# Aakash1312/Fluid-Simulation

Measured on AMD Instinct MI355X. Metric: simulated substeps/sec, higher is better.
Workload: dtype f64

## Files before the change

fluid-simulation_amd/csrc/common.h:

```cpp
#pragma once
#include <hip/hip_runtime.h>
#include <stdint.h>

namespace fl {

constexpr uint8_t F_SOLID = 1;
constexpr uint8_t F_FLUID = 2;
constexpr int F_CNT_SHIFT = 2;

struct Grid {
    int N;
    int lo;
    int hi;
    int nx, ny, nz;
    int ox, oy, oz;
    __host__ __device__ inline size_t idx(int ix, int iy, int iz) const
    {
        return ((size_t)ix * ny + (size_t)iy) * nz + (size_t)iz;
    }
    __host__ __device__ inline size_t cells() const { return (size_t)nx * ny * nz; }
    __host__ __device__ inline long sx() const { return (long)ny * nz; }
    __host__ __device__ inline int cx0() const { return lo + ox; }
    __host__ __device__ inline int cy0() const { return lo + oy; }
    __host__ __device__ inline int cz0() const { return lo + oz; }
// ... 153 lines not shown

constexpr int SUM3_PRE = 4;
struct Sum3Loads {
    double a[SUM3_PRE], b[SUM3_PRE], c[SUM3_PRE];
};
__device__ __forceinline__ void sum3_load1(const double* __restrict__ a, int n, double* v)
{
    const int last = n > 0 ? n - 1 : 0;
#pragma unroll
    for (int k = 0; k < SUM3_PRE; ++k) {
        const int i = (int)threadIdx.x + 256 * k;
        v[k] = a[i < last ? i : last];
    }
}
template <bool LATE_C = false>
__device__ __forceinline__ void block_sum3_load(const double* __restrict__ a, int na, const double* __restrict__ b, int nb,
                                                const double* __restrict__ c, int nc, Sum3Loads& v)
{
    sum3_load1(a, na, v.a);
    sum3_load1(nb > 0 ? b : a, nb, v.b);
    if (!LATE_C) sum3_load1(nc > 0 ? c : a, nc, v.c);
}
__device__ __forceinline__ double sum3_thread(const double* __restrict__ a, int n, const double* v)
{
    double s = 0;
#pragma unroll
    for (int k = 0; k < SUM3_PRE; ++k)
        if ((int)threadIdx.x + 256 * k < n) s += v[k];
    for (int i = (int)threadIdx.x + 256 * SUM3_PRE; i < n; i += 256) s += a[i];
    return s;
}
template <bool LATE_C = false>
__device__ __forceinline__ void block_sum3_sum(Sum3Loads& v, const double* __restrict__ a, int na, const double* __restrict__ b, int nb,
                                               const double* __restrict__ c, int nc, double* sm, double& ra, double& rb, double& rc)
{
    if (LATE_C) sum3_load1(nc > 0 ? c : a, nc, v.c);
    double va = sum3_thread(a, na, v.a), vb = sum3_thread(b, nb, v.b), vc = sum3_thread(c, nc, v.c);
    va = wave_sum(va); vb = wave_sum(vb); vc = wave_sum(vc);
    const int lane = threadIdx.x & 63, w = threadIdx.x >> 6;
    if (lane == 0) { sm[w] = va; sm[4 + w] = vb; sm[8 + w] = vc; }
    __syncthreads();
    ra = ((sm[0] + sm[1]) + sm[2]) + sm[3];
    rb = ((sm[4] + sm[5]) + sm[6]) + sm[7];
    rc = ((sm[8] + sm[9]) + sm[10]) + sm[11];
}
__device__ __forceinline__ void block_sum3(const double* __restrict__ a, int na, const double* __restrict__ b, int nb,
                                           const double* __restrict__ c, int nc, double* sm, double& ra, double& rb, double& rc)
{
    Sum3Loads v;
    block_sum3_load(a, na, b, nb, c, nc, v);
    block_sum3_sum(v, a, na, b, nb, c, nc, sm, ra, rb, rc);
}

struct Particles {
    double *px, *py, *pz, *vx, *vy, *vz;
    uint32_t* pid;
    __host__ __device__ inline Particles shifted(long o) const
    {
        Particles q = *this;
        q.px += o; q.py += o; q.pz += o; q.vx += o; q.vy += o; q.vz += o; q.pid += o;
        return q;
    }
};
constexpr uint32_t PID_DEAD = 0xFFFFFFFFu;

void launch_bin_count(hipStream_t st, Grid g, long n, Particles p, int* key, int* slot, int* cell_count, int* part, StepState* ss);
void launch_bin_scatter(hipStream_t st, long n, const int* key, const int* slot, const int* cell_start, const uint32_t* pid, int* order,
                         uint32_t* spid);
void launch_bin_rank(hipStream_t st, long n_pos, long pos0, const int* key, const int* cell_start, const int* order, const uint32_t* spid,
                     int* order2);
void launch_reorder(hipStream_t st, long n, const int* order, Particles src, Particles dst, double* w = nullptr, long wstride = 0);
void launch_weights(hipStream_t st, long n, Particles p, double* w, long stride);
void launch_axpby_box(hipStream_t st, Grid g, Box box, double a, const double* x, double b, const double* y, double* out, const PcgState* gate = nullptr);
long p2g_max_items(Box box);
size_t p2g_part_doubles(Box box);
constexpr int P2G_PILED = 256;
void launch_p2g(hipStream_t st, Grid g, Box box, Particles p, const double* pw, long wstride, const int* cell_start, const uint8_t* flags,
                double* part, int* items, float* container, double* u, double* v, double* w, double* ub, double* vb, double* wb, int2* crowd_list = nullptr,
                Particles park = Particles{});
void launch_p2g_tiles(hipStream_t st, Grid g, Box box, Particles p, const double* pw, long wstride, const int* cell_start, const uint8_t* flags,
                      float* container, double* u, double* v, double* w, double* ub, double* vb, double* wb);
void launch_g2p_tiled(hipStream_t st, Grid g, Box pb, Particles p, const int* cell_start, const double* dcx, const double* dcy, const double* dcz,
                      const double* pcx, const double* pcy, const double* pcz, double blend, StepState* ss);
void launch_g2p(hipStream_t st, Grid g, long n, Particles p, const double* dcx, const double* dcy, const double* dcz, const double* pcx,
                const double* pcy, const double* pcz, double blend, StepState* ss);
void launch_advect(hipStream_t st, Grid g, long n, Particles p, const uint8_t* flags, double max_dt, double dx, StepState* ss);
void launch_advect_bin(hipStream_t st, Grid g, long n, Particles p, const uint8_t* flags, double max_dt, double dx, StepState* ss, int* key,
                       int* slot, int* cell_count, int* part);
void launch_pack_particles(hipStream_t st, long n, Particles p, double* pos_aos, double* vel_aos);
void launch_unpack_records(hipStream_t st, long n, const double* rec, Particles p, long off);
void launch_pack_records(hipStream_t st, long n, Particles p, long off, double* rec);
void launch_unpack_ids(hipStream_t st, long n, const double* pos, const double* vel, const uint32_t* ids, Particles p);
void launch_pack_ids(hipStream_t st, long n, Particles p, long off, double* pos, double* vel, uint32_t* ids);
void launch_unpack_particles(hipStream_t st, long n, const double* pos_aos, const double* vel_aos, Particles p);

struct OutWin {
    int ny, nz;
    int ox, oy, oz;
    int olo[3], ohi[3];
    int lo, off;
    int l0[3], nl[3];
    __host__ __device__ inline long leaves() const { return (long)nl[0] * nl[1] * nl[2]; }
};
void launch_out_mark(hipStream_t st, const float* f, const OutWin& w, int* flags);
void launch_out_pack(hipStream_t st, const float* f, const OutWin& w, const int* flags, const int* slot, float* values, int* origin);
struct SdfGeom {
    int lo, hi;
    int bx0, by0, bz0, bnx, bny, bnz;
    int L0;
    int l0[3], nl[3];
    float R, w, dxf, bg, max2, min2;
    __host__ __device__ inline long leaves() const { return (long)nl[0] * nl[1] * nl[2]; }
    __host__ __device__ inline long cells() const { return (long)bnx * bny * bnz; }
};
void launch_sdf_bbox(hipStream_t st, long n, Particles p, int lo, int hi, int* box, bool live = false);
void launch_sdf_count(hipStream_t st, long n, Particles p, const SdfGeom& g, int* cnt, int* place, bool live = false);
void launch_sdf_scatter(hipStream_t st, long n, Particles p, const SdfGeom& g, const int* start, const int* place, double* sx, double* sy,
                        double* sz, int* ssrc = nullptr);
void launch_sdf_search(hipStream_t st, const SdfGeom& g, const int* start, const double* sx, const double* sy, const double* sz, float* tv,
                       uint64_t* tm, int* flags, unsigned* visits);
void launch_sdf_pack(hipStream_t st, const SdfGeom& g, const int* flags, const int* slot, const float* tv, const uint64_t* tm, float* values,
                     uint64_t* active, int* origin);
void launch_sdf_search_attr(hipStream_t st, const SdfGeom& g, const int* start, const double* sx, const double* sy, const double* sz, float* tv,
                            uint64_t* tm, int* flags, const int* ssrc, Particles p, uint32_t* tid, float* tvel,
                            float* tmin = nullptr);
void launch_sdf_pack_attr(hipStream_t st, const SdfGeom& g, const int* flags, const int* slot, const float* tv, const uint64_t* tm, float* values,
                          uint64_t* active, int* origin, const uint32_t* tid, const float* tvel, uint32_t* ids, float* vel,
                          const float* tmin = nullptr, float* dist2 = nullptr);
void launch_sdf_box(hipStream_t st, const SdfGeom& g, int axis, int W, float off, const int* flags, const uint64_t* tm, const float* src,
                    float* dst);
void launch_sdf_offset(hipStream_t st, const SdfGeom& g, float off, const int* flags, const uint64_t* tm, float* tv);
void launch_sdf_track(hipStream_t st, const SdfGeom& g, bool norm, bool trim, const int* flags, uint64_t* tm, const float* src, float* dst,
                      uint32_t* tid, float* tvel);
void launch_sdf_relist(hipStream_t st, const SdfGeom& g, const int* flags, const uint64_t* tm, const float* tv, int* list);
void launch_mesh_mark(hipStream_t st, const SdfGeom& g, const float* tv, const int* flags, uint64_t* cmask, int* cpre, int* vcnt, int* qcnt,
                      unsigned* tot);
void launch_mesh_emit(hipStream_t st, const SdfGeom& g, const float* tv, const int* flags, const uint64_t* tm, const float* tvel,
                      const uint64_t* cmask, const int* cpre, const int* vcnt, const int* qcnt, const int* vbase, const int* qbase, float* vertices,
                      uint32_t* quads, float* vvel, float* vnrm);
void launch_mesh_tris(hipStream_t st, long nq, long nv, const uint32_t* quads, const float* vertices, uint32_t* tris);
struct RenderGeom {
    SdfGeom g;
    int any;
    int ne[3];
    int e0[3], e1[3];
    __host__ __device__ inline long ext_leaves() const { return (long)ne[0] * ne[1] * ne[2]; }
};
}
struct fluid_camera;
struct fluid_shade;
namespace fl {
void launch_render(hipStream_t st, const RenderGeom& r, const fluid_camera& cam, const fluid_shade& sh, const float* tv, const int* flags,
                   unsigned char* neg, unsigned* occ, unsigned* hits, unsigned char* rgb, float* depth, float* normals);
void launch_exclusive_scan(hipStream_t st, const int* in, int* out, long n, int* block_sums, int* total);
void launch_sort_tail(hipStream_t st, const int* cell_count, int* cell_start, long c1, long ncell);
void launch_index_scan(hipStream_t st, Grid g, const uint8_t* flags, int* indices, int* block_sums, int* total);
void launch_index_scan_flat(hipStream_t st, const uint8_t* flags, int* indices, long n, int* block_sums, int* total);
void launch_flags(hipStream_t st, Grid g, const uint8_t* solid, const float* container, uint8_t* flags, int x0, int x1);
void launch_index_scan_range(hipStream_t st, Grid g, const uint8_t* flags, int* indices, int* block_sums, int* total, int x0, int x1);
void launch_rhs_div(hipStream_t st, Grid g, Box box, const uint8_t* flags, const double* u, const double* v, const double* w,
                    float* rhs, float* diver, double dx, double gdt0, double gdt1, double gdt2, bool rows = false, const PcgState* gate = nullptr);
void launch_vel_update(hipStream_t st, Grid g, Box box, const uint8_t* flags, const double* p, double* u, double* v, double* w,
                       double k, double g0, double g1, double g2, bool rows = false, const PcgState* gate = nullptr);
void launch_flip_delta(hipStream_t st, Grid g, Box box, const double* u, const double* v, const double* w,
                       const double* ub, const double* vb, const double* wb, double* dcx, double* dcy, double* dcz, double* pcx, double* pcy, double* pcz);
void launch_err_norm(hipStream_t st, Grid g, Box box, const uint8_t* flags, const float* b, const float* b2, double* part, StepState* ss,
                     const PcgState* gate = nullptr);
void launch_zero_step_state(hipStream_t st, StepState* ss, int N);
struct ZeroList { float* f4[4]; double* f8[7]; };
void launch_zero_fields(hipStream_t st, const ZeroList& z, Grid g, Box box, bool rows = false);
void launch_unpack_box(hipStream_t st, Grid g, Box box, const double* buf, float* container, double* u, double* v, double* w, double* ub, double* vb,
                       double* wb);

void launch_extrap_init(hipStream_t st, Grid g, const uint8_t* solid, const float* container, int* layer);
void launch_extrap_layer(hipStream_t st, Grid g, int pass, int* layer, double* u, double* v, double* w, int* n_new);
void launch_resample(hipStream_t st, Grid g, long n, Particles p, const int* cell_start, int per_cell, int xlim, double far_, int* n_parked);

struct SinkSet { int n; Box box[8]; };
__host__ __device__ inline uint64_t sm64(uint64_t x)
{
    uint64_t z = x + 0x9E3779B97F4A7C15ull;
    z = (z ^ (z >> 30)) * 0xBF58476D1CE4E5B9ull;
    z = (z ^ (z >> 27)) * 0x94D049BB133111EBull;
    return z ^ (z >> 31);
}
struct OwnBox {
    int lo[3], hi[3];
    int has_lo[3], has_hi[3];
};
struct SolidView {
    const uint8_t* p;
    int o[3];
    long sx, sy;
};
void launch_src_count(hipStream_t st, Grid g, long n, Particles p, Box box, int* hist, bool skip_dead);
void launch_src_plan(hipStream_t st, Grid g, Box box, uint64_t h0, int per_cell, bool fill, OwnBox ob, SolidView sv, const int* hist, int* cnt,
                     int* cnt_own);
void launch_src_emit(hipStream_t st, Grid g, Box box, uint64_t h0, int per_cell, bool fill, OwnBox ob, SolidView sv, const int* hist, const int* off,
                     const int* off_own, Particles p, uint32_t id0, const double vel[3]);
void launch_src_append(hipStream_t st, long n, const double* pos, const double* vel, Particles p, uint32_t pid0);
void launch_interp_from_grid(hipStream_t st, Grid g, long n, Particles p, const double* u, const double* v, const double* w);
void launch_sink_mark(hipStream_t st, Grid g, long n, Particles p, const SinkSet& sk, int* keep_dev, int* keep_pid, int* removed);
void launch_sink_compact(hipStream_t st, long n, Particles a, Particles b, const int* keep_dev, const int* dev_off, const int* pid_new);

void launch_spline_eval(hipStream_t st, int which, long n, const double* x, double* w);
void launch_dot(hipStream_t st, long n, const double* a, const double* b, double* part, int nb, double* out);

LBox make_lbox(const Box& b);
size_t lbox_max_cells(int N);
int pcg_sq_blocks(const LBox& L);
int pcg_xr_blocks(const LBox& L);
void launch_cnt_local(hipStream_t st, Grid g, LBox L, const uint8_t* flags, uint8_t* cnt);
template <typename T>
void launch_pcg_init(hipStream_t st, Grid g, LBox L, const uint8_t* cnt, const float* b, T* x, T* r, Coef<T> cf, double* part_bb,
                     double* part_rz0, PcgState* ps);
template <typename T>
void launch_pcg_sq(hipStream_t st, LBox L, const uint8_t* cnt, const T* r, const T* s_in, T* s_out, T* q, Coef<T> cf,
                   const double* part_rr, const double* part_rz_new, const double* part_rz_old, double* part_pq, PcgState* ps, int first,
                   double tol, int n_rz = -1, int zmode = 0, int sparse = 0, int n_prev = -1);
template <typename T>
void launch_pcg_xr(hipStream_t st, LBox L, const uint8_t* cnt, T* x, T* r, const T* s, const T* q, Coef<T> cf, const double* part_rz_cur,
                   const double* part_pq, double* part_rr, double* part_rz_next, PcgState* ps, int n_rz = -1, int sparse = 0);
void launch_pcg_sq_zf(hipStream_t st, LBox L, const uint8_t* cnt, const float* z, const double* s_in, double* s_out, double* q, Coef<double> cf,
                      const double* part_rr, int n_prev, const double* part_rz_new, const double* part_rz_old, double* part_pq, PcgState* ps, int first,
                      double tol, int n_rz, int sparse, const int* tlist, int nlist);
int pcg_list_blocks(int nlist);
template <typename T>
void launch_pcg_sq_list(hipStream_t st, LBox L, const uint8_t* cnt, const T* r, const T* s_in, T* s_out, T* q, Coef<T> cf,
                        const double* part_rr, int n_prev, const double* part_rz_new, const double* part_rz_old, double* part_pq, PcgState* ps,
                        int first, double tol, int n_rz, int zmode, const int* tlist, int nlist);
template <typename T>
void launch_pcg_xr_list(hipStream_t st, LBox L, const uint8_t* cnt, T* x, T* r, const T* s, const T* q, Coef<T> cf, const double* part_rz_cur,
                        int n_rz, const double* part_pq, double* part_rr, double* part_rz_next, PcgState* ps, const int* tlist, int nlist);
int pcg_row_count(const LBox& L);
int pcg_rows_blocks(int nrows);
void launch_row_list(hipStream_t st, LBox L, const uint8_t* cnt, int* flags, int* pos, int* list, int* block_sums, int* count);
constexpr int DROP_CAP = 65536;
constexpr int DROP_NCTR = 64;
void launch_drop_find(hipStream_t st, LBox L, uint8_t* cnt, int* ctr, int* pre, int* total, int* comp_n, int* comp_cells, const Box* own = nullptr);
void launch_drop_solve(hipStream_t st, Grid g, LBox L, int n_comp, const int* pre, const int* comp_n, const int* comp_cells, const uint8_t* flags,
                       const float* b, Coef<double> cf, double tol, double* pressure, double* keep, int* n_fail = nullptr, const PcgState* gate = nullptr);
template <typename T>
void launch_pcg_xr_rows(hipStream_t st, LBox L, const uint8_t* cnt, T* x, T* r, const T* s, const T* q, Coef<T> cf, const double* part_rz_cur,
                        int n_rz, const double* part_pq, int n_pq, double* part_rr, double* part_rz_next, PcgState* ps, const int* rlist, int nrows);
template <typename T>
void launch_pcg_sq_dist(hipStream_t st, LBox L, const uint8_t* cnt, const T* r, const T* s_in, T* s_out, T* q, Coef<T> cf, const double* g_rr,
                        const double* g_rz_new, const double* g_rz_old, double* part_pq, PcgState* ps, int first, double tol, int zmode);
template <typename T>
void launch_pcg_xr_dist(hipStream_t st, LBox L, const uint8_t* cnt, T* x, T* r, const T* s, const T* q, Coef<T> cf, const double* g_rz_cur,
                        const double* g_pq, double* part_rr, double* part_rz_next, PcgState* ps);
void launch_sum2(hipStream_t st, const double* a, int na, const double* b, int nb, double* out_a, double* out_b);
void launch_pcg_az_dist_zf(hipStream_t st, LBox L, const uint8_t* cnt, const float* z, double* w, Coef<double> cf, double* part_zw, PcgState* ps, const int* tlist, int nlist);
void launch_pcg_cgear_upd_zf(hipStream_t st, LBox L, const uint8_t* cnt, double* x, double* r, double* s, double* q, const float* z, const double* w, const double* g,
                             double* cg, int cur, double* part_rr, PcgState* ps, int first, double tol);
void launch_pcg_poll_stage(hipStream_t st, const double* part_rr, int n, const PcgState* ps, double* out);
void launch_pcg_poll_test(hipStream_t st, const double* g, PcgState* ps);
void launch_sum4(hipStream_t st, const double* a, int na, const double* b, int nb, const double* c, int nc, const double* e, int ne, double* out);
template <typename T>
void launch_pcg_az_dist(hipStream_t st, LBox L, const uint8_t* cnt, const T* z, T* w, Coef<T> cf, double* part_zw, PcgState* ps, const int* tlist = nullptr,
                        int nlist = 0);
template <typename T>
void launch_pcg_cgear_upd(hipStream_t st, LBox L, const uint8_t* cnt, T* x, T* r, T* s, T* q, const T* z, const T* w, const double* g, double* cg, int cur,
                          double* part_rr, PcgState* ps, int first, double tol);
template <typename T>
void launch_stencil_apply(hipStream_t st, Grid g, Box box, const uint8_t* flags, const T* s, T* q, Coef<T> cf);
template <typename T>
bool launch_stencil_march(hipStream_t st, Grid g, const uint8_t* flags, const T* s, T* q, Coef<T> cf, int variant, int cxcode);
template <typename T>
void launch_store_pressure(hipStream_t st, Grid g, LBox L, const uint8_t* cnt, const T* x, double* pressure, double* keep = nullptr,
                           const PcgState* ps = nullptr, bool gated = false);
template <typename T>
void launch_pcg_init_guess(hipStream_t st, Grid g, LBox L, const uint8_t* cnt, const float* b, const double* guess, const double* guess2, double ca,
                           double cb, T* x, T* r, Coef<T> cf, double* part_bb, double* part_rr0, PcgState* ps);

MLevel mg_level0(const LBox& L);
MLevel mg_coarser(const MLevel& f);
void launch_mg_type0(hipStream_t st, Grid g, LBox L, MLevel m, const uint8_t* flags, const uint8_t* cnt, uint8_t* typ);
void launch_mg_coarsen(hipStream_t st, MLevel mf, const uint8_t* tf, MLevel mc, uint8_t* tc, uint8_t* cnt_c);
void launch_mg_coarsen_types(hipStream_t st, MLevel mf, const uint8_t* tf, MLevel mc, uint8_t* tc);
void launch_mg_counts(hipStream_t st, MLevel m, const uint8_t* typ, uint8_t* cnt);
template <typename T>
void launch_mg_restrict(hipStream_t st, MLevel mf, const T* rf, MLevel mc, const uint8_t* cnt_c, T* fc, const PcgState* ps);
constexpr int MG_TAIL_MAX = 4;
constexpr size_t MG_TAIL_LDS = 144 * 1024;
size_t mg_tail_lds_bytes(int nl, const MLevel* lv, size_t elem);
int mg_up_blocks(const MLevel& m);
template <typename T, typename F>
void launch_mg_down(hipStream_t st, MLevel m, const uint8_t* cnt, const F* f, T* u, T* r, MLevel mc, const uint8_t* cnt_c, T* fc, MgCoef<T> cf,
                    const PcgState* ps, const int* tlist = nullptr, int nlist = 0, bool pcr = false);
template <typename T, typename F, typename O>
void launch_mg_up(hipStream_t st, MLevel m, const uint8_t* cnt, const F* f, const T* u, O* out, MLevel mc, const T* ec, MgCoef<T> cf,
                  double* part_dot, const PcgState* ps, double wc, const int* tlist = nullptr, int nlist = 0, const uint8_t* own = nullptr,
                  int pconst = 0);
bool gal_fits_coarsest(const MLevel& m);
void launch_gal_level1(hipStream_t st, MLevel m0, const uint8_t* cnt0, MgCoef<float> cf0, MLevel m1, float* gd, float* gx, float* gy, float* gz, uint8_t* cnt1);
void launch_gal_coarsen(hipStream_t st, MLevel mf, const float* fd, const float* fx, const float* fy, const float* fz, const uint8_t* cntf, MLevel mc,
                        float* gd, float* gx, float* gy, float* gz, uint8_t* cntc);
int gal_tile_count(const MLevel& m);
void launch_gal_tile_flags(hipStream_t st, MLevel m, const uint8_t* cnt, uint8_t* flags);
void launch_gal_down(hipStream_t st, MLevel m, const uint8_t* cnt, const float* gd, const float* gx, const float* gy, const float* gz, const float* f, float* u,
                     MLevel mc, float* fc, const PcgState* ps);
void launch_gal_up(hipStream_t st, MLevel m, const uint8_t* cnt, const float* gd, const float* gx, const float* gy, const float* gz, const float* f, const float* u,
                   float* out, MLevel mc, const float* ec, float wc, const PcgState* ps);
void launch_gal_coarsest(hipStream_t st, MLevel m, const float* gd, const float* gx, const float* gy, const float* gz, const float* f, float* u, int sweeps,
                         const PcgState* ps);
void launch_mg_tile_flags(hipStream_t st, MLevel m, const uint8_t* cnt, uint8_t* flags);
void launch_sq_tile_flags(hipStream_t st, LBox L, const uint8_t* cnt, uint8_t* flags);
int sq_tile_count(const LBox& L);
void launch_compact_flags(hipStream_t st, const uint8_t* flags, int n, int* list, int* count);
template <typename T>
void launch_mg_tail(hipStream_t st, int nl, const T* f0, const MLevel* lv, uint8_t* const* cnt, T* u0, const T* off, int sweeps, const PcgState* ps,
                    double wc);

}
```

fluid-simulation_amd/csrc/fluid_api.hip:

```cpp
#include "sim.h"
#include <algorithm>

using namespace fl;

static thread_local std::string g_err;
int fluid_fail(int code, const std::string& msg)
{
    g_err = msg;
    return code;
}
#define fail fluid_fail

Box fl::clip_dilate(const Box& b, int d, const Grid& g)
{
    Box r;
    r.x0 = b.x0 - d < 0 ? 0 : b.x0 - d;
    r.y0 = b.y0 - d < 0 ? 0 : b.y0 - d;
    r.z0 = b.z0 - d < 0 ? 0 : b.z0 - d;
    r.x1 = b.x1 + d > g.nx - 1 ? g.nx - 1 : b.x1 + d;
    r.y1 = b.y1 + d > g.ny - 1 ? g.ny - 1 : b.y1 + d;
    r.z1 = b.z1 + d > g.nz - 1 ? g.nz - 1 : b.z1 + d;
    return r;
}

// ... 124 lines not shown
    p->cg_tol = 2.220446049250313e-16;
    p->cg_max_iters = 0;
    p->max_outer_passes = 0;
    p->precision = FLUID_PRECISION_FP64;
    p->preconditioner = FLUID_PRECOND_MG;
    p->flip_blend = 1.0;
    p->solve_start = FLUID_START_WARM;
    p->mg_precision = FLUID_MG_FP32;
    p->dist_solve = FLUID_DIST_AUTO;
    return FLUID_OK;
}

int fluid_destroy(fluid_sim_t* s)
{
    if (!s) return FLUID_OK;
    if (s->st) hipStreamSynchronize(s->st);
    if (s->ds) dist_destroy(s);
    prof_resolve(s);
    free_particles(s);
    sources_free(s);
    output_free(s);
    render_free(s);
    mesh_free(s);
    sdf_free(s);
    void* ptrs[] = {s->solid, s->flags, s->container, s->rhs, s->diver, s->diver2, s->u, s->v, s->w, s->ub, s->vb, s->wb, s->dcx, s->dcy,
                    s->dcz, s->pressure, s->p_guess, s->p_guess2, s->p_q, s->indices, s->scan_sums, s->ipart, s->R, s->S[0], s->Q, s->X, s->mg_slab, s->mg_part, s->cntL, s->part_bb, s->part_rr,
                    s->part_rz[0], s->part_rz[1], s->part_pq, s->part_err, s->cell_count, s->cell_start, s->ss,
                    s->pcx, s->pcy, s->pcz, s->p2g_part, s->p2g_items, s->p2g_crowd, s->tl_flags, s->tl_mg, s->tl_sq, s->d_small, s->row_flags, s->row_pos, s->row_list, s->drop_n, s->drop_cells, s->drop_ctr, s->gal_slab};
    for (void* p : ptrs) if (p) hipFree(p);
    for (int i = 0; i < 2; ++i) if (s->ev_poll[i]) hipEventDestroy(s->ev_poll[i]);
    if (s->h_ss) hipHostFree(s->h_ss);
    if (s->h_small) hipHostFree(s->h_small);
    if (s->st) hipStreamDestroy(s->st);
    delete s;
    return FLUID_OK;
}

int fluid_create(const fluid_params_t* p, fluid_sim_t** out)
{
    if (!p || !out) return fail(FLUID_ERR_ARG, "null argument");
    Grid g;
    g.N = p->n;
    g.lo = -(p->n / 2);
    g.hi = g.lo + p->n - 1;
    g.nx = g.ny = g.nz = p->n;
    g.ox = g.oy = g.oz = 0;
    return fluid_create_window(p, g, out);
}

}

int fl::fluid_create_window(const fluid_params_t* p, const Grid& g, fluid_sim_t** out)
{
    if (!p || !out) return fail(FLUID_ERR_ARG, "null argument");
    if (p->n < 8 || p->n > 1024) return fail(FLUID_ERR_ARG, "n must be in [8,1024]");
    if (!(p->dx > 0) || !(p->rho > 0) || !(p->max_dt > 0)) return fail(FLUID_ERR_ARG, "dx, rho, max_dt must be > 0");
    if (p->precision != FLUID_PRECISION_FP64 && p->precision != FLUID_PRECISION_FP32) return fail(FLUID_ERR_ARG, "bad precision");
    if (!(p->flip_blend >= 0.0 && p->flip_blend <= 1.0)) return fail(FLUID_ERR_ARG, "flip_blend must be in [0,1] (1 = the reference's pure FLIP)");
    if (p->preconditioner != FLUID_PRECOND_MG && p->preconditioner != FLUID_PRECOND_JACOBI) return fail(FLUID_ERR_ARG, "bad preconditioner");
    if (p->solve_start != FLUID_START_WARM && p->solve_start != FLUID_START_ZERO) return fail(FLUID_ERR_ARG, "bad solve_start");
    if (p->mg_precision != FLUID_MG_FP32 && p->mg_precision != FLUID_MG_FP64) return fail(FLUID_ERR_ARG, "bad mg_precision");
    if (p->dist_solve < FLUID_DIST_AUTO || p->dist_solve > FLUID_DIST_REPLICATED || p->pad_ != 0) return fail(FLUID_ERR_ARG, "bad dist_solve / pad_");
    int ndev = 0;
    if (hipGetDeviceCount(&ndev) != hipSuccess || ndev <= 0)
        return fail(FLUID_ERR_HIP, "no HIP device visible: libfluid_hip has no CPU path");
    if (p->device < 0 || p->device >= ndev) return fail(FLUID_ERR_ARG, "device ordinal out of range");
    HIPCHK(hipSetDevice(p->device));
    fluid_sim* s = new fluid_sim();
    s->prm = *p;
    s->g = g;
    s->ncell = g.cells();
    s->dt = p->max_dt;
    s->mg_fp32 = p->mg_precision == FLUID_MG_FP32;
    s->warm = p->solve_start == FLUID_START_WARM;
    if (const char* e = getenv("FLUID_MG_CSWEEPS")) s->mg_csweeps = atoi(e);
    if (const char* e = getenv("FLUID_TILE_LISTS")) s->lists_force = atoi(e) != 0;
    if (const char* e = getenv("FLUID_P2G_FORM")) s->p2g_force = !strcmp(e, "rows") ? 1 : (!strcmp(e, "tiles") ? 2 : (!strcmp(e, "crowd") ? 3 : 0));
    if (const char* e = getenv("FLUID_MG_GALERKIN")) s->gal_mode = atoi(e);
    if (const char* e = getenv("FLUID_DROPLETS")) s->drops_on = atoi(e) != 0;
    if (const char* e = getenv("FLUID_ROW_SWEEPS")) s->row_sweeps = atoi(e) != 0;
    if (const char* e = getenv("FLUID_DROPLETS_MIN")) s->drop_min = atoi(e);
    if (const char* e = getenv("FLUID_ADVECT_BIN")) s->advect_bin = atoi(e) != 0;
    if (const char* e = getenv("FLUID_SOLVE_TAIL")) s->solve_tail = atoi(e) != 0;
    *out = nullptr;
    auto bail = [&](int rc) { fluid_destroy(s); return rc; };
#define A(expr) do { hipError_t e_ = (expr); if (e_ != hipSuccess) return bail(fail(FLUID_ERR_HIP, std::string(#expr) + ": " + hipGetErrorString(e_))); } while (0)
    A(hipStreamCreateWithFlags(&s->st, hipStreamNonBlocking));
    const size_t n = s->ncell;
    A(dalloc(&s->solid, n)); A(dalloc(&s->flags, n));
    A(dalloc(&s->container, n)); A(dalloc(&s->rhs, n)); A(dalloc(&s->diver, n)); A(dalloc(&s->diver2, n));
    A(dalloc(&s->u, n)); A(dalloc(&s->v, n)); A(dalloc(&s->w, n));
    A(dalloc(&s->ub, n)); A(dalloc(&s->vb, n)); A(dalloc(&s->wb, n));
    A(dalloc(&s->dcx, n)); A(dalloc(&s->dcy, n)); A(dalloc(&s->dcz, n));
    A(dalloc(&s->pressure, n));
    if (s->warm) {
        A(dalloc(&s->p_guess, n)); A(dalloc(&s->p_guess2, n));
        if (hipMemset(s->p_guess, 0, n * sizeof(double)) != hipSuccess || hipMemset(s->p_guess2, 0, n * sizeof(double)) != hipSuccess) return bail(FLUID_ERR_HIP);
        if (const char* e = getenv("FLUID_EXTRAPOLATE")) s->extrapolate = atoi(e) != 0;
        if (s->extrapolate) { A(dalloc(&s->p_q, n)); if (hipMemset(s->p_q, 0, n * sizeof(double)) != hipSuccess) return bail(FLUID_ERR_HIP); }
    }
    A(dalloc(&s->indices, n));
    A(dalloc(&s->scan_sums, (n + 2) / 2048 + 16));
    A(dalloc(&s->ipart, (size_t)1024 * 8));
    const size_t se = solver_elem(s);
    s->lmax = lbox_max_cells(std::max(g.nx, std::max(g.ny, g.nz)));
    const size_t ln = s->lmax;
    A(dalloc((char**)&s->R, ln * se)); A(dalloc((char**)&s->S[0], 2 * ln * se + 256));
    s->S[1] = (char*)s->S[0] + ln * se;
    A(dalloc((char**)&s->Q, ln * se)); A(dalloc((char**)&s->X, ln * se)); A(dalloc(&s->cntL, ln + 64));
    A(dalloc(&s->mg_part, ln / 256 + 64));
    A(dalloc(&s->part_bb, (size_t)MAX_PARTIALS)); A(dalloc(&s->part_rr, (size_t)MAX_PARTIALS));
    A(dalloc(&s->part_rz[0], (size_t)MAX_PARTIALS)); A(dalloc(&s->part_rz[1], (size_t)MAX_PARTIALS));
    A(dalloc(&s->part_pq, (size_t)MAX_PARTIALS)); A(dalloc(&s->part_err, (size_t)2 * MAX_PARTIALS));
    static_assert(sizeof(StepState) <= STATE_PS_OFF, "PcgState overlaps StepState");
    A(dalloc((char**)&s->ss, STATE_PS_OFF + sizeof(PcgState)));
    s->ps = (PcgState*)((char*)s->ss + STATE_PS_OFF);
    A(dalloc(&s->cell_count, n + 4)); A(dalloc(&s->cell_start, n + 4));
    A(dalloc(&s->d_small, (size_t)32));
    A(hipHostMalloc((void**)&s->h_small, 32 * sizeof(int)));
    A(hipEventCreateWithFlags(&s->ev_poll[0], hipEventDisableTiming));
    A(hipEventCreateWithFlags(&s->ev_poll[1], hipEventDisableTiming));
    A(hipHostMalloc((void**)&s->h_ss, STATE_PS_OFF + 2 * sizeof(PcgState)));
    s->h_ps = (PcgState*)((char*)s->h_ss + STATE_PS_OFF);
#undef A
    std::vector<uint8_t> sol(n, 0);
    const int N = p->n;
    for (int x = 0; x < g.nx; ++x)
        for (int y = 0; y < g.ny; ++y)
            for (int z = 0; z < g.nz; ++z) {
                const int X = x + g.ox, Y = y + g.oy, Z = z + g.oz;
                if (X < 2 || X > N - 3 || Y < 2 || Y > N - 3 || Z < 2 || Z > N - 3) sol[g.idx(x, y, z)] = 1;
            }
    hipError_t e = hipMemcpy(s->solid, sol.data(), n, hipMemcpyHostToDevice);
    if (e == hipSuccess) e = hipMemcpy(s->flags, sol.data(), n, hipMemcpyHostToDevice);
    if (e == hipSuccess) e = hipDeviceSynchronize();
    if (e != hipSuccess) return bail(fail(FLUID_ERR_HIP, std::string("solid upload: ") + hipGetErrorString(e)));
    *out = s;
    return FLUID_OK;
}

extern "C" {

int fluid_set_solid(fluid_sim_t* s, const uint8_t* solid)
{
    if (!s || !solid) return fail(FLUID_ERR_ARG, "null argument");
    const int N = s->g.N;
    const Grid g = s->g;
    for (int x = 0; x < N; ++x)
        for (int y = 0; y < N; ++y)
            for (int z = 0; z < N; ++z) {
                size_t c = ((size_t)x * N + y) * N + z;
                bool outsideW = x < 2 || x > N - 3 || y < 2 || y > N - 3 || z < 2 || z > N - 3;
                if (outsideW && !solid[c]) return fail(FLUID_ERR_ARG, "cells outside W=[lo+2,hi-2]^3 must be solid");
            }
    std::vector<uint8_t> sol(s->ncell);
    for (int x = 0; x < g.nx; ++x)
        for (int y = 0; y < g.ny; ++y)
            for (int z = 0; z < g.nz; ++z)
                sol[g.idx(x, y, z)] = solid[((size_t)(x + g.ox) * N + (y + g.oy)) * N + (z + g.oz)] ? 1 : 0;
    dist_keep_solid(s, solid);
    HIPCHK(hipStreamSynchronize(s->st));
    HIPCHK(hipMemcpy(s->solid, sol.data(), s->ncell, hipMemcpyHostToDevice));
    HIPCHK(hipMemcpy(s->flags, sol.data(), s->ncell, hipMemcpyHostToDevice));
    s->have_p2g = s->have_flags = false;
    s->flags_valid = false;
    s->have_guess = false;
// ... 23 lines not shown
    s->binned = false;
    s->vel_ok = false;
    return FLUID_OK;
}

int fluid_download_particles(fluid_sim_t* s, double* pos, double* vel)
{
    if (!s || !pos || !vel) return fail(FLUID_ERR_ARG, "null argument");
    if (s->dist) return fail(FLUID_ERR_STATE, "decomposed run: use fluid_download_particles_ids");
    if (s->np == 0) return FLUID_OK;
    HIPCHK(hipSetDevice(s->prm.device));
    launch_pack_particles(s->st, s->np, s->pa.shifted(s->p_off), s->stage_pos, s->stage_vel);
    HIPCHK(hipGetLastError());
    HIPCHK(hipMemcpyAsync(pos, s->stage_pos, 3 * s->np * sizeof(double), hipMemcpyDeviceToHost, s->st));
    HIPCHK(hipMemcpyAsync(vel, s->stage_vel, 3 * s->np * sizeof(double), hipMemcpyDeviceToHost, s->st));
    HIPCHK(hipStreamSynchronize(s->st));
    return FLUID_OK;
}

int64_t fluid_num_particles(fluid_sim_t* s) { return s ? s->np : -1; }
int fluid_set_dt(fluid_sim_t* s, double dt)
{
    if (!s || !(dt > 0)) return fail(FLUID_ERR_ARG, "dt must be > 0");
    s->dt = dt;
    return FLUID_OK;
}
int fluid_get_dt(fluid_sim_t* s, double* dt)
{
    if (!s || !dt) return fail(FLUID_ERR_ARG, "null argument");
    *dt = s->dt;
    return FLUID_OK;
}

static inline double u01(uint64_t seed, uint64_t ctr)
{
    uint64_t z = seed * 0x9E3779B97F4A7C15ull + ctr * 0xBF58476D1CE4E5B9ull + 0x94D049BB133111EBull;
    z ^= z >> 30; z *= 0xBF58476D1CE4E5B9ull;
    z ^= z >> 27; z *= 0x94D049BB133111EBull;
    z ^= z >> 31;
    return (double)(z >> 11) * (1.0 / 9007199254740992.0);
}

int64_t fluid_scene_water_cube_drop(int32_t n, int32_t ppc, uint64_t seed, double* pos)
{
    if (n < 8 || ppc < 1) return -1;
    const int m = (int)std::lround((double)n * 41.0 / 121.0);
    const int c0 = -(m / 2), c1 = c0 + m - 1;
    const int lo = -(n / 2), hi = lo + n - 1;
    int64_t cnt = 0;
    uint64_t ctr = 0;
    for (int x = c0; x <= c1; ++x)
        for (int y = c0; y <= c1; ++y)
            for (int z = c0; z <= c1; ++z)
                for (int k = 0; k < ppc; ++k) {
                    const double px = x - 0.5 + u01(seed, ctr), py = y - 0.5 + u01(seed, ctr + 1), pz = z - 0.5 + u01(seed, ctr + 2);
                    ctr += 3;
                    if (px > lo + 2 && px < hi - 2 && py > lo + 2 && py < hi - 2 && pz > lo + 2 && pz < hi - 2) {
                        if (pos) { pos[3 * cnt] = px; pos[3 * cnt + 1] = py; pos[3 * cnt + 2] = pz; }
                        cnt++;
                    }
                }
    return cnt;
}

}

int fl::read_ss(fluid_sim* s)
{
    HIPCHK(hipMemcpyAsync(s->h_ss, s->ss, sizeof(StepState), hipMemcpyDeviceToHost, s->st));
    HIPCHK(hipStreamSynchronize(s->st));
    return FLUID_OK;
}

int fl::clear_dirty(fluid_sim* s)
{
    if (box_empty(s->dirty)) return FLUID_OK;
    const ZeroList z = {{s->container, s->rhs, s->diver, s->diver2}, {s->u, s->v, s->w, s->ub, s->vb, s->wb, s->pressure}};
    launch_zero_fields(s->st, z, s->g, s->dirty, !s->dist && s->row_sweeps);
    HIPCHK(hipGetLastError());
    s->dirty = Box{0, 0, 0, -1, -1, -1};
    return FLUID_OK;
}

int fl::sort_pass(fluid_sim* s, int ax0, int ax1, int* h_tail)
{
    const Grid g = s->g;
    const long ncell = (long)s->ncell, n2 = g.sx();
    const long c0 = (long)ax0 * n2, c1 = (long)(ax1 + 1) * n2;
    launch_zero_step_state(s->st, s->ss, g.N);
    HIPCHK(hipMemsetAsync(s->cell_count + c0, 0, (c1 - c0) * sizeof(int), s->st));
    HIPCHK(hipMemsetAsync(s->cell_count + ncell, 0, 4 * sizeof(int), s->st));
    launch_bin_count(s->st, g, s->np, s->pa.shifted(s->p_off), s->key, s->slot, s->cell_count, s->ipart, s->ss);
    launch_exclusive_scan(s->st, s->cell_count + c0, s->cell_start + c0, c1 - c0, s->scan_sums, s->cell_start + c1);
    launch_sort_tail(s->st, s->cell_count, s->cell_start, c1, ncell);
    launch_bin_scatter(s->st, s->np, s->key, s->slot, s->cell_start, s->pa.shifted(s->p_off).pid, s->order, s->spid);
    launch_bin_rank(s->st, s->np, 0, s->key, s->cell_start, s->order, s->spid, s->order2);
    HIPCHK(hipGetLastError());
    if (h_tail) HIPCHK(hipMemcpyAsync(h_tail, s->cell_start + ncell, 3 * sizeof(int), hipMemcpyDeviceToHost, s->st));
    return read_ss(s);
}

static int sort_binned(fluid_sim* s)
{
    const Grid g = s->g;
    const long ncell = (long)s->ncell, n2 = g.sx();
    const long c0 = (long)s->bin_x0 * n2, c1 = (long)(s->bin_x1 + 1) * n2;
    launch_zero_step_state(s->st, s->ss, g.N);
    launch_exclusive_scan(s->st, s->cell_count + c0, s->cell_start + c0, c1 - c0, s->scan_sums, s->cell_start + c1);
    launch_sort_tail(s->st, s->cell_count, s->cell_start, c1, ncell);
    launch_bin_scatter(s->st, s->np, s->key, s->slot, s->cell_start, s->pa.shifted(s->p_off).pid, s->order, s->spid);
    launch_bin_rank(s->st, s->np, 0, s->key, s->cell_start, s->order, s->spid, s->order2);
    HIPCHK(hipGetLastError());
    StepState& h = *s->h_ss;
    for (int a = 0; a < 3; ++a) h.bbox_min[a] = s->bin_min[a], h.bbox_max[a] = s->bin_max[a];
    h.n_out = s->bin_n_out;
    h.max_cell = s->bin_max_cell;
    return FLUID_OK;
}

static int phase_sort(fluid_sim* s)
{
    const Grid g = s->g;
    int tok = prof_begin(s, FLUID_PROF_SORT, (double)s->np);
    int ax0 = 0, ax1 = g.nx - 1;
    const bool guess = s->sort_hint && !box_empty(s->Pb);
    if (guess) {
        ax0 = std::max(0, s->Pb.x0 - 3);
        ax1 = std::min(g.nx - 1, s->Pb.x1 + 3);
    }
    const bool binned = s->binned && guess && ax0 == s->bin_x0 && ax1 == s->bin_x1 && s->np > 0;
    s->binned = false;
    const auto missed = [&](const int* bmin, const int* bmax) {
        return guess && bmax[0] >= 0 && (bmin[0] < std::min(ax0 + 2, s->Pb.x0) || bmax[0] > std::max(ax1 - 2, s->Pb.x1));
    };
    int rc;
    if (binned && !missed(s->bin_min, s->bin_max)) {
        if ((rc = sort_binned(s))) return rc;
    } else {
        rc = binned ? FLUID_OK : sort_pass(s, ax0, ax1);
        if (rc) return rc;
        if (binned || missed(s->h_ss->bbox_min, s->h_ss->bbox_max)) {
            if ((rc = sort_pass(s, 0, g.nx - 1))) return rc;
        }
    }
    s->sort_hint = true;
    s->n_out = s->h_ss->n_out;
    s->max_cell = s->h_ss->max_cell;
    const StepState& h = *s->h_ss;
    if (h.bbox_max[0] < 0) {
        s->Pb = Box{0, 0, 0, -1, -1, -1};
    } else {
        s->Pb = Box{h.bbox_min[0], h.bbox_min[1], h.bbox_min[2], h.bbox_max[0], h.bbox_max[1], h.bbox_max[2]};
    }
    if (!box_empty(s->Pb)) {
        s->Rb = clip_dilate(s->Pb, 1, g);
        s->Sb = clip_dilate(s->Pb, 2, g);
    } else {
        s->Rb = s->Sb = s->Pb;
    }
    launch_reorder(s->st, s->np, s->order2, s->pa.shifted(s->p_off), s->pb, s->pw, s->cap);
    HIPCHK(hipGetLastError());
    std::swap(s->pa, s->pb);
    s->p_off = 0;
    prof_end(s, FLUID_PROF_SORT, tok);
    s->sorted = true;
    return FLUID_OK;
}

int fl::run_p2g(fluid_sim* s, const Box& box)
{
    const long ref_cells = s->p2g_ref_cells > 0 ? s->p2g_ref_cells : s->Rb.cells();
    const bool airy = s->last_num_active > 0 && (double)s->last_num_active < 0.3 * (double)ref_cells;
    const bool huge = (size_t)12 * sizeof(double) * (size_t)box.cells() > ((size_t)16 << 30);
    const bool piled = s->max_cell > P2G_PILED || airy;
    if (s->p2g_force ? s->p2g_force == 2 : huge) {
        s->stats.paths |= FLUID_PATH_P2G_TILES;
        launch_p2g_tiles(s->st, s->g, box, s->pa, s->pw, s->cap, s->cell_start, s->flags, s->container, s->u, s->v, s->w, s->ub, s->vb, s->wb);
        return FLUID_OK;
    }
    const bool crowd = s->p2g_force ? s->p2g_force == 3 : piled;
    if (crowd) {
        s->stats.paths |= FLUID_PATH_P2G_CROWD;
        const size_t nl = (size_t)s->cap / 16 + 64;
        if (nl > s->p2g_crowd_cap) {
            if (s->p2g_crowd) { HIPCHK(hipStreamSynchronize(s->st)); hipFree(s->p2g_crowd); s->p2g_crowd = nullptr; }
            HIPCHK(hipMalloc((void**)&s->p2g_crowd, nl * sizeof(int2)));
            s->p2g_crowd_cap = nl;
        }
    }
    const size_t need = p2g_part_doubles(box);
    if (need > s->p2g_part_cap) {
        if (s->p2g_part) { HIPCHK(hipStreamSynchronize(s->st)); hipFree(s->p2g_part); s->p2g_part = nullptr; }
// ... 32 lines not shown
        prof_end(s, FLUID_PROF_P2G, tok);
        if (rc) return rc;
        HIPCHK(hipGetLastError());
        s->dirty = s->Sb;
    }
    s->have_p2g = true;
    s->step_counter++;
    s->have_flags = false;
    return FLUID_OK;
}

template <typename T>
Coef<T> fl::make_coef(const fluid_sim* s)
{
    const double scale = s->dt / (s->prm.rho * s->prm.dx * s->prm.dx);
    Coef<T> c;
    float acc = 0.0f;
    c.diag[0] = 0;
    c.inv[0] = 0;
    for (int k = 1; k <= 6; ++k) {
        acc = (float)((double)acc + scale);
        c.diag[k] = (T)acc;
        c.inv[k] = (T)1 / c.diag[k];
    }
    c.off = (T)(float)(-1 * scale);
    return c;
}
template Coef<double> fl::make_coef<double>(const fluid_sim*);
template Coef<float> fl::make_coef<float>(const fluid_sim*);

hipError_t fl::zero_search(fluid_sim* s, size_t lb)
{
    const size_t step = (lb + 255) / 256 * 256;
    s->S[1] = (char*)s->S[0] + step;
    return hipMemsetAsync(s->S[0], 0, step + lb, s->st);
}


static int gal_build(fluid_sim* s);
static int mg_setup(fluid_sim* s)
{
    s->mgl[0] = mg_level0(s->L);
    int nl = 1;
    while (nl < fluid_sim::MG_MAXL && (nl < 2 || s->mgl[nl - 1].dx > 8 || s->mgl[nl - 1].dy > 8 || s->mgl[nl - 1].dz > 8)) {
        s->mgl[nl] = mg_coarser(s->mgl[nl - 1]);
        ++nl;
    }
    if (s->mgl[nl - 1].dx > 8 || s->mgl[nl - 1].dy > 8 || s->mgl[nl - 1].dz > 8) return fail(FLUID_ERR_STATE, "multigrid: too many levels");
    s->mg_nl = nl;
    int tail = nl - 1;
    const size_t es = s->mg_fp32 ? sizeof(float) : sizeof(double);
    auto fits = [&](int t) {
        const size_t b = nl - t <= MG_TAIL_MAX ? mg_tail_lds_bytes(nl - t, s->mgl + t, es) : 0;
        return b > 0 && b <= MG_TAIL_LDS;
    };
    while (tail > 1 && fits(tail - 1)) --tail;
    if (!fits(tail)) return fail(FLUID_ERR_STATE, "multigrid: coarsest level does not fit the tail kernel");
    s->mg_tail = tail;
    size_t total = 0;
    auto take = [&](size_t bytes) { const size_t o = total; total += (bytes + 255) / 256 * 256; return o; };
    size_t o_typ[fluid_sim::MG_MAXL], o_cnt[fluid_sim::MG_MAXL], o_u[fluid_sim::MG_MAXL], o_v[fluid_sim::MG_MAXL], o_f[fluid_sim::MG_MAXL],
        o_r[fluid_sim::MG_MAXL];
    for (int l = 0; l < nl; ++l) {
        const size_t c = s->mgl[l].cells + 64;
        o_typ[l] = take(c); o_cnt[l] = take(c);
        o_u[l] = take(c * es); o_v[l] = take(c * es); o_f[l] = take(c * es); o_r[l] = take(c * es);
    }
    const size_t o_z = take((s->mgl[0].cells + 64) * 8);
    if (total > s->mg_slab_cap) {
        if (s->mg_slab) { HIPCHK(hipStreamSynchronize(s->st)); hipFree(s->mg_slab); s->mg_slab = nullptr; }
        const size_t cap = total + total / 4;
        HIPCHK(hipMalloc((void**)&s->mg_slab, cap));
        s->mg_slab_cap = cap;
    }
    for (int l = 0; l < nl; ++l) {
        s->mg_typ[l] = (uint8_t*)(s->mg_slab + o_typ[l]);
        s->mg_cnt[l] = l ? (uint8_t*)(s->mg_slab + o_cnt[l]) : nullptr;
        s->mg_u[l] = s->mg_slab + o_u[l]; s->mg_v[l] = s->mg_slab + o_v[l];
        s->mg_f[l] = l ? s->mg_slab + o_f[l] : nullptr;
        s->mg_r[l] = s->mg_slab + o_r[l];
    }
    s->Zmg = s->mg_slab + o_z;
    HIPCHK(hipMemsetAsync(s->mg_slab, 0, total, s->st));
    launch_mg_type0(s->st, s->g, s->L, s->mgl[0], s->flags, s->cntL, s->mg_typ[0]);
    for (int l = 1; l < nl; ++l) launch_mg_coarsen(s->st, s->mgl[l - 1], s->mg_typ[l - 1], s->mgl[l], s->mg_typ[l], s->mg_cnt[l]);
    { int rcg = gal_build(s); if (rcg) return rcg; }
    HIPCHK(hipGetLastError());
    return FLUID_OK;
}

MgCoef<double> fl::mg_coef(const fluid_sim* s, int level)
{
    MgCoef<double> c;
    if (level == 0) {
        const Coef<double> f = make_coef<double>(s);
        for (int k = 0; k < 7; ++k) { c.diag[k] = f.diag[k]; c.inv[k] = f.inv[k]; }
        c.off = f.off;
        return c;
    }
    const double scale = s->dt / (s->prm.rho * s->prm.dx * s->prm.dx) / std::pow(4.0, level);
    c.off = -scale;
    c.diag[0] = 0; c.inv[0] = 0;
    for (int k = 1; k < 7; ++k) { c.diag[k] = scale * k; c.inv[k] = 1.0 / c.diag[k]; }
    return c;
}

static int mg_rz_blocks(const fluid_sim* s) { return s->lists_on ? s->n_tl_mg : mg_up_blocks(s->mgl[0]); }

template <typename V>
static MgCoef<V> mg_coef_as(const fluid_sim* s, int level)
{
    const MgCoef<double> d = mg_coef(s, level);
    MgCoef<V> c;
    for (int k = 0; k < 7; ++k) { c.diag[k] = (V)d.diag[k]; c.inv[k] = (V)d.inv[k]; }
    c.off = (V)d.off;
    return c;
}
static int gal_build(fluid_sim* s)
{
    s->gal = false;
    s->gal_eligible = false;
    const int nl = s->mg_nl;
    int lc = 1;
    while (lc < nl - 1 && !gal_fits_coarsest(s->mgl[lc])) ++lc;
    if (!(s->gal_mode && s->lists_on && s->mg_fp32 && !s->dist && (long)s->mgl[0].dx * s->mgl[0].dy * s->mgl[0].dz > 200000 &&
          gal_fits_coarsest(s->mgl[lc]) && lc >= 2)) {
        s->gal_it[0] = s->gal_it[1] = -1;
        return FLUID_OK;
    }
    s->gal_eligible = true;
    bool use = s->gal_mode >= 2;
    if (s->gal_mode == 1) {
        if (s->gal_it[0] < 0) use = false;
        else if (s->gal_it[1] < 0) use = true;
        else {
            use = 21 * s->gal_it[1] < 20 * s->gal_it[0];
            if (++s->gal_since_probe >= 32) { use = !use; s->gal_since_probe = 0; }
        }
    }
    if (!use) return FLUID_OK;
    size_t total = 0, off[fluid_sim::MG_MAXL][6];
    for (int l = 1; l <= lc; ++l)
        for (int q = 0; q < 6; ++q) {
            off[l][q] = total;
            total += (q < 5 ? ((q < 4 ? sizeof(float) : 1) * (s->mgl[l].cells + 64) + 255) / 256 * 256 : ((size_t)gal_tile_count(s->mgl[l]) + 255) / 256 * 256);
        }
    if (total > s->gal_slab_cap) {
        if (s->gal_slab) { HIPCHK(hipStreamSynchronize(s->st)); hipFree(s->gal_slab); s->gal_slab = nullptr; }
        HIPCHK(hipMalloc((void**)&s->gal_slab, total + total / 4));
        s->gal_slab_cap = total + total / 4;
    }
    HIPCHK(hipMemsetAsync(s->gal_slab, 0, total, s->st));
    for (int l = 1; l <= lc; ++l) {
        for (int q = 0; q < 4; ++q) s->gal_c[l][q] = (float*)(s->gal_slab + off[l][q]);
        s->gal_cnt[l] = (uint8_t*)(s->gal_slab + off[l][4]);
        s->gal_tfl[l] = (uint8_t*)(s->gal_slab + off[l][5]);
    }
    launch_gal_level1(s->st, s->mgl[0], s->cntL, mg_coef_as<float>(s, 0), s->mgl[1], s->gal_c[1][0], s->gal_c[1][1], s->gal_c[1][2], s->gal_c[1][3], s->gal_cnt[1]);
    for (int l = 2; l <= lc; ++l)
        launch_gal_coarsen(s->st, s->mgl[l - 1], s->gal_c[l - 1][0], s->gal_c[l - 1][1], s->gal_c[l - 1][2], s->gal_c[l - 1][3], s->gal_cnt[l - 1], s->mgl[l],
                           s->gal_c[l][0], s->gal_c[l][1], s->gal_c[l][2], s->gal_c[l][3], s->gal_cnt[l]);
    for (int l = 1; l < lc; ++l) launch_gal_tile_flags(s->st, s->mgl[l], s->gal_cnt[l], s->gal_tfl[l]);
    s->gal = true;
    s->gal_lc = lc;
    s->gal_dt = s->dt;
    HIPCHK(hipGetLastError());
    return FLUID_OK;
}
static int mg_vcycle_gal(fluid_sim* s, const double* rhs0, float* z0, double* part_rz)
{
    typedef float V;
    const PcgState* ps = s->ps;
    const int lc = s->gal_lc;
    auto U = [&](int l) { return (V*)s->mg_u[l]; };
    auto W = [&](int l) { return (V*)s->mg_v[l]; };
    auto F = [&](int l) { return (V*)s->mg_f[l]; };
    auto C = [&](int l, int q) { return (const float*)s->gal_c[l][q]; };
    const MLevel& m0 = s->mgl[0];
    launch_mg_down<V, double>(s->st, m0, s->cntL, rhs0, U(0), (V*)s->mg_r[0], s->mgl[1], nullptr, F(1), mg_coef_as<V>(s, 0), ps, s->tl_mg, s->n_tl_mg, true);
    for (int l = 1; l < lc; ++l) launch_gal_down(s->st, s->mgl[l], s->gal_tfl[l], C(l, 0), C(l, 1), C(l, 2), C(l, 3), F(l), U(l), s->mgl[l + 1], F(l + 1), ps);
    launch_gal_coarsest(s->st, s->mgl[lc], C(lc, 0), C(lc, 1), C(lc, 2), C(lc, 3), F(lc), U(lc), s->gal_sweeps, ps);
    for (int l = lc - 1; l >= 1; --l)
        launch_gal_up(s->st, s->mgl[l], s->gal_tfl[l], C(l, 0), C(l, 1), C(l, 2), C(l, 3), F(l), U(l), W(l), s->mgl[l + 1], l + 1 == lc ? U(l + 1) : W(l + 1),
                      (float)s->gal_wc, ps);
    const int tok = prof_begin(s, FLUID_PROF_MG_UP0, (double)s->Rb.cells());
    launch_mg_up<V, double, float>(s->st, m0, s->cntL, rhs0, (const V*)U(0), z0, s->mgl[1], W(1), mg_coef_as<V>(s, 0), part_rz, ps, s->gal_wc, s->tl_mg, s->n_tl_mg,
                                   nullptr, 1);
    prof_end(s, FLUID_PROF_MG_UP0, tok);
    HIPCHK(hipGetLastError());
    return FLUID_OK;
}

template <typename V>
static int mg_vcycle_t(fluid_sim* s, const double* rhs0, V* z0, double* part_rz)
{
    const int nl = s->mg_nl, tail = s->mg_tail;
    const PcgState* ps = s->ps;
    auto U = [&](int l) { return (V*)s->mg_u[l]; };
    auto W = [&](int l) { return (V*)s->mg_v[l]; };
    auto F = [&](int l) { return (V*)s->mg_f[l]; };
    auto R = [&](int l) { return (V*)s->mg_r[l]; };
    for (int l = 0; l < tail; ++l) {
        const MLevel& m = s->mgl[l];
        const bool fold = l > 0 || (long)m.dx * m.dy * m.dz <= 200000;
        V* fc = fold ? F(l + 1) : nullptr;
        const uint8_t* cc = fold ? s->mg_cnt[l + 1] : nullptr;
        const bool lst = s->lists_on && !fold;
        if (l == 0) launch_mg_down<V, double>(s->st, m, s->cntL, rhs0, U(0), R(0), s->mgl[1], cc, fc, mg_coef_as<V>(s, 0), ps, lst ? s->tl_mg : nullptr, s->n_tl_mg);
        else launch_mg_down<V, V>(s->st, m, s->mg_cnt[l], (const V*)F(l), U(l), R(l), s->mgl[l + 1], cc, fc, mg_coef_as<V>(s, l), ps);
        if (!fold) launch_mg_restrict<V>(s->st, m, (const V*)R(l), s->mgl[l + 1], s->mg_cnt[l + 1], F(l + 1), ps);
    }
    {
        V off[fluid_sim::MG_MAXL];
        for (int l = tail; l < nl; ++l) off[l] = (V)mg_coef(s, l).off;
        launch_mg_tail<V>(s->st, nl - tail, (const V*)F(tail), s->mgl + tail, s->mg_cnt + tail, U(tail), off + tail, s->mg_csweeps, ps, s->mg_wc[3]);
    }
    for (int l = tail - 1; l >= 0; --l) {
        const MLevel& m = s->mgl[l];
        const V* ec = l + 1 == tail ? U(l + 1) : W(l + 1);
        if (l == 0) {
            const int tok = prof_begin(s, FLUID_PROF_MG_UP0, (double)s->Rb.cells());
            launch_mg_up<V, double, V>(s->st, m, s->cntL, rhs0, (const V*)U(0), z0, s->mgl[1], ec, mg_coef_as<V>(s, 0), part_rz, ps, s->mg_wc[0],
                                       s->lists_on ? s->tl_mg : nullptr, s->n_tl_mg);
            prof_end(s, FLUID_PROF_MG_UP0, tok);
        } else {
            launch_mg_up<V, V, V>(s->st, m, s->mg_cnt[l], (const V*)F(l), (const V*)U(l), W(l), s->mgl[l + 1], ec, mg_coef_as<V>(s, l), nullptr, ps, s->mg_wc[l == 1 ? 1 : 2]);
        }
    }
    HIPCHK(hipGetLastError());
    return FLUID_OK;
}
static int mg_vcycle(fluid_sim* s, const double* rhs0, void* z0, double* part_rz)
{
    if (s->gal && s->lists_on) return mg_vcycle_gal(s, rhs0, (float*)z0, part_rz);
    return s->mg_fp32 ? mg_vcycle_t<float>(s, rhs0, (float*)z0, part_rz) : mg_vcycle_t<double>(s, rhs0, (double*)z0, part_rz);
}

static int phase_vel_update(fluid_sim* s, const PcgState* gate = nullptr);
static int phase_rhs_div(fluid_sim* s, int which, const PcgState* gate = nullptr);
static int solve_mg(fluid_sim* s, bool with_tail)
{
    typedef double T;
    const Grid g = s->g;
    const LBox L = s->L;
    T* X = (T*)s->X;
    T* R = (T*)s->R;
    T* Q = (T*)s->Q;
    T* Sx[2] = {(T*)s->S[0], (T*)s->S[1]};
    T* Z = (T*)s->Zmg;
    const uint8_t* cnt = s->cntL;
    const Coef<T> cf = make_coef<T>(s);
    const double tol = s->prm.cg_tol;
    long max_it = s->prm.cg_max_iters > 0 ? s->prm.cg_max_iters : 2 * (long)s->stats.num_active;
    if (max_it < 1) max_it = 1;
    const double cells = (double)s->Rb.cells();
    const int sparse = (double)s->stats.num_active < 0.4 * (double)L.cells();
    const bool lists = s->lists_on;
    const bool rows = lists && s->rows_on && s->n_rows > 0;
    const int n_init = pcg_xr_blocks(L), n_list = rows ? pcg_rows_blocks(s->n_rows) : pcg_list_blocks(s->n_tl_sq);
    const int n_rz_raw = mg_rz_blocks(s);
    const bool fold = n_rz_raw > 1024;
    const int n_rz = fold ? 1 : n_rz_raw;
    int rc;
    int tsolve = prof_begin(s, FLUID_PROF_SOLVE, cells);
    if (s->gal && s->gal_dt != s->dt) {
        const int keep = s->gal_mode; s->gal_mode = 2; rc = gal_build(s); s->gal_mode = keep;
        if (rc) return rc;
    }
    if (s->gal) s->stats.paths |= FLUID_PATH_MG_GALERKIN;
    const bool guess = s->warm && s->have_guess;
    const double *g1, *g2;
    double gca, gcb;
    s->start_guess(g1, g2, gca, gcb);
    if (guess) launch_pcg_init_guess<T>(s->st, g, L, cnt, s->diver, g1, g2, gca, gcb, X, R, cf, s->part_bb, s->part_rz[1], s->ps);
    else launch_pcg_init<T>(s->st, g, L, cnt, s->diver, X, R, cf, s->part_bb, s->part_rr, s->ps);
    long it = 0;
    const int pclass = s->pass_class();
    long batch = s->mg_last_iters_k[pclass] > 5 ? s->mg_last_iters_k[pclass] + 1 : 4;
    bool done = false;
    const bool zf = s->mg_fp32 || (s->gal && s->lists_on);
    auto sq = [&](int cur, const double* part_rr, int n_prev, const double* rz_new, const double* rz_old, int first, int sp) {
        const int prv = cur ^ 1;
        if (zf)
            launch_pcg_sq_zf(s->st, L, cnt, (const float*)s->Zmg, Sx[prv], Sx[cur], Q, cf, part_rr, n_prev, rz_new, rz_old, s->part_pq, s->ps, first, tol, n_rz, sp,
                             lists ? s->tl_sq : nullptr, s->n_tl_sq);
        else if (lists)
            launch_pcg_sq_list<T>(s->st, L, cnt, Z, Sx[prv], Sx[cur], Q, cf, part_rr, n_prev, rz_new, rz_old, s->part_pq, s->ps, first, tol, n_rz, 1, s->tl_sq, s->n_tl_sq);
        else
            launch_pcg_sq<T>(s->st, L, cnt, Z, Sx[prv], Sx[cur], Q, cf, part_rr, rz_new, rz_old, s->part_pq, s->ps, first, tol, n_rz, 1, sp, n_prev);
    };
    const bool will_make_q = s->warm && s->p_q && s->stats.outer_passes == 1 && s->guess_step == s->step_counter && s->guess_pass == 0;
    auto solution_out = [&](const PcgState* gate) {
        launch_store_pressure<T>(s->st, g, L, cnt, X, s->pressure, s->warm ? s->p_guess2 : nullptr, s->ps, gate != nullptr);
        launch_drop_solve(s->st, g, L, s->n_drop, s->drop_ctr + 64 * DROP_NCTR, s->drop_n, s->drop_cells, s->flags, s->diver, make_coef<double>(s), tol,
                          s->pressure, s->warm ? s->p_guess2 : nullptr, &s->ss->n_drop_fail, gate);
        if (will_make_q) launch_axpby_box(s->st, g, s->Rb, 1.0, s->p_guess2, -(1.0 - s->prm.update_frac), s->p_guess, s->p_q, gate);
    };
    bool first_poll = true;
// ... 224 lines not shown
    HIPCHK(hipStreamSynchronize(s->st));
    int iters = s->h_ps->iters;
    const double rr = s->h_ps->rr;
    if (!s->h_ps->done) {
        iters = (int)max_it;
    }
    launch_store_pressure<T>(s->st, g, L, cnt, X, s->pressure);
    launch_drop_solve(s->st, g, L, s->n_drop, s->drop_ctr + 64 * DROP_NCTR, s->drop_n, s->drop_cells, s->flags, s->diver, make_coef<double>(s), tol,
                      s->pressure, nullptr, &s->ss->n_drop_fail);
    HIPCHK(hipGetLastError());
    prof_end(s, FLUID_PROF_SOLVE, tsolve);
    s->stats.cg_iters_last = iters;
    s->stats.cg_iters += iters;
    s->stats.relres = s->h_ps->bb > 0 ? std::sqrt(rr / s->h_ps->bb) : 0.0;
    if (s->h_ps->breakdown) return fail(FLUID_ERR_SOLVER, "PCG breakdown: s.As <= 0 or NaN (matrix not SPD for these flags)");
    return FLUID_OK;
}

static int phase_solve(fluid_sim* s, bool with_tail = false)
{
    s->tail_ran = false;
    if (!s->have_flags) return fail(FLUID_ERR_STATE, "solve before flags_index");
    if (box_empty(s->Rb)) return FLUID_OK;
    if (use_mg(s) && s->mg_nl >= 2) return solve_mg(s, with_tail);
    return s->prm.precision == FLUID_PRECISION_FP32 ? solve_impl<float>(s) : solve_impl<double>(s);
}

static int phase_vel_update(fluid_sim* s, const PcgState* gate)
{
    if (!s->have_flags) return fail(FLUID_ERR_STATE, "vel_update before flags_index");
    if (box_empty(s->Sb)) return FLUID_OK;
    const double dtp = s->dt * s->prm.update_frac;
    const double k = dtp / (s->prm.rho * s->prm.dx);
    launch_vel_update(s->st, s->g, s->Sb, s->flags, s->pressure, s->u, s->v, s->w, k, s->prm.gravity[0] * dtp, s->prm.gravity[1] * dtp,
                      s->prm.gravity[2] * dtp, !s->dist && s->row_sweeps, gate);
    HIPCHK(hipGetLastError());
    return FLUID_OK;
}

int fl::phase_pressure_pass(fluid_sim* s, double* error)
{
    int rc;
    if ((rc = phase_rhs_div(s, 0))) return rc;
    if ((rc = phase_solve(s, true))) return rc;
    const bool tail_ran = s->tail_ran;
    s->tail_ran = false;
    if (!tail_ran) {
        if ((rc = phase_vel_update(s))) return rc;
        if ((rc = phase_rhs_div(s, 1))) return rc;
    }
    double err = NAN;
    if (!box_empty(s->Rb)) {
        if (!tail_ran) {
            launch_err_norm(s->st, s->g, s->Rb, s->flags, s->diver, s->diver2, s->part_err, s->ss);
            HIPCHK(hipGetLastError());
            if ((rc = read_ss(s))) return rc;
        }
        if (s->h_ss->n_drop_fail > 0) s->stats.paths |= FLUID_PATH_DROPLETS_SHORT;
        err = std::sqrt(s->h_ss->err_num) / std::sqrt(s->h_ss->err_den);
    }
    s->stats.error = err;
    s->stats.outer_passes++;
    if (error) *error = err;
    return FLUID_OK;
}

int fl::pic_fields(fluid_sim* s)
{
    if (s->prm.flip_blend >= 1.0 || s->pcx) return FLUID_OK;
    double** f[3] = {&s->pcx, &s->pcy, &s->pcz};
    for (double** q : f) {
        HIPCHK(hipMalloc((void**)q, s->ncell * sizeof(double)));
        HIPCHK(hipMemsetAsync(*q, 0, s->ncell * sizeof(double), s->st));
    }
    return FLUID_OK;
}

static int phase_flip_advect(fluid_sim* s)
{
    if (!s->have_p2g) return fail(FLUID_ERR_STATE, "flip_advect before p2g");
    HIPCHK(hipSetDevice(s->prm.device));
    int rcp = pic_fields(s);
    if (rcp) return rcp;
    if (!box_empty(s->Rb)) launch_flip_delta(s->st, s->g, s->Rb, s->u, s->v, s->w, s->ub, s->vb, s->wb, s->dcx, s->dcy, s->dcz, s->pcx, s->pcy, s->pcz);
    int tok = prof_begin(s, FLUID_PROF_G2P, (double)s->np);
    if (s->sorted && s->p_off == 0 && (double)s->np >= 4.0 * (double)s->Pb.cells()) {
        launch_g2p_tiled(s->st, s->g, s->Pb, s->pa, s->cell_start, s->dcx, s->dcy, s->dcz, s->pcx, s->pcy, s->pcz, s->prm.flip_blend, s->ss);
        if (!box_empty(s->Pb)) s->stats.paths |= FLUID_PATH_G2P_TILES;
        if (s->n_out > 0)
            launch_g2p(s->st, s->g, s->n_out, s->pa.shifted(s->np - s->n_out), s->dcx, s->dcy, s->dcz, s->pcx, s->pcy, s->pcz, s->prm.flip_blend, s->ss);
    } else {
        launch_g2p(s->st, s->g, s->np, s->pa.shifted(s->p_off), s->dcx, s->dcy, s->dcz, s->pcx, s->pcy, s->pcz, s->prm.flip_blend, s->ss);
    }
    prof_end(s, FLUID_PROF_G2P, tok);
    const bool bin = s->advect_bin && !s->dist && s->np > 0 && s->sorted && s->sort_hint && !box_empty(s->Pb);
    s->binned = false;
    if (bin) {
        const Grid g = s->g;
        s->bin_x0 = std::max(0, s->Pb.x0 - 3);
        s->bin_x1 = std::min(g.nx - 1, s->Pb.x1 + 3);
        const long n2 = g.sx(), c0 = (long)s->bin_x0 * n2, c1 = (long)(s->bin_x1 + 1) * n2;
        HIPCHK(hipMemsetAsync(s->cell_count + c0, 0, (c1 - c0) * sizeof(int), s->st));
        HIPCHK(hipMemsetAsync(s->cell_count + s->ncell, 0, 4 * sizeof(int), s->st));
        launch_advect_bin(s->st, g, s->np, s->pa.shifted(s->p_off), s->flags, s->prm.max_dt, s->prm.dx, s->ss, s->key, s->slot, s->cell_count, s->ipart);
    } else {
        launch_advect(s->st, s->g, s->np, s->pa.shifted(s->p_off), s->flags, s->prm.max_dt, s->prm.dx, s->ss);
    }
    HIPCHK(hipGetLastError());
    int rc = read_ss(s);
    if (rc) return rc;
    if (bin) {
        const StepState& h = *s->h_ss;
        for (int a = 0; a < 3; ++a) s->bin_min[a] = h.bbox_min[a], s->bin_max[a] = h.bbox_max[a];
        s->bin_n_out = h.n_out;
        s->bin_max_cell = h.max_cell;
        s->binned = true;
    }
    s->dt = s->h_ss->dt;
    double ms;
    memcpy(&ms, &s->h_ss->max_speed_bits, sizeof(double));
    s->stats.max_speed = ms;
    s->stats.dt_out = s->dt;
    s->sorted = false;
    s->have_p2g = false;
    s->vel_ok = true;
    return FLUID_OK;
}

extern "C" {

#define PHASE_GUARD(s)                                                                                        \
    if (!(s)) return fail(FLUID_ERR_ARG, "null handle");                                                      \
    if ((s)->dist) return fail(FLUID_ERR_STATE, "per-phase entry points are single-GPU only; a decomposed run steps with fluid_step")
int fluid_p2g(fluid_sim_t* s) { PHASE_GUARD(s); return phase_p2g(s); }
int fluid_flags_index(fluid_sim_t* s) { PHASE_GUARD(s); return phase_flags(s); }
int fluid_rhs_div(fluid_sim_t* s, int which) { PHASE_GUARD(s); return phase_rhs_div(s, which, nullptr); }
int fluid_solve(fluid_sim_t* s) { PHASE_GUARD(s); return phase_solve(s, false); }
int fluid_vel_update(fluid_sim_t* s) { PHASE_GUARD(s); return phase_vel_update(s, nullptr); }
int fluid_pressure_pass(fluid_sim_t* s, double* error) { PHASE_GUARD(s); return phase_pressure_pass(s, error); }
int fluid_flip_advect(fluid_sim_t* s) { PHASE_GUARD(s); return phase_flip_advect(s); }

int fluid_extrapolate(fluid_sim_t* s, int32_t* n_layers)
{
    PHASE_GUARD(s);
    if (!s->have_p2g) return fail(FLUID_ERR_STATE, "extrapolate before p2g");
    HIPCHK(hipSetDevice(s->prm.device));
    const Grid g = s->g;
    int* layer = s->indices;
    int* n_new = s->d_small;
    launch_extrap_init(s->st, g, s->solid, s->container, layer);
    int pass = 0;
    for (bool more = true; more;) {
        HIPCHK(hipMemsetAsync(n_new, 0, sizeof(int), s->st));
        for (int k = 0; k < 8; ++k) launch_extrap_layer(s->st, g, ++pass, layer, s->u, s->v, s->w, n_new);
        HIPCHK(hipGetLastError());
        HIPCHK(hipMemcpyAsync(s->h_small, n_new, sizeof(int), hipMemcpyDeviceToHost, s->st));
        HIPCHK(hipStreamSynchronize(s->st));
        more = s->h_small[0] != 0 && pass < 3 * g.N + 8;
    }
    const size_t bytes = s->ncell * sizeof(double);
    HIPCHK(hipMemcpyAsync(s->ub, s->u, bytes, hipMemcpyDeviceToDevice, s->st));
    HIPCHK(hipMemcpyAsync(s->vb, s->v, bytes, hipMemcpyDeviceToDevice, s->st));
    HIPCHK(hipMemcpyAsync(s->wb, s->w, bytes, hipMemcpyDeviceToDevice, s->st));
    s->flags_valid = false;
    s->have_flags = false;
    s->dirty = Box{0, 0, 0, g.nx - 1, g.ny - 1, g.nz - 1};
    HIPCHK(hipStreamSynchronize(s->st));
    if (n_layers) *n_layers = pass;
    return FLUID_OK;
}

int fluid_get_droplets(fluid_sim_t* s, int32_t* n_components, int64_t* cells, int32_t cap_components)
{
    if (!s) return fail(FLUID_ERR_ARG, "null handle");
    if (n_components) *n_components = s->n_drop;
    if (!cells || s->n_drop <= 0 || cap_components <= 0) return FLUID_OK;
    HIPCHK(hipSetDevice(s->prm.device));
    const int n = std::min(s->n_drop, (int)cap_components);
    std::vector<int> pre(DROP_NCTR + 1), an(DROP_CAP), ac((size_t)DROP_CAP * 64), hn(n), hc((size_t)n * 64);
    HIPCHK(hipStreamSynchronize(s->st));
    HIPCHK(hipMemcpy(pre.data(), s->drop_ctr + 64 * DROP_NCTR, pre.size() * sizeof(int), hipMemcpyDeviceToHost));
    HIPCHK(hipMemcpy(an.data(), s->drop_n, an.size() * sizeof(int), hipMemcpyDeviceToHost));
    HIPCHK(hipMemcpy(ac.data(), s->drop_cells, ac.size() * sizeof(int), hipMemcpyDeviceToHost));
    for (int d = 0, c = 0; d < n; ++d) {
        while (c + 1 < DROP_NCTR && pre[c + 1] <= d) ++c;
        const size_t slot = (size_t)c * (DROP_CAP / DROP_NCTR) + (size_t)(d - pre[c]);
// ... 305 lines not shown
```

fluid-simulation_amd/csrc/fluid_dist.hip:

```cpp
#include "sim.h"
#include "dist_kernels.h"

using namespace fl;
#define fail fluid_fail
int cuts_from_hist(int n, const int64_t* hist, int P, int32_t* cuts);

#define COMMCHK(expr)                                                                              \
    do {                                                                                           \
        if ((expr) != 0) return fail(FLUID_ERR_HIP, std::string("comm callback failed: ") + #expr); \
    } while (0)

namespace {

constexpr int HALO_W = 4;

struct IBox {
    int lo[3], hi[3];
};
inline bool ib_empty(const IBox& b) { return b.hi[0] <= b.lo[0] || b.hi[1] <= b.lo[1] || b.hi[2] <= b.lo[2]; }
inline IBox ib_isect(const IBox& a, const IBox& b)
{
    IBox r;
    for (int k = 0; k < 3; ++k) { r.lo[k] = std::max(a.lo[k], b.lo[k]); r.hi[k] = std::min(a.hi[k], b.hi[k]); }
    if (ib_empty(r)) for (int k = 0; k < 3; ++k) { r.lo[k] = a.lo[k]; r.hi[k] = a.lo[k]; }
// ... 830 lines not shown
            if (halo_pending) {
                if (d->n_int) launch_mg_down<G, double>(s->st, L.m, L.cnt, rhs0, GU(0), (G*)s->mg_r[0], mc, nullptr, GF(1), coef_as<G>(s, 0), ps, d->tl_int, d->n_int, true);
                if ((rc = halo_exchange_end(s, L.plan, sizeof(double)))) return rc;
                if (d->n_bnd) launch_mg_down<G, double>(s->st, L.m, L.cnt, rhs0, GU(0), (G*)s->mg_r[0], mc, nullptr, GF(1), coef_as<G>(s, 0), ps, d->tl_bnd, d->n_bnd, true);
            } else {
                launch_mg_down<G, double>(s->st, L.m, L.cnt, rhs0, GU(0), (G*)s->mg_r[0], mc, nullptr, GF(1), coef_as<G>(s, 0), ps, s->lists_on ? s->tl_mg : nullptr,
                                          s->n_tl_mg, true);
            }
            HIPCHK(hipGetLastError());
        } else if (halo_pending) {
            if ((rc = halo_exchange_end(s, L.plan, sizeof(double)))) return rc;
        }
        if (d->split_exchange) {
            if ((rc = halo_exchange1(s, d->plan_split, sizeof(G), GF(1)))) return rc;
        } else {
            int lo[3];
            for (int a = 0; a < 3; ++a) lo[a] = d->dom0.lo[a] >> 1;
            IBox gb;
            for (int a = 0; a < 3; ++a) { gb.lo[a] = lo[a]; gb.hi[a] = lo[a] + (a == 0 ? s->mgl[1].dx : (a == 1 ? s->mgl[1].dy : s->mgl[1].dz)); }
            const IBox o = ib_isect(block_level(d, d->comm.rank, 1, s->g.N), gb);
            launch_mask_outside<G>(s->st, s->mgl[1], to_box(o, lo), GF(1));
            HIPCHK(hipGetLastError());
            if ((rc = comm_allreduce(s, GF(1), (long)s->mgl[1].cells, FLUID_DT_F32, FLUID_OP_SUM))) return rc;
        }
        for (int l = 1; l < lc; ++l) launch_gal_down(s->st, s->mgl[l], s->gal_tfl[l], C(l, 0), C(l, 1), C(l, 2), C(l, 3), GF(l), GU(l), s->mgl[l + 1], GF(l + 1), ps);
        launch_gal_coarsest(s->st, s->mgl[lc], C(lc, 0), C(lc, 1), C(lc, 2), C(lc, 3), GF(lc), GU(lc), s->gal_sweeps, ps);
        for (int l = lc - 1; l >= 1; --l)
            launch_gal_up(s->st, s->mgl[l], s->gal_tfl[l], C(l, 0), C(l, 1), C(l, 2), C(l, 3), GF(l), GU(l), GW(l), s->mgl[l + 1], l + 1 == lc ? GU(l + 1) : GW(l + 1),
                          (float)s->gal_wc, ps);
        if (!ib_empty(L.dom)) {
            const int tok = prof_begin(s, FLUID_PROF_MG_UP0, (double)ib_cells(L.dom));
            if (zf)
                launch_mg_up<G, double, float>(s->st, L.m, L.cnt, rhs0, (const G*)GU(0), (float*)z0v, mc, GW(1), coef_as<G>(s, 0), part_rz, ps, s->gal_wc,
                                               s->lists_on ? s->tl_mg : nullptr, s->n_tl_mg, d->cnt_pcg, 1);
            else
                launch_mg_up<G, double, double>(s->st, L.m, L.cnt, rhs0, (const G*)GU(0), z0, mc, GW(1), coef_as<G>(s, 0), part_rz, ps, s->gal_wc,
                                                s->lists_on ? s->tl_mg : nullptr, s->n_tl_mg, d->cnt_pcg, 1);
            prof_end(s, FLUID_PROF_MG_UP0, tok);
        }
        HIPCHK(hipGetLastError());
        return FLUID_OK;
    }
    for (int l = 0; l < split; ++l) {
        DLevel& L = d->lv[l];
        const MLevel mc = ib_empty(L.dom) ? s->mgl[l + 1] : under(l);
        const uint8_t* cc = l + 1 < split ? d->lv[l + 1].cnt : s->mg_cnt[l + 1];
        if (!ib_empty(L.dom)) {
            if (l == 0) {
                if (halo_pending) {
                    if (d->n_int) launch_mg_down<V, double>(s->st, L.m, L.cnt, rhs0, U(0), R(0), mc, nullptr, nullptr, coef_as<V>(s, 0), ps, d->tl_int, d->n_int);
                    if ((rc = halo_exchange_end(s, L.plan, sizeof(double)))) return rc;
                    if (d->n_bnd) launch_mg_down<V, double>(s->st, L.m, L.cnt, rhs0, U(0), R(0), mc, nullptr, nullptr, coef_as<V>(s, 0), ps, d->tl_bnd, d->n_bnd);
                } else {
                    launch_mg_down<V, double>(s->st, L.m, L.cnt, rhs0, U(0), R(0), mc, nullptr, nullptr, coef_as<V>(s, 0), ps, s->lists_on ? s->tl_mg : nullptr, s->n_tl_mg);
                }
                launch_mg_restrict<V>(s->st, L.m, (const V*)R(0), mc, cc, F(1), ps);
            } else {
                launch_mg_down<V, V>(s->st, L.m, L.cnt, (const V*)F(l), U(l), R(l), mc, cc, F(l + 1), coef_as<V>(s, l), ps);
            }
            HIPCHK(hipGetLastError());
        }
        if (l + 1 < split) {
            if ((rc = halo_exchange1(s, d->lv[l + 1].plan, sizeof(V), F(l + 1)))) return rc;
        } else {
            if (d->split_exchange) {
                if ((rc = halo_exchange1(s, d->plan_split, sizeof(V), F(l + 1)))) return rc;
            } else {
                int lo[3];
                for (int a = 0; a < 3; ++a) lo[a] = d->dom0.lo[a] >> (l + 1);
                IBox gb;
                for (int a = 0; a < 3; ++a) { gb.lo[a] = lo[a]; gb.hi[a] = lo[a] + (a == 0 ? s->mgl[l + 1].dx : (a == 1 ? s->mgl[l + 1].dy : s->mgl[l + 1].dz)); }
                const IBox o = ib_isect(block_level(d, d->comm.rank, l + 1, s->g.N), gb);
                launch_mask_outside<V>(s->st, s->mgl[l + 1], to_box(o, lo), F(l + 1));
                HIPCHK(hipGetLastError());
                if ((rc = comm_allreduce(s, F(l + 1), (long)s->mgl[l + 1].cells, sizeof(V) == 4 ? FLUID_DT_F32 : FLUID_DT_F64, FLUID_OP_SUM))) return rc;
            }
        }
    }
    for (int l = split; l < tail; ++l)
        launch_mg_down<V, V>(s->st, s->mgl[l], s->mg_cnt[l], (const V*)F(l), U(l), R(l), s->mgl[l + 1], s->mg_cnt[l + 1], F(l + 1), coef_as<V>(s, l), ps);
    {
        V off[fluid_sim::MG_MAXL];
        for (int l = tail; l < nl; ++l) off[l] = (V)mg_coef(s, l).off;
        launch_mg_tail<V>(s->st, nl - tail, (const V*)F(tail), s->mgl + tail, s->mg_cnt + tail, U(tail), off + tail, s->mg_csweeps, ps, s->mg_wc[3]);
    }
    for (int l = tail - 1; l >= split; --l) {
        const V* ec = l + 1 == tail ? U(l + 1) : W(l + 1);
        launch_mg_up<V, V, V>(s->st, s->mgl[l], s->mg_cnt[l], (const V*)F(l), (const V*)U(l), W(l), s->mgl[l + 1], ec, coef_as<V>(s, l), nullptr, ps,
                              s->mg_wc[l == 1 ? 1 : 2]);
    }
    HIPCHK(hipGetLastError());
    for (int l = split - 1; l >= 0; --l) {
        DLevel& L = d->lv[l];
        const V* ec = l + 1 == tail ? U(l + 1) : W(l + 1);
        if (!ib_empty(L.dom)) {
            const MLevel mc = under(l);
            if (l == 0) {
                const int tok = prof_begin(s, FLUID_PROF_MG_UP0, (double)ib_cells(L.dom));
                if constexpr (std::is_same<V, float>::value) {
                    if (zf)
                        launch_mg_up<float, double, float>(s->st, L.m, L.cnt, rhs0, (const float*)U(0), (float*)z0v, mc, ec, coef_as<float>(s, 0), part_rz, ps, s->mg_wc[0],
                                                           s->lists_on ? s->tl_mg : nullptr, s->n_tl_mg, d->cnt_pcg);
                }
                if (!zf)
                    launch_mg_up<V, double, double>(s->st, L.m, L.cnt, rhs0, (const V*)U(0), z0, mc, ec, coef_as<V>(s, 0), part_rz, ps, s->mg_wc[0],
                                                    s->lists_on ? s->tl_mg : nullptr, s->n_tl_mg, d->cnt_pcg);
                prof_end(s, FLUID_PROF_MG_UP0, tok);
            } else {
                launch_mg_up<V, V, V>(s->st, L.m, L.cnt, (const V*)F(l), (const V*)U(l), W(l), mc, ec, coef_as<V>(s, l), nullptr, ps, s->mg_wc[l == 1 ? 1 : 2]);
            }
            HIPCHK(hipGetLastError());
        }
        if (l > 0 && (rc = halo_exchange1(s, L.plan, sizeof(V), W(l)))) return rc;
    }
    return FLUID_OK;
}

int dist_solve(fluid_sim* s)
{
    typedef double T;
    DistState* d = s->ds;
    const Grid g = s->g;
    const LBox L = s->L;
    T *X = (T*)s->X, *R = (T*)s->R, *Q = (T*)s->Q, *Z = (T*)s->Zmg;
    T* Sx[2] = {(T*)s->S[0], (T*)s->S[1]};
    const uint8_t* cnt = d->cnt_pcg;
    const Coef<T> cf = make_coef<T>(s);
    const double tol = s->prm.cg_tol;
    const bool mg = use_mg(s);
    long max_it = s->prm.cg_max_iters > 0 ? s->prm.cg_max_iters : 2 * (long)s->stats.num_active;
    if (max_it < 1) max_it = 1;
    const bool lists = mg && s->lists_on;
    const int nxr = pcg_xr_blocks(L), nsq = lists && d->cg_form == 1 ? pcg_list_blocks(s->n_tl_sq) : pcg_sq_blocks(L);
    const int n_rz = ib_empty(d->lv[0].dom) ? 0 : (lists ? s->n_tl_mg : mg_up_blocks(d->lv[0].m));
    const double cells = (double)ib_cells(d->lv[0].own);
    int rc;
    int tsolve = prof_begin(s, FLUID_PROF_SOLVE, cells);
    const bool guess = mg && s->warm && s->have_guess;
    const double *g1, *g2;
    double gca, gcb;
    s->start_guess(g1, g2, gca, gcb);
    if (guess) launch_pcg_init_guess<T>(s->st, g, L, cnt, s->diver, g1, g2, gca, gcb, X, R, cf, s->part_bb, s->part_rz[1], s->ps);
    else launch_pcg_init<T>(s->st, g, L, cnt, s->diver, X, R, cf, s->part_bb, s->part_rz[0], s->ps);
    if (mg && d->overlap && !d->overlap_checked && d->comm.size > 1) {
        HaloPlan& hp = d->lv[0].plan;
        const size_t nb = hp.n ? (size_t)hp.rtotal * sizeof(T) : 0;
        std::vector<unsigned char> a(nb), b(nb);
        if ((rc = halo_exchange1(s, hp, sizeof(T), R))) return rc;
        if (nb) HIPCHK(hipMemcpyAsync(a.data(), d->hr, nb, hipMemcpyDeviceToHost, s->st));
        if (nb) HIPCHK(hipMemsetAsync(d->hr, 0xFF, nb, s->st));
        if (hp.n && !ib_empty(d->lv[0].dom)) {
            if ((rc = halo_exchange_begin(s, hp, sizeof(T), R))) return rc;
            if ((rc = halo_exchange_end(s, hp, sizeof(T)))) return rc;
        } else if ((rc = halo_exchange1(s, hp, sizeof(T), R))) return rc;
        if (nb) HIPCHK(hipMemcpyAsync(b.data(), d->hr, nb, hipMemcpyDeviceToHost, s->st));
        HIPCHK(hipStreamSynchronize(s->st));
        int* flag = d->h_cnt + 97;
        *flag = nb && memcmp(a.data(), b.data(), nb) != 0 ? 1 : 0;
        HIPCHK(hipMemcpyAsync(d->d_cnt + 97, flag, sizeof(int), hipMemcpyHostToDevice, s->st));
        if ((rc = comm_allreduce(s, d->d_cnt + 97, 1, FLUID_DT_I32, FLUID_OP_MAX))) return rc;
        HIPCHK(hipMemcpyAsync(flag, d->d_cnt + 97, sizeof(int), hipMemcpyDeviceToHost, s->st));
        HIPCHK(hipStreamSynchronize(s->st));
        d->overlap_checked = *flag ? 2 : 1;
        if (*flag) d->overlap = false;
    }
    long it = 0;
    const int pclass = s->pass_class();
// ... 884 lines not shown
```

fluid-simulation_amd/csrc/kernels_grid.hip:

```cpp
#include "common.h"

namespace fl {

constexpr int SCAN_T = 256;
constexpr int SCAN_E = 8;
constexpr int SCAN_CHUNK = SCAN_T * SCAN_E;

template <int MODE>
__device__ __forceinline__ int scan_load(const void* in, long i)
{
    if (MODE == 0) return ((const int*)in)[i];
    return (((const uint8_t*)in)[i] & F_FLUID) ? 1 : 0;
}

template <int MODE, bool VEC>
__device__ __forceinline__ void scan_load8(const void* in, long base, long n, int v[SCAN_E])
{
    if (VEC && base >= 0 && base + SCAN_E <= n) {
        if (MODE == 0) {
            const int4 a = *(const int4*)((const int*)in + base), b = *(const int4*)((const int*)in + base + 4);
            v[0] = a.x; v[1] = a.y; v[2] = a.z; v[3] = a.w;
            v[4] = b.x; v[5] = b.y; v[6] = b.z; v[7] = b.w;
        } else {
            const uint2 w = *(const uint2*)((const uint8_t*)in + base);
#pragma unroll
            for (int e = 0; e < 4; ++e) {
                v[e] = ((w.x >> (8 * e)) & F_FLUID) ? 1 : 0;
                v[4 + e] = ((w.y >> (8 * e)) & F_FLUID) ? 1 : 0;
            }
        }
    } else {
#pragma unroll
        for (int e = 0; e < SCAN_E; ++e) v[e] = (base + e >= 0 && base + e < n) ? scan_load<MODE>(in, base + e) : 0;
    }
}

template <int MODE, bool VEC>
__global__ __launch_bounds__(SCAN_T) void k_scan_sums(const void* __restrict__ in, long n, int lead, int* __restrict__ block_sums)
{
    __shared__ int sm[4];
    const long base = (long)blockIdx.x * SCAN_CHUNK + (long)threadIdx.x * SCAN_E - lead;
    int v[SCAN_E];
    scan_load8<MODE, VEC>(in, base, n, v);
    int s = 0;
#pragma unroll
    for (int e = 0; e < SCAN_E; ++e) s += v[e];
    s = block_sum<int, 4>(s, sm);
    if (threadIdx.x == 0) block_sums[blockIdx.x] = s;
}

__global__ __launch_bounds__(1024) void k_scan_block_sums(int* __restrict__ block_sums, int nb, int* __restrict__ total)
{
    __shared__ int wsum[16];
    __shared__ int carry_s;
    if (threadIdx.x == 0) carry_s = 0;
    __syncthreads();
    const int lane = threadIdx.x & 63, w = threadIdx.x >> 6;
    for (int base = 0; base < nb; base += 1024) {
        int i = base + threadIdx.x;
        int v = i < nb ? block_sums[i] : 0;
        int inc = v;
#pragma unroll
        for (int o = 1; o < 64; o <<= 1) {
            int t = __shfl_up(inc, o, 64);
            if (lane >= o) inc += t;
        }
        if (lane == 63) wsum[w] = inc;
        __syncthreads();
        int woff = 0;
        for (int k = 0; k < w; ++k) woff += wsum[k];
        int carry = carry_s;
        if (i < nb) block_sums[i] = carry + woff + inc - v;
        __syncthreads();
        if (threadIdx.x == 1023) carry_s = carry + woff + inc;
        __syncthreads();
    }
    if (threadIdx.x == 0) *total = carry_s;
}

template <int MODE, bool VEC>
__global__ __launch_bounds__(SCAN_T) void k_scan_final(const void* __restrict__ in, long n, int lead, const int* __restrict__ block_sums,
                                                       int* __restrict__ out)
{
    __shared__ int wsum[4];
    const long base = (long)blockIdx.x * SCAN_CHUNK + (long)threadIdx.x * SCAN_E - lead;
    int v[SCAN_E];
    scan_load8<MODE, VEC>(in, base, n, v);
    int s = 0;
#pragma unroll
    for (int e = 0; e < SCAN_E; ++e) s += v[e];
    const int lane = threadIdx.x & 63, w = threadIdx.x >> 6;
    int inc = s;
#pragma unroll
    for (int o = 1; o < 64; o <<= 1) {
        int t = __shfl_up(inc, o, 64);
        if (lane >= o) inc += t;
    }
    if (lane == 63) wsum[w] = inc;
    __syncthreads();
    int off = block_sums[blockIdx.x] + inc - s;
    for (int k = 0; k < w; ++k) off += wsum[k];
    int r[SCAN_E];
#pragma unroll
    for (int e = 0; e < SCAN_E; ++e) {
        r[e] = (MODE == 0 || v[e]) ? off : -1;
        off += v[e];
    }
    if (VEC && base >= 0 && base + SCAN_E <= n) {
        *(int4*)(out + base) = make_int4(r[0], r[1], r[2], r[3]);
        *(int4*)(out + base + 4) = make_int4(r[4], r[5], r[6], r[7]);
    } else {
#pragma unroll
        for (int e = 0; e < SCAN_E; ++e)
            if (base + e >= 0 && base + e < n) out[base + e] = r[e];
    }
}

template <int MODE>
static void scan_impl(hipStream_t st, const void* in, int* out, long n, int* block_sums, int* total)
{
    const int lead = MODE == 0 ? (int)(((uintptr_t)in & 15) / 4) : (int)((uintptr_t)in & 7);
    const bool vec = (((uintptr_t)out - (uintptr_t)4 * lead) & 15) == 0 && (MODE == 1 || ((uintptr_t)in & 3) == 0);
    if (vec) {
        const int nb = (int)((n + lead + SCAN_CHUNK - 1) / SCAN_CHUNK);
        hipLaunchKernelGGL((k_scan_sums<MODE, true>), dim3(nb), dim3(SCAN_T), 0, st, in, n, lead, block_sums);
        hipLaunchKernelGGL(k_scan_block_sums, dim3(1), dim3(1024), 0, st, block_sums, nb, total);
        hipLaunchKernelGGL((k_scan_final<MODE, true>), dim3(nb), dim3(SCAN_T), 0, st, in, n, lead, (const int*)block_sums, out);
    } else {
        const int nb = (int)((n + SCAN_CHUNK - 1) / SCAN_CHUNK);
        hipLaunchKernelGGL((k_scan_sums<MODE, false>), dim3(nb), dim3(SCAN_T), 0, st, in, n, 0, block_sums);
        hipLaunchKernelGGL(k_scan_block_sums, dim3(1), dim3(1024), 0, st, block_sums, nb, total);
        hipLaunchKernelGGL((k_scan_final<MODE, false>), dim3(nb), dim3(SCAN_T), 0, st, in, n, 0, (const int*)block_sums, out);
    }
}

void launch_exclusive_scan(hipStream_t st, const int* in, int* out, long n, int* block_sums, int* total)
{
    scan_impl<0>(st, in, out, n, block_sums, total);
}
void launch_index_scan_flat(hipStream_t st, const uint8_t* flags, int* indices, long n, int* block_sums, int* total)
{
    scan_impl<1>(st, flags, indices, n, block_sums, total);
}
void launch_index_scan(hipStream_t st, Grid g, const uint8_t* flags, int* indices, int* block_sums, int* total)
{
    scan_impl<1>(st, flags, indices, (long)g.cells(), block_sums, total);
}

__global__ __launch_bounds__(256) void k_flags(Grid g, const uint8_t* __restrict__ solid, const float* __restrict__ container,
                                               uint8_t* __restrict__ flags, long c_begin, long c_end)
{
    long c = c_begin + (long)blockIdx.x * 256 + threadIdx.x;
    if (c >= c_end) return;
    const int iz = (int)(c % g.nz), iy = (int)((c / g.nz) % g.ny), ix = (int)(c / g.sx());
    const uint8_t sol = solid[c] ? F_SOLID : 0;
    uint8_t f = sol;
    if (!sol && container[c] > 0) {
        int cnt = 0;
        cnt += (ix > 0) ? !solid[c - g.sx()] : 1;
        cnt += (ix < g.nx - 1) ? !solid[c + g.sx()] : 1;
        cnt += (iy > 0) ? !solid[c - g.nz] : 1;
        cnt += (iy < g.ny - 1) ? !solid[c + g.nz] : 1;
        cnt += (iz > 0) ? !solid[c - 1] : 1;
        cnt += (iz < g.nz - 1) ? !solid[c + 1] : 1;
        f = (uint8_t)(F_FLUID | (cnt << F_CNT_SHIFT));
    }
    flags[c] = f;
}

__global__ __launch_bounds__(256) void k_flags4(Grid g, const uint8_t* __restrict__ solid, const float* __restrict__ container,
                                                uint8_t* __restrict__ flags, long c_begin, long c_end)
{
    const long c = c_begin + ((long)blockIdx.x * 256 + threadIdx.x) * 4;
    if (c >= c_end) return;
    const int iz = (int)(c % g.nz), iy = (int)((c / g.nz) % g.ny), ix = (int)(c / g.sx());
    const uint32_t so = *(const uint32_t*)(solid + c);
    const float4 co = *(const float4*)(container + c);
    const float cv[4] = {co.x, co.y, co.z, co.w};
    bool any = false;
#pragma unroll
    for (int q = 0; q < 4; ++q) any |= !((so >> (8 * q)) & 0xff) && cv[q] > 0;
    uint32_t out = 0;
#pragma unroll
    for (int q = 0; q < 4; ++q) out |= (((so >> (8 * q)) & 0xff) ? (uint32_t)F_SOLID : 0u) << (8 * q);
    if (any) {
        const uint32_t xm = ix > 0 ? *(const uint32_t*)(solid + c - g.sx()) : 0u, xp = ix < g.nx - 1 ? *(const uint32_t*)(solid + c + g.sx()) : 0u;
        const uint32_t ym = iy > 0 ? *(const uint32_t*)(solid + c - g.nz) : 0u, yp = iy < g.ny - 1 ? *(const uint32_t*)(solid + c + g.nz) : 0u;
        const uint32_t zm = iz > 0 ? solid[c - 1] : 0u, zp = iz + 4 < g.nz ? solid[c + 4] : 0u;
        out = 0;
#pragma unroll
        for (int q = 0; q < 4; ++q) {
            const uint32_t sol = (so >> (8 * q)) & 0xff;
            uint32_t f = sol ? (uint32_t)F_SOLID : 0u;
            if (!sol && cv[q] > 0) {
                int cnt = 0;
                cnt += !((xm >> (8 * q)) & 0xff);
                cnt += !((xp >> (8 * q)) & 0xff);
                cnt += !((ym >> (8 * q)) & 0xff);
                cnt += !((yp >> (8 * q)) & 0xff);
                cnt += !(q == 0 ? zm : (so >> (8 * (q - 1))) & 0xff);
                cnt += !(q == 3 ? zp : (so >> (8 * (q + 1))) & 0xff);
                f = (uint32_t)(F_FLUID | (cnt << F_CNT_SHIFT));
            }
            out |= f << (8 * q);
        }
    }
    *(uint32_t*)(flags + c) = out;
}

void launch_flags(hipStream_t st, Grid g, const uint8_t* solid, const float* container, uint8_t* flags, int x0, int x1)
{
    const long n2 = g.sx(), c0 = (long)x0 * n2, c1 = (long)(x1 + 1) * n2;
    if (c1 <= c0) return;
    if (g.nz % 4 == 0)
        hipLaunchKernelGGL(k_flags4, dim3((unsigned)(((c1 - c0) / 4 + 255) / 256)), dim3(256), 0, st, g, solid, container, flags, c0, c1);
    else
        hipLaunchKernelGGL(k_flags, dim3((unsigned)((c1 - c0 + 255) / 256)), dim3(256), 0, st, g, solid, container, flags, c0, c1);
}

void launch_index_scan_range(hipStream_t st, Grid g, const uint8_t* flags, int* indices, int* block_sums, int* total, int x0, int x1)
{
// ... 503 lines not shown
```

fluid-simulation_amd/csrc/kernels_mg.hip:

```cpp
#include "common.h"
#include <cstdlib>
#include <cstring>

namespace fl {

constexpr double MG_W1 = 0.5617, MG_W2 = 1.3895;

template <typename T>
__device__ __forceinline__ void mg_load_coef(T* sd, T* si, const MgCoef<T>& cf)
{
    if (threadIdx.x == 0) {
#pragma unroll
        for (int i = 0; i < 7; ++i) {
            sd[i] = cf.diag[i];
            si[i] = cf.inv[i];
        }
    }
    __syncthreads();
}

__device__ __forceinline__ bool mg_cell(const MLevel& m, long t, int& i, int& j, int& k)
{
    const unsigned n = (unsigned)m.dx * (unsigned)m.dy * (unsigned)m.dz;
    if (t >= (long)n) return false;
    const unsigned u = (unsigned)t, dz = (unsigned)m.dz, dy = (unsigned)m.dy;
    const unsigned q = u / dz;
    k = (int)(u - q * dz);
    const unsigned p = q / dy;
    j = (int)(q - p * dy);
    i = (int)p;
    return true;
}

__global__ __launch_bounds__(256) void k_mg_type0(Grid g, LBox L, MLevel m, const uint8_t* __restrict__ flags, const uint8_t* __restrict__ cnt,
                                                  uint8_t* __restrict__ typ)
{
    int i, j, k;
    if (!mg_cell(m, (long)blockIdx.x * 256 + threadIdx.x, i, j, k)) return;
    const int gx = L.x0 + i - 1, gy = L.y0 + j - 1, gz = L.z0 + k - 1;
    uint8_t t = 0;
    const size_t c = m.at(i, j, k);
    if (gx >= 0 && gx < g.nx && gy >= 0 && gy < g.ny && gz >= 0 && gz < g.nz) {
        const uint8_t f = flags[g.idx(gx, gy, gz)];
        t = (f & F_SOLID) ? 0 : (cnt[c] ? 2 : 1);
    }
    typ[c] = t;
}

__global__ __launch_bounds__(256) void k_mg_coarsen(MLevel mf, const uint8_t* __restrict__ tf, MLevel mc, uint8_t* __restrict__ tc)
{
    int I, J, K;
    if (!mg_cell(mc, (long)blockIdx.x * 256 + threadIdx.x, I, J, K)) return;
    bool any_air = false, all_solid = true;
#pragma unroll
    for (int a = 0; a < 8; ++a) {
        const int i = 2 * I + (a & 1), j = 2 * J + ((a >> 1) & 1), k = 2 * K + (a >> 2);
        uint8_t t = 0;
        if (i < mf.dx && j < mf.dy && k < mf.dz) t = tf[mf.at(i, j, k)];
        any_air |= (t == 1);
        all_solid &= (t == 0);
    }
    tc[mc.at(I, J, K)] = any_air ? 1 : (all_solid ? 0 : 2);
}

__global__ __launch_bounds__(256) void k_mg_cnt(MLevel m, const uint8_t* __restrict__ typ, uint8_t* __restrict__ cnt)
{
    int i, j, k;
    if (!mg_cell(m, (long)blockIdx.x * 256 + threadIdx.x, i, j, k)) return;
    const size_t c = m.at(i, j, k);
    uint8_t n = 0;
    if (typ[c] == 2) {
        n = (typ[c - m.sx] != 0) + (typ[c + m.sx] != 0) + (typ[c - m.sy] != 0) + (typ[c + m.sy] != 0) + (typ[c - 1] != 0) + (typ[c + 1] != 0);
    }
    cnt[c] = n;
}


struct IoPlain {
    template <typename X> static __device__ __forceinline__ X ld(const X* p) { return *p; }
    template <typename X> static __device__ __forceinline__ void st(X* p, X v) { *p = v; }
};
struct IoSc1 {
    template <typename X> static __device__ __forceinline__ X ld(const X* p) { return __hip_atomic_load(p, __ATOMIC_RELAXED, __HIP_MEMORY_SCOPE_AGENT); }
    template <typename X> static __device__ __forceinline__ void st(X* p, X v) { __hip_atomic_store(p, v, __ATOMIC_RELAXED, __HIP_MEMORY_SCOPE_AGENT); }
};


template <typename T, typename IO = IoPlain>
__device__ __forceinline__ void d_restrict(const MLevel& mf, const T* __restrict__ rf, const MLevel& mc, const uint8_t* __restrict__ cnt_c,
                                           T* __restrict__ fc, long t)
{
    int I, J, K;
    if (!mg_cell(mc, t, I, J, K)) return;
    const size_t C = mc.at(I, J, K);
    T out = 0;
    if (!cnt_c[C]) return;
    {
        auto w = [](int a) { return (a == 0 || a == 3) ? (T)0.25 : (T)0.75; };
        const int i0 = 2 * I - 1, j0 = 2 * J - 1, k0 = 2 * K - 1;
        T acc = 0;
        if (i0 >= 0 && i0 + 3 < mf.dx && j0 >= 0 && j0 + 3 < mf.dy && k0 >= 0 && k0 + 3 < mf.dz) {
            const T* p = rf + mf.at(i0, j0, k0);
#pragma unroll
            for (int a = 0; a < 4; ++a) {
#pragma unroll
                for (int b = 0; b < 4; ++b) {
                    const T* q = p + a * mf.sx + b * mf.sy;
                    acc += w(a) * w(b) * ((T)0.25 * (q[0] + q[3]) + (T)0.75 * (q[1] + q[2]));
                }
            }
        } else {
            for (int a = 0; a < 4; ++a) {
                const int i = i0 + a;
                if (i < 0 || i >= mf.dx) continue;
                for (int b = 0; b < 4; ++b) {
                    const int j = j0 + b;
                    if (j < 0 || j >= mf.dy) continue;
                    T row = 0;
#pragma unroll
                    for (int d = 0; d < 4; ++d) {
                        const int k = k0 + d;
                        if (k >= 0 && k < mf.dz) row += w(d) * rf[mf.at(i, j, k)];
                    }
                    acc += w(a) * w(b) * row;
                }
            }
        }
        out = acc * (T)0.125;
    }
    IO::st(fc + C, out);
}

template <int RY, int RZ>
__device__ __forceinline__ void region_cell(int t, int& x, int& y, int& z)
{
    x = t / (RY * RZ);
    const int r = t - x * (RY * RZ);
    y = r / RZ;
    z = r - y * RZ;
}
__device__ __forceinline__ bool in_level(const MLevel& m, int i, int j, int k)
{
    return (unsigned)i < (unsigned)m.dx && (unsigned)j < (unsigned)m.dy && (unsigned)k < (unsigned)m.dz;
}

__device__ __forceinline__ int clampi(int v, int hi) { return min(max(v, 0), hi); }

template <typename T, int TX, int TY, int TZ, bool RESTRICT>
struct DownTile {
    static constexpr int H = RESTRICT ? 3 : 2;
    static constexpr int AX = TX + 2 * H, AY = TY + 2 * H, AZ = TZ + 2 * H;
    static constexpr int BX = AX - 2, BY = AY - 2, BZ = AZ - 2;
    static constexpr int CX = BX - 2, CY = BY - 2, CZ = BZ - 2;
    static constexpr int nA = AX * AY * AZ, nB = BX * BY * BZ, nR = RESTRICT ? CX * CY * CZ : 4;
    static constexpr int oA = 0, oB = (oA + nA * (int)sizeof(T) + 15) / 16 * 16, oR = (oB + nB * (int)sizeof(T) + 15) / 16 * 16,
                         oC = (oR + nR * (int)sizeof(T) + 15) / 16 * 16, bytes = (oC + nA + 15) / 16 * 16;
};
// ... 289 lines not shown
    }
    __syncthreads();
    if (actB && (NG == 1 || xb0 < BX)) {
        const int a0 = (yb + 1) * AZ + zb + 1 + xb0 * AY * AZ;
        T cm = sA[a0], c0 = sA[a0 + AY * AZ];
#pragma unroll
        for (int p = 0; p < PB; ++p) {
            const int x = xb0 + p;
            if (NG == 1 || x < BX) {
                const int a = a0 + (p + 1) * AY * AZ;
                const T cp = sA[a + AY * AZ];
                const int n = sC[a];
                const T nb = cm + cp + sA[a - AZ] + sA[a + AZ] + sA[a - 1] + sA[a + 1];
                sB[(x * BY + yb) * BZ + zb] = c0 + (T)MG_W2 * si[n] * (fb[p] - (sd[n] * c0 + off * nb));
                cm = c0;
                c0 = cp;
            }
        }
    }
    __syncthreads();
    double acc = 0;
    if (NG == 1 || xt0 < TX) {
        const int b0 = ((xt0 + 1) * BY + yt + 1) * BZ + zt + 1;
        T cm = sB[b0 - BY * BZ], c0 = sB[b0];
#pragma unroll
        for (int x = 0; x < XT; ++x) {
            if (NG == 1 || xt0 + x < TX) {
                const int b = b0 + x * BY * BZ;
                const T cp = sB[b + BY * BZ];
                const int n = sC[((xt0 + x + 2) * AY + yt + 2) * AZ + zt + 2];
                const T nb = cm + cp + sB[b - BZ] + sB[b + BZ] + sB[b - 1] + sB[b + 1];
                const T o = c0 + (T)MG_W1 * si[n] * ((T)ft[x] - (sd[n] * c0 + off * nb));
                if (n && live) {
                    const size_t qo = qt + (size_t)((long)(i0 + xt0 + x) * sx);
                    IO::st(out + qo, (O)o);
                    if (!own || (own[qo] && !(own[qo] & 0x80))) acc += (double)ft[x] * (double)o;
                }
                cm = c0;
                c0 = cp;
            }
        }
    }
    if (NG == 1 && part_dot) {
        acc = block_sum<double, 4>(acc, red);
        if (threadIdx.x == 0) part_dot[blockIdx.x] = acc;
    }
}

template <typename T, typename F, typename O, int TX, int TY, int TZ>
__global__ __launch_bounds__(256, 5) void k_mg_up(MLevel m, const uint8_t* __restrict__ cnt, const F* __restrict__ f, const T* __restrict__ u,
                                                                      O* __restrict__ out, MLevel mc, const T* __restrict__ ec, MgCoef<T> cf,
                                                                      double* __restrict__ part_dot, const PcgState* ps, int gx, int gy, T wc,
                                                                      const int* __restrict__ tlist, const uint8_t* __restrict__ own, int pconst)
{
    __shared__ __attribute__((aligned(16))) char lds[UpTile<T, TX, TY, TZ>::bytes];
    __shared__ T sd[8], si[8];
    __shared__ double red[4];
    const int dn = vload(&ps->done);
    const int tile = tlist ? tlist[xcd_remap(blockIdx.x, gridDim.x)] : xcd_remap(blockIdx.x, gridDim.x);
    mg_up_body<T, F, O, TX, TY, TZ, IoPlain, 1>(m, cnt, f, u, out, mc, ec, &cf, cf.off, part_dot, tile, gx, gy, wc, own, true, (int)threadIdx.x, lds, sd, si, red, 0,
                                                pconst != 0, dn);
}

template <typename T>
__global__ __launch_bounds__(256) void k_mg_restrict(MLevel mf, const T* __restrict__ rf, MLevel mc, const uint8_t* __restrict__ cnt_c,
                                                     T* __restrict__ fc, const PcgState* ps)
{
    if (ps && ps->done) return;
    d_restrict<T>(mf, rf, mc, cnt_c, fc, (long)blockIdx.x * 256 + threadIdx.x);
}

constexpr int MG_TAIL_Q0 = 4;
template <typename T>
struct MgTail {
    int nl;
    MLevel mg[MG_TAIL_MAX];
    const uint8_t* cnt[MG_TAIL_MAX];
    const T* f0;
    T* u0;
    MLevel ml[MG_TAIL_MAX];
    int o_u[MG_TAIL_MAX], o_v[MG_TAIL_MAX], o_f[MG_TAIL_MAX], o_c[MG_TAIL_MAX];
    int lds_bytes;
    T off[MG_TAIL_MAX];
    int sweeps;
    double wc;
};

struct TailCell {
    int c;
    int n;
    int up;
    int down;
    int bits;
};
__device__ __forceinline__ TailCell tail_cell(const MLevel& m, bool has_coarser, const MLevel& coarser, bool has_finer, const MLevel& finer, int t)
{
    TailCell d;
    d.c = -1; d.n = 0; d.up = 0; d.down = 0; d.bits = 0;
    int i, j, k;
    if (mg_cell(m, t, i, j, k)) {
        d.c = (int)m.at(i, j, k);
        d.bits = (i & 1) | ((j & 1) << 1) | ((k & 1) << 2) | ((((i + j + k) & 1) == 0) << 3);
        if (has_coarser) d.up = (int)coarser.at(i >> 1, j >> 1, k >> 1);
        if (has_finer) d.down = (int)finer.at(2 * i - 1, 2 * j - 1, 2 * k - 1);
    }
    return d;
}
template <typename T>
__device__ __forceinline__ T tail_nb(const T* p, int c, int sx, int sy)
{
    return p[c - sx] + p[c + sx] + p[c - sy] + p[c + sy] + p[c - 1] + p[c + 1];
}

template <typename T, typename IO>
__device__ __forceinline__ void mg_tail_body(const MgTail<T>& a, double* tail_lds, T (*sd)[8], T (*si)[8], int tid)
{
    char* base = (char*)tail_lds;
#define TU(lv) ((T*)(base + a.o_u[lv]))
#define TV(lv) ((T*)(base + a.o_v[lv]))
#define TF(lv) ((T*)(base + a.o_f[lv]))
#define TC(lv) ((uint8_t*)(base + a.o_c[lv]))
    TailCell z[MG_TAIL_Q0];
    T zf[MG_TAIL_Q0];
    int zg[MG_TAIL_Q0];
#pragma unroll
    for (int q = 0; q < MG_TAIL_Q0; ++q) {
        z[q] = tail_cell(a.ml[0], a.nl > 1, a.ml[1], false, a.ml[0], tid + 1024 * q);
        zg[q] = 0;
        zf[q] = 0;
        if (z[q].c >= 0) {
            int i, j, k;
            mg_cell(a.mg[0], tid + 1024 * q, i, j, k);
            zg[q] = (int)a.mg[0].at(i, j, k);
            z[q].n = a.cnt[0][zg[q]];
            zf[q] = IO::ld(a.f0 + zg[q]);
        }
    }
    TailCell w[MG_TAIL_MAX];
#pragma unroll
    for (int l = 1; l < MG_TAIL_MAX; ++l) {
        w[l].c = -1; w[l].n = 0; w[l].up = 0; w[l].down = 0; w[l].bits = 0;
        if (l < a.nl) {
            w[l] = tail_cell(a.ml[l], l + 1 < a.nl, a.ml[l + 1 < MG_TAIL_MAX ? l + 1 : l], true, a.ml[l - 1], tid);
            if (w[l].c >= 0) {
                int i, j, k;
                mg_cell(a.mg[l], tid, i, j, k);
                w[l].n = a.cnt[l][a.mg[l].at(i, j, k)];
            }
        }
    }
    if (tid < a.nl * 8) {
        const int l = tid >> 3, n = tid & 7;
        T off = a.off[0];
#pragma unroll
        for (int q = 1; q < MG_TAIL_MAX; ++q) off = (l == q) ? a.off[q] : off;
        const T d = -off * (T)n;
        sd[l][n] = d;
        si[l][n] = n ? (T)1 / d : (T)0;
    }
    for (int q = tid; q < a.lds_bytes / 8; q += 1024) tail_lds[q] = 0;
    __syncthreads();
#pragma unroll
    for (int q = 0; q < MG_TAIL_Q0; ++q) {
        if (z[q].c >= 0) {
            TC(0)[z[q].c] = (uint8_t)z[q].n;
            TF(0)[z[q].c] = z[q].n ? zf[q] : (T)0;
        }
    }
#pragma unroll
    for (int l = 1; l < MG_TAIL_MAX; ++l)
        if (l < a.nl && w[l].c >= 0) TC(l)[w[l].c] = (uint8_t)w[l].n;
    __syncthreads();
    const T w1 = (T)MG_W1, w2 = (T)MG_W2;
#define OWN(lv, ...)                                                                   \
    do {                                                                               \
        if ((lv) == 0) {                                                               \
            _Pragma("unroll") for (int q_ = 0; q_ < MG_TAIL_Q0; ++q_) {                \
                const TailCell& cell = z[q_];                                          \
                if (cell.c >= 0) { __VA_ARGS__ }                                       \
            }                                                                          \
        } else {                                                                       \
            const TailCell& cell = w[(lv) ? (lv) : 1];                                 \
            if (cell.c >= 0) { __VA_ARGS__ }                                           \
        }                                                                              \
    } while (0)
#pragma unroll
    for (int l = 0; l < MG_TAIL_MAX - 1; ++l) {
        if (l < a.nl - 1) {
            const int sx = (int)a.ml[l].sx, sy = (int)a.ml[l].sy;
            T *U = TU(l), *V = TV(l), *F = TF(l);
            const T off = a.off[l];
            OWN(l, V[cell.c] = w1 * si[l][cell.n] * F[cell.c];);
            __syncthreads();
            OWN(l, const T v = V[cell.c]; U[cell.c] = v + w2 * si[l][cell.n] * (F[cell.c] - (sd[l][cell.n] * v + off * tail_nb(V, cell.c, sx, sy))););
            __syncthreads();
            OWN(l, V[cell.c] = cell.n ? F[cell.c] - (sd[l][cell.n] * U[cell.c] + off * tail_nb(U, cell.c, sx, sy)) : (T)0;);
            __syncthreads();
            {
                const TailCell& cc = w[l + 1];
                if (cc.c >= 0 && cc.n) {
                    auto wt = [](int q) { return (q == 0 || q == 3) ? (T)0.25 : (T)0.75; };
                    const T* p = V + cc.down;
                    T acc = 0;
#pragma unroll
                    for (int x = 0; x < 4; ++x) {
#pragma unroll
                        for (int y = 0; y < 4; ++y) {
                            const T* q = p + x * sx + y * sy;
                            acc += wt(x) * wt(y) * ((T)0.25 * (q[0] + q[3]) + (T)0.75 * (q[1] + q[2]));
                        }
                    }
                    TF(l + 1)[cc.c] = acc * (T)0.125;
                }
            }
            __syncthreads();
        }
    }
#pragma unroll
    for (int lc = 0; lc < MG_TAIL_MAX; ++lc) {
        if (lc == a.nl - 1) {
            const TailCell& cell = lc == 0 ? z[0] : w[lc ? lc : 1];
            T* su = TU(lc);
            const int sx = (int)a.ml[lc].sx, sy = (int)a.ml[lc].sy;
            const bool mine = cell.c >= 0 && cell.n;
            const bool isred = (cell.bits & 8) != 0;
            const T fv = mine ? TF(lc)[cell.c] : (T)0, inv = si[lc][cell.n], off = a.off[lc];
            for (int s = 0; s < 2 * a.sweeps; ++s) {
                const bool fwd = s < a.sweeps;
#pragma unroll
                for (int h = 0; h < 2; ++h) {
                    const bool col = fwd ? (h == 0) : (h == 1);
                    if (mine && isred == col) su[cell.c] = (fv - off * tail_nb(su, cell.c, sx, sy)) * inv;
                    __syncthreads();
                }
            }
        }
    }
#pragma unroll
    for (int l = MG_TAIL_MAX - 2; l >= 0; --l) {
        if (l < a.nl - 1) {
            const int sx = (int)a.ml[l].sx, sy = (int)a.ml[l].sy;
            const int cx = (int)a.ml[l + 1].sx, cy = (int)a.ml[l + 1].sy;
            T *U = TU(l), *V = TV(l), *F = TF(l);
            const T* E = TU(l + 1);
            const T off = a.off[l];
            OWN(l, {
                const int ex = (cell.bits & 1) ? cx : -cx, ey = (cell.bits & 2) ? cy : -cy, ez = (cell.bits & 4) ? 1 : -1;
                const T* e = E + cell.up;
                const T p = (T)0.75, m = (T)0.25;
                const T pe = p * p * p * e[0] + p * p * m * (e[ex] + e[ey] + e[ez]) + p * m * m * (e[ex + ey] + e[ex + ez] + e[ey + ez]) +
                             m * m * m * e[ex + ey + ez];
                if (cell.n) U[cell.c] += (T)a.wc * pe;
            });
            __syncthreads();
            OWN(l, const T v = U[cell.c]; V[cell.c] = v + w2 * si[l][cell.n] * (F[cell.c] - (sd[l][cell.n] * v + off * tail_nb(U, cell.c, sx, sy))););
            __syncthreads();
            OWN(l, const T v = V[cell.c]; U[cell.c] = v + w1 * si[l][cell.n] * (F[cell.c] - (sd[l][cell.n] * v + off * tail_nb(V, cell.c, sx, sy))););
            __syncthreads();
        }
    }
#pragma unroll
    for (int q = 0; q < MG_TAIL_Q0; ++q)
        if (z[q].c >= 0 && z[q].n) IO::st(a.u0 + zg[q], TU(0)[z[q].c]);
#undef OWN
#undef TU
#undef TV
#undef TF
#undef TC
}

template <typename T>
__global__ __launch_bounds__(1024) void k_mg_tail(MgTail<T> a, const PcgState* ps)
{
    extern __shared__ double tail_lds[];
    __shared__ T sd[MG_TAIL_MAX][8], si[MG_TAIL_MAX][8];
    if (ps && ps->done) return;
    mg_tail_body<T, IoPlain>(a, tail_lds, sd, si, threadIdx.x);
}

static inline unsigned mg_blocks(const MLevel& m) { return (unsigned)(((long)m.dx * m.dy * m.dz + 255) / 256); }

MLevel mg_level0(const LBox& L)
{
    MLevel m;
    m.dx = L.nx + 2; m.dy = L.ny + 2; m.dz = L.nz + 2;
    m.sx = (long)L.Ly * L.Lz; m.sy = L.Lz;
    m.ox = 0; m.oy = 0; m.oz = LBOX_K0 - 1;
    m.cells = L.cells() + 2 * (size_t)L.Lz;
    return m;
}
MLevel mg_coarser(const MLevel& f)
{
    MLevel m;
    m.dx = (f.dx + 1) / 2; m.dy = (f.dy + 1) / 2; m.dz = (f.dz + 1) / 2;
    const int Lz = (16 + m.dz + 1 + 15) / 16 * 16;
    m.sy = Lz; m.sx = (long)(m.dy + 2) * Lz;
    m.ox = 1; m.oy = 1; m.oz = 16;
    m.cells = (size_t)(m.dx + 2) * m.sx + Lz;
    return m;
}

void launch_mg_type0(hipStream_t st, Grid g, LBox L, MLevel m, const uint8_t* flags, const uint8_t* cnt, uint8_t* typ)
{
    hipLaunchKernelGGL(k_mg_type0, dim3(mg_blocks(m)), dim3(256), 0, st, g, L, m, flags, cnt, typ);
}
void launch_mg_coarsen_types(hipStream_t st, MLevel mf, const uint8_t* tf, MLevel mc, uint8_t* tc)
{
    if (mg_blocks(mc)) hipLaunchKernelGGL(k_mg_coarsen, dim3(mg_blocks(mc)), dim3(256), 0, st, mf, tf, mc, tc);
}
void launch_mg_counts(hipStream_t st, MLevel m, const uint8_t* typ, uint8_t* cnt)
{
    if (mg_blocks(m)) hipLaunchKernelGGL(k_mg_cnt, dim3(mg_blocks(m)), dim3(256), 0, st, m, typ, cnt);
}
void launch_mg_coarsen(hipStream_t st, MLevel mf, const uint8_t* tf, MLevel mc, uint8_t* tc, uint8_t* cnt_c)
{
    hipLaunchKernelGGL(k_mg_coarsen, dim3(mg_blocks(mc)), dim3(256), 0, st, mf, tf, mc, tc);
    hipLaunchKernelGGL(k_mg_cnt, dim3(mg_blocks(mc)), dim3(256), 0, st, mc, (const uint8_t*)tc, cnt_c);
}
template <typename T>
void launch_mg_restrict(hipStream_t st, MLevel mf, const T* rf, MLevel mc, const uint8_t* cnt_c, T* fc, const PcgState* ps)
{
    if (mg_blocks(mc)) hipLaunchKernelGGL((k_mg_restrict<T>), dim3(mg_blocks(mc)), dim3(256), 0, st, mf, rf, mc, cnt_c, fc, ps);
}
constexpr int MG_TX = 8, MG_TY = 8, MG_TZ = 16;
constexpr int MG_RX = 8, MG_RY = 8, MG_RZ = 8;
constexpr unsigned MG_FEW_TILES = 384;
template <int TX, int TY, int TZ>
__global__ __launch_bounds__(256) void k_mg_tile_flags(MLevel m, const uint8_t* __restrict__ cnt, int gx, int gy, uint8_t* __restrict__ flags)
{
    const int tile = blockIdx.x;
    const int tbx = tile % gx, tby = (tile / gx) % gy, tbz = tile / (gx * gy);
    const int i0 = tbz * TX, j0 = tby * TY, k0 = tbx * TZ;
    int any = 0;
    for (int t = threadIdx.x; t < TX * TY * TZ; t += 256) {
        const int z = t % TZ, y = (t / TZ) % TY, x = t / (TZ * TY);
        const int i = i0 + x, j = j0 + y, k = k0 + z;
        if (i < m.dx && j < m.dy && k < m.dz) any |= cnt[m.at(i, j, k)];
    }
    any = __syncthreads_or(any);
    if (threadIdx.x == 0) flags[tile] = any != 0;
}

static inline bool mg_ng4() { return true; }
static inline dim3 mg_tiles(const MLevel& m, int tx, int ty, int tz)
{
    return dim3((unsigned)((m.dz + tz - 1) / tz), (unsigned)((m.dy + ty - 1) / ty), (unsigned)((m.dx + tx - 1) / tx));
}
int mg_up_blocks(const MLevel& m)
{
    const dim3 g = mg_tiles(m, MG_TX, MG_TY, MG_TZ);
    return (int)(g.x * g.y * g.z);
}
template <typename T, typename F>
void launch_mg_down(hipStream_t st, MLevel m, const uint8_t* cnt, const F* f, T* u, T* r, MLevel mc, const uint8_t* cnt_c, T* fc, MgCoef<T> cf,
                    const PcgState* ps, const int* tlist, int nlist, bool pcr)
{
    if (m.dx <= 0 || m.dy <= 0 || m.dz <= 0) return;
    if (fc && !pcr) {
        const dim3 g = mg_tiles(m, MG_RX, MG_RY, MG_RZ);
        if (sizeof(F) == sizeof(T) && g.x * g.y * g.z <= MG_FEW_TILES && mg_ng4())
            hipLaunchKernelGGL((k_mg_down<T, F, MG_RX, MG_RY, MG_RZ, true, 4>), dim3(g.x * g.y * g.z), dim3(1024), 0, st, m, cnt, f, u, r, mc, cnt_c, fc, cf,
                               ps, (int)g.x, (int)g.y, (const int*)nullptr);
        else
            hipLaunchKernelGGL((k_mg_down<T, F, MG_RX, MG_RY, MG_RZ, true>), dim3(g.x * g.y * g.z), dim3(256), 0, st, m, cnt, f, u, r, mc, cnt_c, fc, cf,
                               ps, (int)g.x, (int)g.y, (const int*)nullptr);
    } else {
        const dim3 g = mg_tiles(m, MG_TX, MG_TY, MG_TZ);
        hipLaunchKernelGGL((k_mg_down<T, F, MG_TX, MG_TY, MG_TZ, false>), dim3(tlist ? (unsigned)nlist : g.x * g.y * g.z), dim3(256), 0, st, m, cnt, f, u,
                           r, mc, cnt_c, fc, cf, ps, (int)g.x, (int)g.y, tlist);
    }
}
template <typename T, typename F, typename O>
void launch_mg_up(hipStream_t st, MLevel m, const uint8_t* cnt, const F* f, const T* u, O* out, MLevel mc, const T* ec, MgCoef<T> cf,
                  double* part_dot, const PcgState* ps, double wc, const int* tlist, int nlist, const uint8_t* own, int pconst)
{
    const dim3 g = mg_tiles(m, MG_TX, MG_TY, MG_TZ);
    if (!tlist && g.x * g.y * g.z == 0) return;
    hipLaunchKernelGGL((k_mg_up<T, F, O, MG_TX, MG_TY, MG_TZ>), dim3(tlist ? (unsigned)nlist : g.x * g.y * g.z), dim3(256), 0, st, m, cnt, f, u, out, mc,
                       ec, cf, part_dot, ps, (int)g.x, (int)g.y, (T)wc, tlist, own, pconst);
}
void launch_mg_tile_flags(hipStream_t st, MLevel m, const uint8_t* cnt, uint8_t* flags)
{
    const dim3 g = mg_tiles(m, MG_TX, MG_TY, MG_TZ);
    hipLaunchKernelGGL((k_mg_tile_flags<MG_TX, MG_TY, MG_TZ>), dim3(g.x * g.y * g.z), dim3(256), 0, st, m, cnt, (int)g.x, (int)g.y, flags);
}

static MLevel tail_lds_level(const MLevel& g)
{
    MLevel m;
    m.dx = g.dx; m.dy = g.dy; m.dz = g.dz;
    m.sy = g.dz + 3; m.sx = (long)(g.dy + 3) * (g.dz + 3);
    m.ox = m.oy = m.oz = 1;
    m.cells = (size_t)(g.dx + 3) * m.sx;
    return m;
}
size_t mg_tail_lds_bytes(int nl, const MLevel* lv, size_t elem)
{
    size_t total = 0;
    for (int l = 0; l < nl; ++l) {
        const long cells = (long)lv[l].dx * lv[l].dy * lv[l].dz;
        if (cells > (l == 0 ? 1024L * MG_TAIL_Q0 : 1024L)) return 0;
        const size_t c = tail_lds_level(lv[l]).cells;
        total += 3 * ((c * elem + 15) / 16 * 16) + (c + 15) / 16 * 16;
    }
    return total;
}
template <typename T>
static MgTail<T> make_mg_tail(int nl, const T* f0, const MLevel* lv, uint8_t* const* cnt, T* u0, const T* off, int sweeps, double wc)
{
    MgTail<T> a;
    a.wc = wc;
    a.nl = nl;
    a.f0 = f0; a.u0 = u0;
    size_t o = 0;
    auto take = [&](size_t bytes) { const size_t at = o; o += (bytes + 15) / 16 * 16; return (int)at; };
    for (int l = 0; l < MG_TAIL_MAX; ++l) {
        const int q = l < nl ? l : nl - 1;
        a.mg[l] = lv[q]; a.cnt[l] = cnt[q]; a.off[l] = off[q];
        a.ml[l] = tail_lds_level(lv[q]);
        if (l < nl) {
            const size_t c = a.ml[l].cells;
            a.o_u[l] = take(c * sizeof(T)); a.o_v[l] = take(c * sizeof(T)); a.o_f[l] = take(c * sizeof(T)); a.o_c[l] = take(c);
        } else {
            a.o_u[l] = a.o_u[q]; a.o_v[l] = a.o_v[q]; a.o_f[l] = a.o_f[q]; a.o_c[l] = a.o_c[q];
        }
    }
    a.lds_bytes = (int)o;
    a.sweeps = sweeps;
    return a;
}
template <typename T>
void launch_mg_tail(hipStream_t st, int nl, const T* f0, const MLevel* lv, uint8_t* const* cnt, T* u0, const T* off, int sweeps, const PcgState* ps,
                    double wc)
{
    const MgTail<T> a = make_mg_tail<T>(nl, f0, lv, cnt, u0, off, sweeps, wc);
    static bool attr_set = false;
    if (!attr_set) {
        hipFuncSetAttribute((const void*)k_mg_tail<T>, hipFuncAttributeMaxDynamicSharedMemorySize, (int)MG_TAIL_LDS);
        attr_set = true;
    }
    hipLaunchKernelGGL((k_mg_tail<T>), dim3(1), dim3(1024), (size_t)a.lds_bytes, st, a, ps);
}

#define INSTMG(T)                                                                                                                        \
    template void launch_mg_down<T, T>(hipStream_t, MLevel, const uint8_t*, const T*, T*, T*, MLevel, const uint8_t*, T*, MgCoef<T>, const PcgState*, \
                                       const int*, int, bool); \
    template void launch_mg_up<T, T, T>(hipStream_t, MLevel, const uint8_t*, const T*, const T*, T*, MLevel, const T*, MgCoef<T>, double*,  \
                                        const PcgState*, double, const int*, int, const uint8_t*, int);                                                                          \
    template void launch_mg_restrict<T>(hipStream_t, MLevel, const T*, MLevel, const uint8_t*, T*, const PcgState*);                     \
    template void launch_mg_tail<T>(hipStream_t, int, const T*, const MLevel*, uint8_t* const*, T*, const T*, int, const PcgState*, double);
INSTMG(double)
INSTMG(float)
template void launch_mg_down<float, double>(hipStream_t, MLevel, const uint8_t*, const double*, float*, float*, MLevel, const uint8_t*, float*,
                                            MgCoef<float>, const PcgState*, const int*, int, bool);
template void launch_mg_up<float, double, double>(hipStream_t, MLevel, const uint8_t*, const double*, const float*, double*, MLevel, const float*,
                                                  MgCoef<float>, double*, const PcgState*, double, const int*, int, const uint8_t*, int);
template void launch_mg_up<float, double, float>(hipStream_t, MLevel, const uint8_t*, const double*, const float*, float*, MLevel, const float*,
                                                  MgCoef<float>, double*, const PcgState*, double, const int*, int, const uint8_t*, int);

}
```

fluid-simulation_amd/csrc/kernels_particles.hip:

```cpp
#include "common.h"

namespace fl {

struct BinAcc {
    int mn[3] = {0x7fffffff, 0x7fffffff, 0x7fffffff}, mx[3] = {-1, -1, -1};
    int nout = 0, cmax = 0;
};
__device__ __forceinline__ void bin_one(const Grid& g, long ncell, long i, double px, double py, double pz, bool dead, int* __restrict__ key,
                                        int* __restrict__ slot, int* __restrict__ cell_count, BinAcc& acc)
{
    int bx = (int)round(px) - g.cx0(), by = (int)round(py) - g.cy0(), bz = (int)round(pz) - g.cz0();
    bool in = bx >= 0 && bx < g.nx && by >= 0 && by < g.ny && bz >= 0 && bz < g.nz;
    int k = in ? (int)g.idx(bx, by, bz) : (int)ncell;
    if (dead) { k = (int)ncell + 1; in = false; }
    key[i] = k;
    {
        const int lane = threadIdx.x & 63;
        const int kp = __shfl_up(k, 1, 64);
        const bool head = lane == 0 || kp != k;
        const unsigned long long hm = __ballot(head);
        const unsigned long long below = hm & ((2ull << lane) - 1ull);
        const int start = 63 - __clzll((long long)below);
        const unsigned long long above = (lane == 63) ? 0ull : (hm >> (lane + 1)) << (lane + 1);
        const unsigned long long act = __ballot(true);
// ... 665 lines not shown
                sw_ = ((sw_ + w0) + W[1]) + w2;
            }
        }
    }
    if (!live) return;
    if (wf > 0) {
        const double wd = (double)wf;
        su /= wd; sv_ /= wd; sw_ /= wd;
    }
    container[c] = wf;
    u[c] = su; v[c] = sv_; w[c] = sw_;
    ub[c] = su; vb[c] = sv_; wb[c] = sw_;
}

__global__ __launch_bounds__(256) void k_g2p(Grid g, long n, Particles p, const double* __restrict__ dcx, const double* __restrict__ dcy,
                                             const double* __restrict__ dcz, const double* __restrict__ pcx, const double* __restrict__ pcy,
                                             const double* __restrict__ pcz, double blend, StepState* ss)
{
    __shared__ double sm[4];
    long i = (long)blockIdx.x * 256 + threadIdx.x;
    double len = 0;
    if (i < n && p.pid[i] != PID_DEAD) {
        const double cx = p.px[i], cy = p.py[i], cz = p.pz[i];
        const int wlo = g.lo + 2, whi = g.hi - 2;
        const int fcx = (int)round(cx), fcy = (int)round(cy), fcz = (int)round(cz);
        double wx[3], wy[3], wz[3];
        int ox[3], oy[3], oz[3];
        const int sxs = (int)g.sx();
#pragma unroll
        for (int d = 0; d < 3; ++d) {
            const int ax = fcx - 1 + d, ay = fcy - 1 + d, az = fcz - 1 + d;
            wx[d] = (ax >= wlo && ax <= whi) ? spline_at(cx, ax, d) : 0.0;
            wy[d] = (ay >= wlo && ay <= whi) ? spline_at(cy, ay, d) : 0.0;
            wz[d] = (az >= wlo && az <= whi) ? spline_at(cz, az, d) : 0.0;
            ox[d] = (min(max(ax, g.cx0()), g.cx1()) - g.cx0()) * sxs;
            oy[d] = (min(max(ay, g.cy0()), g.cy1()) - g.cy0()) * g.nz;
            oz[d] = min(max(az, g.cz0()), g.cz1()) - g.cz0();
        }
        double weight = 0, d0 = 0, d1 = 0, d2 = 0, q0 = 0, q1 = 0, q2 = 0;
#pragma unroll
        for (int xi = 0; xi < 3; ++xi)
#pragma unroll
            for (int yi = 0; yi < 3; ++yi)
#pragma unroll
                for (int zi = 0; zi < 3; ++zi) {
                    const int c = ox[xi] + oy[yi] + oz[zi];
                    const double cw = wx[xi] * wy[yi] * wz[zi];
                    weight += cw;
                    d0 += dcx[c] * cw;
                    d1 += dcy[c] * cw;
                    d2 += dcz[c] * cw;
                    if (pcx) {
                        q0 += pcx[c] * cw;
                        q1 += pcy[c] * cw;
                        q2 += pcz[c] * cw;
                    }
                }
        double vx = p.vx[i], vy = p.vy[i], vz = p.vz[i];
        if (weight != 0) {
            vx += d0 / weight;
            vy += d1 / weight;
            vz += d2 / weight;
            if (pcx) {
                vx = blend * vx + (1.0 - blend) * (q0 / weight);
                vy = blend * vy + (1.0 - blend) * (q1 / weight);
                vz = blend * vz + (1.0 - blend) * (q2 / weight);
            }
            p.vx[i] = vx; p.vy[i] = vy; p.vz[i] = vz;
        }
        len = sqrt(vx * vx + vy * vy + vz * vz);
        if (!(len == len)) len = 0;
    }
    len = wave_max(len);
    if ((threadIdx.x & 63) == 0) sm[threadIdx.x >> 6] = len;
    __syncthreads();
    if (threadIdx.x == 0) {
        double m = sm[0];
        for (int k = 1; k < 4; ++k) m = sm[k] > m ? sm[k] : m;
        if (m > 0) atomicMax(&ss->max_speed_bits, (unsigned long long)__double_as_longlong(m));
    }
}

constexpr int G2P_TX = 4, G2P_TY = 4, G2P_TZ = 30;
template <bool PIC>
__global__ __launch_bounds__(256) void k_g2p_tiled(Grid g, Box pb, Particles p, const int* __restrict__ cell_start,
                                                   const double* __restrict__ dcx, const double* __restrict__ dcy,
                                                   const double* __restrict__ dcz, const double* __restrict__ pcx,
                                                   const double* __restrict__ pcy, const double* __restrict__ pcz, double blend, StepState* ss)
{
    constexpr int LX = G2P_TX + 2, LY = G2P_TY + 2, LZ = G2P_TZ + 2, LN = LX * LY * LZ, NROW = G2P_TX * G2P_TY;
    __shared__ double sf[PIC ? 6 : 3][LN];
    __shared__ int srow[NROW][2];
    __shared__ double sm[4];
    const int tid = threadIdx.x;
    const int nty = (pb.ny() + G2P_TY - 1) / G2P_TY, ntz = (pb.nz() + G2P_TZ - 1) / G2P_TZ;
    const int tile = blockIdx.x;
    const int tz = tile % ntz, ty = (tile / ntz) % nty, tx = tile / (ntz * nty);
    const int x0 = pb.x0 + tx * G2P_TX, y0 = pb.y0 + ty * G2P_TY, z0 = pb.z0 + tz * G2P_TZ;
    const int z1 = z0 + G2P_TZ - 1 < pb.z1 ? z0 + G2P_TZ - 1 : pb.z1;
    if (tid < NROW) {
        const int cx = x0 + tid / G2P_TY, cy = y0 + tid % G2P_TY;
        int a = 0, b = 0;
        if (cx <= pb.x1 && cy <= pb.y1) {
            a = cell_start[g.idx(cx, cy, z0)];
            b = cell_start[g.idx(cx, cy, z1) + 1];
        }
        srow[tid][0] = a;
        srow[tid][1] = b;
    }
    for (int t = tid; t < LN; t += 256) {
        const int lx = t / (LY * LZ), r = t - lx * (LY * LZ), ly = r / LZ, lz = r - ly * LZ;
        const int gx = x0 - 1 + lx, gy = y0 - 1 + ly, gz = z0 - 1 + lz;
        const bool in = gx >= 0 && gx < g.nx && gy >= 0 && gy < g.ny && gz >= 0 && gz < g.nz;
        const size_t c = in ? g.idx(gx, gy, gz) : 0;
        sf[0][t] = in ? dcx[c] : 0.0;
        sf[1][t] = in ? dcy[c] : 0.0;
        sf[2][t] = in ? dcz[c] : 0.0;
        if (PIC) {
            sf[PIC ? 3 : 0][t] = in ? pcx[c] : 0.0;
            sf[PIC ? 4 : 0][t] = in ? pcy[c] : 0.0;
            sf[PIC ? 5 : 0][t] = in ? pcz[c] : 0.0;
        }
    }
    __syncthreads();
    const int wlo = g.lo + 2, whi = g.hi - 2;
    double len = 0;
    for (int row = 0; row < NROW; ++row) {
        const int a = srow[row][0], b = srow[row][1];
        for (int i = a + tid; i < b; i += 256) {
            const double cx = p.px[i], cy = p.py[i], cz = p.pz[i];
            const int fcx = (int)round(cx), fcy = (int)round(cy), fcz = (int)round(cz);
            double wx[3], wy[3], wz[3];
#pragma unroll
            for (int d = 0; d < 3; ++d) {
                const int ax = fcx - 1 + d, ay = fcy - 1 + d, az = fcz - 1 + d;
                wx[d] = (ax >= wlo && ax <= whi) ? spline_at(cx, ax, d) : 0.0;
                wy[d] = (ay >= wlo && ay <= whi) ? spline_at(cy, ay, d) : 0.0;
                wz[d] = (az >= wlo && az <= whi) ? spline_at(cz, az, d) : 0.0;
            }
            const int lb = ((fcx - g.cx0() - x0) * LY + (fcy - g.cy0() - y0)) * LZ + (fcz - g.cz0() - z0);
            double weight = 0, d0 = 0, d1 = 0, d2 = 0, q0 = 0, q1 = 0, q2 = 0;
#pragma unroll
            for (int xi = 0; xi < 3; ++xi)
#pragma unroll
                for (int yi = 0; yi < 3; ++yi)
#pragma unroll
                    for (int zi = 0; zi < 3; ++zi) {
                        const int c = lb + (xi * LY + yi) * LZ + zi;
                        const double cw = wx[xi] * wy[yi] * wz[zi];
                        weight += cw;
                        d0 += sf[0][c] * cw;
                        d1 += sf[1][c] * cw;
                        d2 += sf[2][c] * cw;
                        if (PIC) {
                            q0 += sf[PIC ? 3 : 0][c] * cw;
                            q1 += sf[PIC ? 4 : 0][c] * cw;
                            q2 += sf[PIC ? 5 : 0][c] * cw;
                        }
                    }
            double vx = p.vx[i], vy = p.vy[i], vz = p.vz[i];
            if (weight != 0) {
                vx += d0 / weight;
                vy += d1 / weight;
                vz += d2 / weight;
                if (PIC) {
                    vx = blend * vx + (1.0 - blend) * (q0 / weight);
                    vy = blend * vy + (1.0 - blend) * (q1 / weight);
                    vz = blend * vz + (1.0 - blend) * (q2 / weight);
                }
                p.vx[i] = vx; p.vy[i] = vy; p.vz[i] = vz;
            }
            double l = sqrt(vx * vx + vy * vy + vz * vz);
            if (!(l == l)) l = 0;
            len = l > len ? l : len;
        }
    }
    len = wave_max(len);
    if ((tid & 63) == 0) sm[tid >> 6] = len;
    __syncthreads();
    if (tid == 0) {
        double m = sm[0];
        for (int k = 1; k < 4; ++k) m = sm[k] > m ? sm[k] : m;
        if (m > 0) atomicMax(&ss->max_speed_bits, (unsigned long long)__double_as_longlong(m));
    }
}

__device__ __forceinline__ bool is_solid(const Grid& g, const uint8_t* flags, int x, int y, int z)
{
    if (x < g.cx0() || x > g.cx1() || y < g.cy0() || y > g.cy1() || z < g.cz0() || z > g.cz1()) return false;
    return flags[g.idx(x - g.cx0(), y - g.cy0(), z - g.cz0())] & F_SOLID;
}

__device__ __forceinline__ double advect_timestep(double max_dt, double dx, const StepState* ss)
{
    const double maxSpeed = __longlong_as_double((long long)ss->max_speed_bits);
    if (maxSpeed != 0) return max_dt < dx / maxSpeed ? max_dt : dx / maxSpeed;
    return max_dt;
}
__device__ __forceinline__ void advect_one(const Grid& g, const Particles& p, const uint8_t* __restrict__ flags, double timestep, long i, double& P0,
                                           double& P1, double& P2)
// ... 118 lines not shown
    hipLaunchKernelGGL(k_bin_bbox, dim3(1), dim3(256), 0, st, (const int*)part, (int)nb, ss);
}
void launch_bin_scatter(hipStream_t st, long n, const int* key, const int* slot, const int* cell_start, const uint32_t* pid, int* order,
                         uint32_t* spid)
{
    if (n > 0) hipLaunchKernelGGL(k_bin_scatter, dim3(nblk(n)), dim3(256), 0, st, n, key, slot, cell_start, pid, order, spid);
}
void launch_bin_rank(hipStream_t st, long n_pos, long pos0, const int* key, const int* cell_start, const int* order, const uint32_t* spid,
                     int* order2)
{
    if (n_pos > 0) hipLaunchKernelGGL(k_bin_rank, dim3(nblk(n_pos)), dim3(256), 0, st, n_pos, pos0, key, cell_start, order, spid, order2);
}
void launch_reorder(hipStream_t st, long n, const int* order, Particles src, Particles dst, double* w, long wstride)
{
    if (n > 0) hipLaunchKernelGGL(k_reorder, dim3(nblk(n)), dim3(256), 0, st, n, order, src, dst, w, wstride);
}
void launch_weights(hipStream_t st, long n, Particles p, double* w, long stride)
{
    if (n > 0) hipLaunchKernelGGL(k_weights, dim3(nblk(n)), dim3(256), 0, st, n, p, w, stride);
}
static void p2g_cut(const Box& box, int& ntz, int& zt, int& nseg)
{
    ntz = (box.nz() + P2G_ZT - 1) / P2G_ZT;
    zt = (box.nz() + ntz - 1) / ntz;
    nseg = 1;
    long best = -1;
    const long per = (long)(box.nx() + 2) * ntz;
    for (int k = 1; k <= box.ny(); ++k) {
        const long ys = (box.ny() + k - 1) / k, rounds = (per * k + P2G_SLOTS - 1) / P2G_SLOTS, cost = rounds * (ys + 2);
        if (best < 0 || cost < best) { best = cost; nseg = k; }
    }
}
size_t p2g_part_doubles(Box box)
{
    int ntz, zt, nseg;
    p2g_cut(box, ntz, zt, nseg);
    return (size_t)12 * box.cells() + ((size_t)3 * box.nx() * box.ny() * ntz + 7) / 8 + 8;
}
long p2g_max_items(Box box)
{
    int ntz, zt, nseg;
    p2g_cut(box, ntz, zt, nseg);
    return (long)(box.nx() + 2) * box.ny() * ntz;
}
void launch_p2g(hipStream_t st, Grid g, Box box, Particles p, const double* pw, long wstride, const int* cell_start, const uint8_t* flags,
                double* part, int* items, float* container, double* u, double* v, double* w, double* ub, double* vb, double* wb, int2* crowd_list,
                Particles park)
{
    int ntz, zt, nseg;
    p2g_cut(box, ntz, zt, nseg);
    const long cells = box.cells();
    const int budget = P2G_BUDGET;
    const unsigned nt = (unsigned)((box.nx() + 2) * nseg * ntz);
    hipLaunchKernelGGL(k_p2g_items, dim3(nblk((long)(box.nx() + 2) * nseg)), dim3(256), 0, st, g, box, cell_start, nseg, ntz, budget, items);
    const bool vec = ((((uintptr_t)pw | (uintptr_t)p.vx | (uintptr_t)p.vy | (uintptr_t)p.vz) & 15) == 0) && (wstride & 1) == 0;
    uint8_t* colflag = reinterpret_cast<uint8_t*>(part + 12 * cells);
    if (crowd_list) {
        Box sb = box;
        sb.x0 = sb.x0 > 0 ? sb.x0 - 1 : 0, sb.y0 = sb.y0 > 0 ? sb.y0 - 1 : 0, sb.z0 = sb.z0 > 0 ? sb.z0 - 1 : 0;
        sb.x1 = sb.x1 < g.nx - 1 ? sb.x1 + 1 : g.nx - 1, sb.y1 = sb.y1 < g.ny - 1 ? sb.y1 + 1 : g.ny - 1, sb.z1 = sb.z1 < g.nz - 1 ? sb.z1 + 1 : g.nz - 1;
        hipLaunchKernelGGL(k_p2g_crowd_list, dim3(nblk((long)sb.nx() * sb.ny() * ((sb.nz() + 3) / 4))), dim3(256), 0, st, g, sb, cell_start, crowd_list, items + 1);
        hipLaunchKernelGGL(k_p2g_crowd_sum, dim3(2048), dim3(64 * PC_WAVES), 0, st, p, pw, wstride, crowd_list, items + 1, park);
        if (vec) hipLaunchKernelGGL((k_p2g_rows<true, true>), dim3(nt), dim3(P2G_THREADS), 0, st, g, box, p, pw, wstride, cell_start, part, cells, zt, items, park, colflag, ntz);
        else hipLaunchKernelGGL((k_p2g_rows<false, true>), dim3(nt), dim3(P2G_THREADS), 0, st, g, box, p, pw, wstride, cell_start, part, cells, zt, items, park, colflag, ntz);
    } else if (vec) hipLaunchKernelGGL((k_p2g_rows<true, false>), dim3(nt), dim3(P2G_THREADS), 0, st, g, box, p, pw, wstride, cell_start, part, cells, zt, items, park, colflag, ntz);
    else hipLaunchKernelGGL((k_p2g_rows<false, false>), dim3(nt), dim3(P2G_THREADS), 0, st, g, box, p, pw, wstride, cell_start, part, cells, zt, items, park, colflag, ntz);
    hipLaunchKernelGGL(k_p2g_combine, dim3(nblk(cells)), dim3(256), 0, st, g, box, part, cells, flags, container, u, v, w, ub, vb, wb, items, colflag, zt, ntz);
}
void launch_p2g_tiles(hipStream_t st, Grid g, Box box, Particles p, const double* pw, long wstride, const int* cell_start, const uint8_t* flags,
                      float* container, double* u, double* v, double* w, double* ub, double* vb, double* wb)
{
    const int ntz = (box.nz() + P2G_ZT - 1) / P2G_ZT, zt = (box.nz() + ntz - 1) / ntz;
    const unsigned nt = (unsigned)(((box.nx() + P2GT_T - 1) / P2GT_T) * ((box.ny() + P2GT_T - 1) / P2GT_T) * ntz);
    hipLaunchKernelGGL(k_p2g_tiles, dim3(nt), dim3(P2GT_THREADS), 0, st, g, box, p, pw, wstride, cell_start, flags, container, u, v, w, ub, vb, wb, zt);
}
void launch_g2p_tiled(hipStream_t st, Grid g, Box pb, Particles p, const int* cell_start, const double* dcx, const double* dcy, const double* dcz,
                      const double* pcx, const double* pcy, const double* pcz, double blend, StepState* ss)
{
    if (pb.cells() <= 0) return;
    const unsigned nt = (unsigned)(((pb.nx() + G2P_TX - 1) / G2P_TX) * ((pb.ny() + G2P_TY - 1) / G2P_TY) * ((pb.nz() + G2P_TZ - 1) / G2P_TZ));
    if (pcx) hipLaunchKernelGGL(k_g2p_tiled<true>, dim3(nt), dim3(256), 0, st, g, pb, p, cell_start, dcx, dcy, dcz, pcx, pcy, pcz, blend, ss);
    else hipLaunchKernelGGL(k_g2p_tiled<false>, dim3(nt), dim3(256), 0, st, g, pb, p, cell_start, dcx, dcy, dcz, pcx, pcy, pcz, blend, ss);
}
void launch_g2p(hipStream_t st, Grid g, long n, Particles p, const double* dcx, const double* dcy, const double* dcz, const double* pcx,
                const double* pcy, const double* pcz, double blend, StepState* ss)
{
    if (n > 0) hipLaunchKernelGGL(k_g2p, dim3(nblk(n)), dim3(256), 0, st, g, n, p, dcx, dcy, dcz, pcx, pcy, pcz, blend, ss);
}
void launch_advect(hipStream_t st, Grid g, long n, Particles p, const uint8_t* flags, double max_dt, double dx, StepState* ss)
{
    if (n > 0) hipLaunchKernelGGL(k_advect, dim3(nblk(n)), dim3(256), 0, st, g, n, p, flags, max_dt, dx, ss);
    hipLaunchKernelGGL(k_publish_dt, dim3(1), dim3(1), 0, st, max_dt, dx, ss, (const int*)nullptr, 0);
}
void launch_advect_bin(hipStream_t st, Grid g, long n, Particles p, const uint8_t* flags, double max_dt, double dx, StepState* ss, int* key,
                       int* slot, int* cell_count, int* part)
{
    unsigned nb = nblk(n);
    if (nb > 1024) nb = 1024;
    hipLaunchKernelGGL(k_advect_bin, dim3(nb), dim3(256), 0, st, g, n, p, flags, max_dt, dx, ss, key, slot, cell_count, part);
    hipLaunchKernelGGL(k_publish_dt, dim3(1), dim3(256), 0, st, max_dt, dx, ss, (const int*)part, (int)nb);
}
void launch_unpack_records(hipStream_t st, long n, const double* rec, Particles p, long off)
{
    if (n > 0) hipLaunchKernelGGL(k_unpack_records, dim3(nblk(n)), dim3(256), 0, st, n, rec, p, off);
}
void launch_pack_records(hipStream_t st, long n, Particles p, long off, double* rec)
{
    if (n > 0) hipLaunchKernelGGL(k_pack_records, dim3(nblk(n)), dim3(256), 0, st, n, p, off, rec);
}
void launch_unpack_ids(hipStream_t st, long n, const double* pos, const double* vel, const uint32_t* ids, Particles p)
{
    if (n > 0) hipLaunchKernelGGL(k_unpack_ids, dim3(nblk(n)), dim3(256), 0, st, n, pos, vel, ids, p);
}
void launch_pack_ids(hipStream_t st, long n, Particles p, long off, double* pos, double* vel, uint32_t* ids)
{
    if (n > 0) hipLaunchKernelGGL(k_pack_ids, dim3(nblk(n)), dim3(256), 0, st, n, p, off, pos, vel, ids);
}
void launch_pack_particles(hipStream_t st, long n, Particles p, double* pos_aos, double* vel_aos)
{
    if (n > 0) hipLaunchKernelGGL(k_pack, dim3(nblk(n)), dim3(256), 0, st, n, p, pos_aos, vel_aos);
}
void launch_unpack_particles(hipStream_t st, long n, const double* pos_aos, const double* vel_aos, Particles p)
{
    if (n > 0) hipLaunchKernelGGL(k_unpack, dim3(nblk(n)), dim3(256), 0, st, n, pos_aos, vel_aos, p);
}

}
```

fluid-simulation_amd/csrc/sim.h:

```cpp
#pragma once
#include "common.h"
#include "../../include/fluid_hip.h"

#include <cmath>
#include <cstdio>
#include <cstdlib>
#include <cstring>
#include <string>
#include <utility>
#include <vector>

int fluid_fail(int code, const std::string& msg);
#define HIPCHK(expr)                                                                                              \
    do {                                                                                                          \
        hipError_t e_ = (expr);                                                                                   \
        if (e_ != hipSuccess)                                                                                     \
            return fluid_fail(FLUID_ERR_HIP, std::string(#expr) + ": " + hipGetErrorString(e_) + " @" + std::to_string(__LINE__)); \
    } while (0)
#include "snap_ring.h"

using namespace fl;

struct ProfClass {
    long launches = 0, sampled = 0;
// ... 16 lines not shown
    double* p_guess2 = nullptr;
    long guess_step = -1, guess2_step = -1;
    int guess_pass = -1, guess2_pass = -1;
    long step_counter = 0;
    bool extrapolate = true;
    double* p_q = nullptr;
    long q_step = -1;
    void start_guess(const double*& g1, const double*& g2, double& ca, double& cb) const
    {
        g1 = p_guess, g2 = nullptr, ca = 1.0, cb = 0.0;
        const int k = stats.outer_passes;
        const bool same_step = p_guess2 && k >= 2 && guess_step == step_counter && guess2_step == step_counter && guess_pass == k - 1 && guess2_pass == k - 2;
        const double f = 1.0 - prm.update_frac;
        if (extrapolate && same_step) {
            g2 = p_guess2, ca = 1.0 + f, cb = -f;
        } else if (extrapolate && p_q && q_step >= 0 && step_counter - q_step <= 4 && k == 1 && guess_step == step_counter && guess_pass == 0) {
            g2 = p_q, ca = f, cb = 1.0;
        }
    }
    bool make_q() const { return warm && p_q && stats.outer_passes == 1 && guess_step == step_counter && guess_pass == 1 && guess2_step == step_counter && guess2_pass == 0; }
    void rotate_guess()
    {
        std::swap(p_guess, p_guess2);
        guess2_step = guess_step, guess2_pass = guess_pass;
        guess_step = step_counter, guess_pass = stats.outer_passes;
    }
    int *indices = nullptr, *scan_sums = nullptr, *ipart = nullptr;
    void *R = nullptr, *S[2] = {nullptr, nullptr}, *Q = nullptr, *X = nullptr, *Zmg = nullptr;
    double *pcx = nullptr, *pcy = nullptr, *pcz = nullptr;
    uint8_t* cntL = nullptr;
    LBox L{};
    size_t lmax = 0;
    double *part_bb = nullptr, *part_rr = nullptr, *part_rz[2] = {nullptr, nullptr}, *part_pq = nullptr, *part_err = nullptr;
    PcgState* ps = nullptr;
    PcgState* h_ps = nullptr;
    hipEvent_t ev_poll[2] = {nullptr, nullptr};
    long np = 0, cap = 0;
    Particles pa{}, pb{};
    int *key = nullptr, *slot = nullptr, *order = nullptr, *order2 = nullptr, *cell_count = nullptr, *cell_start = nullptr;
    uint32_t* spid = nullptr;
    double *stage_pos = nullptr, *stage_vel = nullptr;
    double* pw = nullptr;
    double* p2g_part = nullptr;
    size_t p2g_part_cap = 0;
    int2* p2g_crowd = nullptr;
    size_t p2g_crowd_cap = 0;
    int* p2g_items = nullptr;
    size_t p2g_items_cap = 0;
    int max_cell = 0;
    uint8_t* tl_flags = nullptr;
    int *tl_mg = nullptr, *tl_sq = nullptr;
    size_t tl_cap = 0;
    int n_tl_mg = 0, n_tl_sq = 0;
    int *row_flags = nullptr, *row_pos = nullptr, *row_list = nullptr;
    size_t row_cap = 0;
    int n_rows = 0;
    bool rows_on = true;
    bool drops_on = true;
    bool row_sweeps = true;
    int* drop_ctr = nullptr;
    int* drop_n = nullptr;
    int* drop_cells = nullptr;
    int n_drop = 0;
    int drop_last = -1;
    int drop_min = 4000;
    int drop_skipped = 0;
    bool lists_hint = false;
    bool lists_on = false;
    int lists_force = -1;
    int p2g_force = 0;
    long p2g_ref_cells = 0;
    long last_num_active = 0;
    StepState* ss = nullptr;
    StepState* h_ss = nullptr;
    Box Pb{0, 0, 0, -1, -1, -1}, Rb{0, 0, 0, -1, -1, -1}, Sb{0, 0, 0, -1, -1, -1};
    Box dirty{0, 0, 0, -1, -1, -1};
    int flag_x0 = 0, flag_x1 = -1;
    bool flags_valid = false;
    bool sorted = false, have_p2g = false, have_flags = false;
    long n_out = 0;
    bool sort_hint = false;
    bool advect_bin = true;
    bool binned = false;
    int bin_x0 = 0, bin_x1 = -1;
    int bin_min[3] = {0, 0, 0}, bin_max[3] = {-1, -1, -1}, bin_n_out = 0, bin_max_cell = 0;
    bool solve_tail = true;
    bool tail_ran = false;
    double dt = 0.1;
    fluid_step_stats_t stats{};
    static constexpr int MG_MAXL = 8;
    int mg_nl = 0, mg_tail = 0;
    long mg_last_iters_k[3] = {0, 0, 0};
    int pass_class() const { return stats.outer_passes < 2 ? stats.outer_passes : 2; }
    int mg_csweeps = 3;
    MLevel mgl[MG_MAXL];
    uint8_t *mg_typ[MG_MAXL] = {}, *mg_cnt[MG_MAXL] = {};
    int gal_mode = 1;
    int gal_it[2] = {-1, -1};
    int gal_since_probe = 0;
    bool gal_eligible = false;
    bool gal = false;
    int gal_lc = 0;
    double gal_dt = 0;
    double gal_wc = 1.8;
    int gal_sweeps = 3;
    char* gal_slab = nullptr;
    size_t gal_slab_cap = 0;
    float* gal_c[MG_MAXL][4] = {};
    uint8_t* gal_cnt[MG_MAXL] = {};
    uint8_t* gal_tfl[MG_MAXL] = {};
    char *mg_u[MG_MAXL] = {}, *mg_v[MG_MAXL] = {}, *mg_f[MG_MAXL] = {}, *mg_r[MG_MAXL] = {};
    double mg_wc[4] = {1.25, 1.1, 1.0, 1.0};
    bool mg_fp32 = true;
    double* mg_part = nullptr;
    char* mg_slab = nullptr;
    size_t mg_slab_cap = 0;
    bool dist = false;
    struct DistState* ds = nullptr;
    long p_off = 0;
    int* d_small = nullptr;
    int* h_small = nullptr;
    struct SrcSlot {
        bool on = false;
        bool mask_ok = false;
        fluid_source_t src{};
        Box box{};
        int* buf = nullptr;
    };
    SrcSlot src[FLUID_MAX_SOURCES];
    Box sink[FLUID_MAX_SINKS] = {};
    bool sink_on[FLUID_MAX_SINKS] = {};
    int* src_sums = nullptr;
    long n_steps = 0;
    bool vel_ok = false;
    long src_emit_last = 0, src_rm_last = 0, src_emit_total = 0, src_rm_total = 0;
    struct OutState* out = nullptr;
    int out_every = 0;
    struct SdfState* sdf = nullptr;
    struct MeshState* mesh = nullptr;
    struct RenderState* render = nullptr;
    int prof_every = 0;
    ProfClass prof[FLUID_PROF_COUNT];
};

namespace fl {
inline bool box_empty(const Box& b) { return b.x1 < b.x0 || b.y1 < b.y0 || b.z1 < b.z0; }
Box clip_dilate(const Box& b, int d, const Grid& g);
template <typename T>
inline hipError_t dalloc(T** p, size_t n)
{
    hipError_t e = hipMalloc((void**)p, n * sizeof(T));
    if (e == hipSuccess) e = hipMemset(*p, 0, n * sizeof(T));
    return e;
}
template <typename T>
inline hipError_t regrow(T*& p, size_t n)
{
    if (p) hipFree(p);
    p = nullptr;
    return hipMalloc((void**)&p, n * sizeof(T));
}
inline int grid_leaves(const Grid& g) { return ((g.hi & ~7) - (g.lo & ~7)) / 8 + 1; }
inline int snap_guard(const fluid_sim* s, const char* why, bool want_dist = false)
{
    if (!s) return fluid_fail(FLUID_ERR_ARG, "null handle");
    return s->dist != want_dist ? fluid_fail(FLUID_ERR_STATE, why) : FLUID_OK;
}
constexpr const char* ATTR_SINGLE = "these surface attribute calls are single-GPU only: a decomposed handle gives a rank record with squared distances (fluid_dist_sdf_snapshot_attr) and the records merge on the host (fluid_sdf_attr_grids_merge)";
inline size_t solver_elem(const fluid_sim* s) { return s->prm.precision == FLUID_PRECISION_FP32 ? 4 : 8; }
inline bool use_mg(const fluid_sim* s) { return s->prm.preconditioner == FLUID_PRECOND_MG && s->prm.precision == FLUID_PRECISION_FP64; }

int prof_begin(fluid_sim* s, int k, double cells);
void prof_end(fluid_sim* s, int k, int tok);
int alloc_particles(fluid_sim* s, long n);
int grow_particles(fluid_sim* s, long need);
int read_ss(fluid_sim* s);
int sort_pass(fluid_sim* s, int ax0, int ax1, int* h_tail = nullptr);
int clear_dirty(fluid_sim* s);
int run_p2g(fluid_sim* s, const Box& box);
// ... 76 lines not shown
```

Baseline: 158.8.

## Fuse sort tail into scan, G2P delta, MG hierarchy build, tail reciprocals, down groups

Adds five default-on options. The sort-tail computation and tail-count zeroing move into the scan's block-sum kernel, and the flip-delta face-averaging moves into the tiled G2P tile load. The MG type and coarsening levels are built by a single hierarchy kernel, the MG tail uses precomputed reciprocal multipliers in place of integer divides, and the mixed-precision MG down-sweep can use a two-group 512-thread variant. The aim is fewer launches and less intermediate memory traffic. In exchange the G2P kernel reads six fields with neighbours per tile cell, and correctness depends on the tail_zero bookkeeping between sort and advect.

```diff
diff --git a/fluid-simulation_amd/csrc/common.h b/fluid-simulation_amd/csrc/common.h
--- a/fluid-simulation_amd/csrc/common.h
+++ b/fluid-simulation_amd/csrc/common.h
@@ -259,6 +259,8 @@
                       float* container, double* u, double* v, double* w, double* ub, double* vb, double* wb);
 void launch_g2p_tiled(hipStream_t st, Grid g, Box pb, Particles p, const int* cell_start, const double* dcx, const double* dcy, const double* dcz,
                       const double* pcx, const double* pcy, const double* pcz, double blend, StepState* ss);
+void launch_g2p_tiled_delta(hipStream_t st, Grid g, Box pb, Particles p, const int* cell_start, const double* u, const double* v, const double* w,
+                            const double* ub, const double* vb, const double* wb, StepState* ss);
 void launch_g2p(hipStream_t st, Grid g, long n, Particles p, const double* dcx, const double* dcy, const double* dcz, const double* pcx,
                 const double* pcy, const double* pcz, double blend, StepState* ss);
 void launch_advect(hipStream_t st, Grid g, long n, Particles p, const uint8_t* flags, double max_dt, double dx, StepState* ss);
@@ -330,6 +332,7 @@
 void launch_render(hipStream_t st, const RenderGeom& r, const fluid_camera& cam, const fluid_shade& sh, const float* tv, const int* flags,
                    unsigned char* neg, unsigned* occ, unsigned* hits, unsigned char* rgb, float* depth, float* normals);
 void launch_exclusive_scan(hipStream_t st, const int* in, int* out, long n, int* block_sums, int* total);
+void launch_exclusive_scan_tail(hipStream_t st, int* in, int* out, long n, int* block_sums, int* total, int* tail_cnt, int* tail_start);
 void launch_sort_tail(hipStream_t st, const int* cell_count, int* cell_start, long c1, long ncell);
 void launch_index_scan(hipStream_t st, Grid g, const uint8_t* flags, int* indices, int* block_sums, int* total);
 void launch_index_scan_flat(hipStream_t st, const uint8_t* flags, int* indices, long n, int* block_sums, int* total);
@@ -453,6 +456,8 @@
 MLevel mg_level0(const LBox& L);
 MLevel mg_coarser(const MLevel& f);
 void launch_mg_type0(hipStream_t st, Grid g, LBox L, MLevel m, const uint8_t* flags, const uint8_t* cnt, uint8_t* typ);
+void launch_mg_hierarchy(hipStream_t st, Grid g, LBox L, int nl, const MLevel* m, uint8_t* const* typ, uint8_t* const* cnt, const uint8_t* flags,
+                         const uint8_t* cnt0);
 void launch_mg_coarsen(hipStream_t st, MLevel mf, const uint8_t* tf, MLevel mc, uint8_t* tc, uint8_t* cnt_c);
 void launch_mg_coarsen_types(hipStream_t st, MLevel mf, const uint8_t* tf, MLevel mc, uint8_t* tc);
 void launch_mg_counts(hipStream_t st, MLevel m, const uint8_t* typ, uint8_t* cnt);
@@ -464,7 +469,8 @@
 int mg_up_blocks(const MLevel& m);
 template <typename T, typename F>
 void launch_mg_down(hipStream_t st, MLevel m, const uint8_t* cnt, const F* f, T* u, T* r, MLevel mc, const uint8_t* cnt_c, T* fc, MgCoef<T> cf,
-                    const PcgState* ps, const int* tlist = nullptr, int nlist = 0, bool pcr = false);
+                    const PcgState* ps, const int* tlist = nullptr, int nlist = 0, bool pcr = false,
+                    int groups = 1);
 template <typename T, typename F, typename O>
 void launch_mg_up(hipStream_t st, MLevel m, const uint8_t* cnt, const F* f, const T* u, O* out, MLevel mc, const T* ec, MgCoef<T> cf,
                   double* part_dot, const PcgState* ps, double wc, const int* tlist = nullptr, int nlist = 0, const uint8_t* own = nullptr,
@@ -487,6 +493,6 @@
 void launch_compact_flags(hipStream_t st, const uint8_t* flags, int n, int* list, int* count);
 template <typename T>
 void launch_mg_tail(hipStream_t st, int nl, const T* f0, const MLevel* lv, uint8_t* const* cnt, T* u0, const T* off, int sweeps, const PcgState* ps,
-                    double wc);
-
-}
+                    double wc, bool recip);
+
+}
diff --git a/fluid-simulation_amd/csrc/fluid_api.hip b/fluid-simulation_amd/csrc/fluid_api.hip
--- a/fluid-simulation_amd/csrc/fluid_api.hip
+++ b/fluid-simulation_amd/csrc/fluid_api.hip
@@ -230,6 +230,11 @@
     if (const char* e = getenv("FLUID_DROPLETS_MIN")) s->drop_min = atoi(e);
     if (const char* e = getenv("FLUID_ADVECT_BIN")) s->advect_bin = atoi(e) != 0;
     if (const char* e = getenv("FLUID_SOLVE_TAIL")) s->solve_tail = atoi(e) != 0;
+    if (const char* e = getenv("FLUID_SORT_FOLD")) s->sort_fold = atoi(e) != 0;
+    if (const char* e = getenv("FLUID_MG_FUSED")) s->mg_fused = atoi(e) != 0;
+    if (const char* e = getenv("FLUID_G2P_DELTA")) s->g2p_delta = atoi(e) != 0;
+    if (const char* e = getenv("FLUID_TAIL_RECIP")) s->tail_recip = atoi(e) != 0;
+    if (const char* e = getenv("FLUID_DOWN_NG2")) s->down_ng2 = atoi(e) != 0;
     *out = nullptr;
     auto bail = [&](int rc) { fluid_destroy(s); return rc; };
 #define A(expr) do { hipError_t e_ = (expr); if (e_ != hipSuccess) return bail(fail(FLUID_ERR_HIP, std::string(#expr) + ": " + hipGetErrorString(e_))); } while (0)
@@ -419,6 +424,19 @@
     return FLUID_OK;
 }
 
+static void sort_scan(fluid_sim* s, long c0, long c1)
+{
+    const long ncell = (long)s->ncell;
+    if (s->sort_fold) {
+        launch_exclusive_scan_tail(s->st, s->cell_count + c0, s->cell_start + c0, c1 - c0, s->scan_sums, s->cell_start + c1, s->cell_count + ncell,
+                                   s->cell_start + ncell);
+        s->tail_zero = true;
+    } else {
+        launch_exclusive_scan(s->st, s->cell_count + c0, s->cell_start + c0, c1 - c0, s->scan_sums, s->cell_start + c1);
+        launch_sort_tail(s->st, s->cell_count, s->cell_start, c1, ncell);
+    }
+}
+
 int fl::sort_pass(fluid_sim* s, int ax0, int ax1, int* h_tail)
 {
     const Grid g = s->g;
@@ -428,8 +446,7 @@
     HIPCHK(hipMemsetAsync(s->cell_count + c0, 0, (c1 - c0) * sizeof(int), s->st));
     HIPCHK(hipMemsetAsync(s->cell_count + ncell, 0, 4 * sizeof(int), s->st));
     launch_bin_count(s->st, g, s->np, s->pa.shifted(s->p_off), s->key, s->slot, s->cell_count, s->ipart, s->ss);
-    launch_exclusive_scan(s->st, s->cell_count + c0, s->cell_start + c0, c1 - c0, s->scan_sums, s->cell_start + c1);
-    launch_sort_tail(s->st, s->cell_count, s->cell_start, c1, ncell);
+    sort_scan(s, c0, c1);
     launch_bin_scatter(s->st, s->np, s->key, s->slot, s->cell_start, s->pa.shifted(s->p_off).pid, s->order, s->spid);
     launch_bin_rank(s->st, s->np, 0, s->key, s->cell_start, s->order, s->spid, s->order2);
     HIPCHK(hipGetLastError());
@@ -440,11 +457,10 @@
 static int sort_binned(fluid_sim* s)
 {
     const Grid g = s->g;
-    const long ncell = (long)s->ncell, n2 = g.sx();
+    const long n2 = g.sx();
     const long c0 = (long)s->bin_x0 * n2, c1 = (long)(s->bin_x1 + 1) * n2;
     launch_zero_step_state(s->st, s->ss, g.N);
-    launch_exclusive_scan(s->st, s->cell_count + c0, s->cell_start + c0, c1 - c0, s->scan_sums, s->cell_start + c1);
-    launch_sort_tail(s->st, s->cell_count, s->cell_start, c1, ncell);
+    sort_scan(s, c0, c1);
     launch_bin_scatter(s->st, s->np, s->key, s->slot, s->cell_start, s->pa.shifted(s->p_off).pid, s->order, s->spid);
     launch_bin_rank(s->st, s->np, 0, s->key, s->cell_start, s->order, s->spid, s->order2);
     HIPCHK(hipGetLastError());
@@ -643,8 +659,12 @@
     }
     s->Zmg = s->mg_slab + o_z;
     HIPCHK(hipMemsetAsync(s->mg_slab, 0, total, s->st));
-    launch_mg_type0(s->st, s->g, s->L, s->mgl[0], s->flags, s->cntL, s->mg_typ[0]);
-    for (int l = 1; l < nl; ++l) launch_mg_coarsen(s->st, s->mgl[l - 1], s->mg_typ[l - 1], s->mgl[l], s->mg_typ[l], s->mg_cnt[l]);
+    if (s->mg_fused) {
+        launch_mg_hierarchy(s->st, s->g, s->L, nl, s->mgl, s->mg_typ, s->mg_cnt, s->flags, s->cntL);
+    } else {
+        launch_mg_type0(s->st, s->g, s->L, s->mgl[0], s->flags, s->cntL, s->mg_typ[0]);
+        for (int l = 1; l < nl; ++l) launch_mg_coarsen(s->st, s->mgl[l - 1], s->mg_typ[l - 1], s->mgl[l], s->mg_typ[l], s->mg_cnt[l]);
+    }
     { int rcg = gal_build(s); if (rcg) return rcg; }
     HIPCHK(hipGetLastError());
     return FLUID_OK;
@@ -738,7 +758,7 @@
     auto F = [&](int l) { return (V*)s->mg_f[l]; };
     auto C = [&](int l, int q) { return (const float*)s->gal_c[l][q]; };
     const MLevel& m0 = s->mgl[0];
-    launch_mg_down<V, double>(s->st, m0, s->cntL, rhs0, U(0), (V*)s->mg_r[0], s->mgl[1], nullptr, F(1), mg_coef_as<V>(s, 0), ps, s->tl_mg, s->n_tl_mg, true);
+    launch_mg_down<V, double>(s->st, m0, s->cntL, rhs0, U(0), (V*)s->mg_r[0], s->mgl[1], nullptr, F(1), mg_coef_as<V>(s, 0), ps, s->tl_mg, s->n_tl_mg, true, s->down_ng2 ? 2 : 1);
     for (int l = 1; l < lc; ++l) launch_gal_down(s->st, s->mgl[l], s->gal_tfl[l], C(l, 0), C(l, 1), C(l, 2), C(l, 3), F(l), U(l), s->mgl[l + 1], F(l + 1), ps);
     launch_gal_coarsest(s->st, s->mgl[lc], C(lc, 0), C(lc, 1), C(lc, 2), C(lc, 3), F(lc), U(lc), s->gal_sweeps, ps);
     for (int l = lc - 1; l >= 1; --l)
@@ -767,14 +787,14 @@
         V* fc = fold ? F(l + 1) : nullptr;
         const uint8_t* cc = fold ? s->mg_cnt[l + 1] : nullptr;
         const bool lst = s->lists_on && !fold;
-        if (l == 0) launch_mg_down<V, double>(s->st, m, s->cntL, rhs0, U(0), R(0), s->mgl[1], cc, fc, mg_coef_as<V>(s, 0), ps, lst ? s->tl_mg : nullptr, s->n_tl_mg);
+        if (l == 0) launch_mg_down<V, double>(s->st, m, s->cntL, rhs0, U(0), R(0), s->mgl[1], cc, fc, mg_coef_as<V>(s, 0), ps, lst ? s->tl_mg : nullptr, s->n_tl_mg, false, s->down_ng2 ? 2 : 1);
         else launch_mg_down<V, V>(s->st, m, s->mg_cnt[l], (const V*)F(l), U(l), R(l), s->mgl[l + 1], cc, fc, mg_coef_as<V>(s, l), ps);
         if (!fold) launch_mg_restrict<V>(s->st, m, (const V*)R(l), s->mgl[l + 1], s->mg_cnt[l + 1], F(l + 1), ps);
     }
     {
         V off[fluid_sim::MG_MAXL];
         for (int l = tail; l < nl; ++l) off[l] = (V)mg_coef(s, l).off;
-        launch_mg_tail<V>(s->st, nl - tail, (const V*)F(tail), s->mgl + tail, s->mg_cnt + tail, U(tail), off + tail, s->mg_csweeps, ps, s->mg_wc[3]);
+        launch_mg_tail<V>(s->st, nl - tail, (const V*)F(tail), s->mgl + tail, s->mg_cnt + tail, U(tail), off + tail, s->mg_csweeps, ps, s->mg_wc[3], s->tail_recip);
     }
     for (int l = tail - 1; l >= 0; --l) {
         const MLevel& m = s->mgl[l];
@@ -1165,10 +1185,14 @@
     HIPCHK(hipSetDevice(s->prm.device));
     int rcp = pic_fields(s);
     if (rcp) return rcp;
-    if (!box_empty(s->Rb)) launch_flip_delta(s->st, s->g, s->Rb, s->u, s->v, s->w, s->ub, s->vb, s->wb, s->dcx, s->dcy, s->dcz, s->pcx, s->pcy, s->pcz);
+    const bool tiled = s->sorted && s->p_off == 0 && (double)s->np >= 4.0 * (double)s->Pb.cells();
+    const bool fused = tiled && s->g2p_delta && !s->pcx;
+    if (!box_empty(s->Rb) && !fused)
+        launch_flip_delta(s->st, s->g, s->Rb, s->u, s->v, s->w, s->ub, s->vb, s->wb, s->dcx, s->dcy, s->dcz, s->pcx, s->pcy, s->pcz);
     int tok = prof_begin(s, FLUID_PROF_G2P, (double)s->np);
-    if (s->sorted && s->p_off == 0 && (double)s->np >= 4.0 * (double)s->Pb.cells()) {
-        launch_g2p_tiled(s->st, s->g, s->Pb, s->pa, s->cell_start, s->dcx, s->dcy, s->dcz, s->pcx, s->pcy, s->pcz, s->prm.flip_blend, s->ss);
+    if (tiled) {
+        if (fused) launch_g2p_tiled_delta(s->st, s->g, s->Pb, s->pa, s->cell_start, s->u, s->v, s->w, s->ub, s->vb, s->wb, s->ss);
+        else launch_g2p_tiled(s->st, s->g, s->Pb, s->pa, s->cell_start, s->dcx, s->dcy, s->dcz, s->pcx, s->pcy, s->pcz, s->prm.flip_blend, s->ss);
         if (!box_empty(s->Pb)) s->stats.paths |= FLUID_PATH_G2P_TILES;
         if (s->n_out > 0)
             launch_g2p(s->st, s->g, s->n_out, s->pa.shifted(s->np - s->n_out), s->dcx, s->dcy, s->dcz, s->pcx, s->pcy, s->pcz, s->prm.flip_blend, s->ss);
@@ -1184,7 +1208,8 @@
         s->bin_x1 = std::min(g.nx - 1, s->Pb.x1 + 3);
         const long n2 = g.sx(), c0 = (long)s->bin_x0 * n2, c1 = (long)(s->bin_x1 + 1) * n2;
         HIPCHK(hipMemsetAsync(s->cell_count + c0, 0, (c1 - c0) * sizeof(int), s->st));
-        HIPCHK(hipMemsetAsync(s->cell_count + s->ncell, 0, 4 * sizeof(int), s->st));
+        if (!s->tail_zero) HIPCHK(hipMemsetAsync(s->cell_count + s->ncell, 0, 4 * sizeof(int), s->st));
+        s->tail_zero = false;
         launch_advect_bin(s->st, g, s->np, s->pa.shifted(s->p_off), s->flags, s->prm.max_dt, s->prm.dx, s->ss, s->key, s->slot, s->cell_count, s->ipart);
     } else {
         launch_advect(s->st, s->g, s->np, s->pa.shifted(s->p_off), s->flags, s->prm.max_dt, s->prm.dx, s->ss);
diff --git a/fluid-simulation_amd/csrc/fluid_dist.hip b/fluid-simulation_amd/csrc/fluid_dist.hip
--- a/fluid-simulation_amd/csrc/fluid_dist.hip
+++ b/fluid-simulation_amd/csrc/fluid_dist.hip
@@ -936,7 +936,7 @@
     {
         V off[fluid_sim::MG_MAXL];
         for (int l = tail; l < nl; ++l) off[l] = (V)mg_coef(s, l).off;
-        launch_mg_tail<V>(s->st, nl - tail, (const V*)F(tail), s->mgl + tail, s->mg_cnt + tail, U(tail), off + tail, s->mg_csweeps, ps, s->mg_wc[3]);
+        launch_mg_tail<V>(s->st, nl - tail, (const V*)F(tail), s->mgl + tail, s->mg_cnt + tail, U(tail), off + tail, s->mg_csweeps, ps, s->mg_wc[3], s->tail_recip);
     }
     for (int l = tail - 1; l >= split; --l) {
         const V* ec = l + 1 == tail ? U(l + 1) : W(l + 1);
diff --git a/fluid-simulation_amd/csrc/kernels_grid.hip b/fluid-simulation_amd/csrc/kernels_grid.hip
--- a/fluid-simulation_amd/csrc/kernels_grid.hip
+++ b/fluid-simulation_amd/csrc/kernels_grid.hip
@@ -49,10 +49,12 @@
     if (threadIdx.x == 0) block_sums[blockIdx.x] = s;
 }
 
-__global__ __launch_bounds__(1024) void k_scan_block_sums(int* __restrict__ block_sums, int nb, int* __restrict__ total)
+__global__ __launch_bounds__(1024) void k_scan_block_sums(int* __restrict__ block_sums, int nb, int* total, int* tail_cnt, int* tail_start)
 {
     __shared__ int wsum[16];
     __shared__ int carry_s;
+    int n_off = 0, n_dead = 0;
+    if (tail_cnt && threadIdx.x == 0) { n_off = tail_cnt[0]; n_dead = tail_cnt[1]; }
     if (threadIdx.x == 0) carry_s = 0;
     __syncthreads();
     const int lane = threadIdx.x & 63, w = threadIdx.x >> 6;
@@ -75,7 +77,16 @@
         if (threadIdx.x == 1023) carry_s = carry + woff + inc;
         __syncthreads();
     }
-    if (threadIdx.x == 0) *total = carry_s;
+    if (threadIdx.x == 0) {
+        const int t = carry_s;
+        *total = t;
+        if (tail_cnt) {
+            tail_start[0] = t;
+            tail_start[1] = t + n_off;
+            tail_start[2] = t + n_off + n_dead;
+            tail_cnt[0] = tail_cnt[1] = tail_cnt[2] = tail_cnt[3] = 0;
+        }
+    }
 }
 
 template <int MODE, bool VEC>
@@ -117,19 +128,20 @@
 }
 
 template <int MODE>
-static void scan_impl(hipStream_t st, const void* in, int* out, long n, int* block_sums, int* total)
+static void scan_impl(hipStream_t st, const void* in, int* out, long n, int* block_sums, int* total, int* tail_cnt = nullptr,
+                      int* tail_start = nullptr)
 {
     const int lead = MODE == 0 ? (int)(((uintptr_t)in & 15) / 4) : (int)((uintptr_t)in & 7);
     const bool vec = (((uintptr_t)out - (uintptr_t)4 * lead) & 15) == 0 && (MODE == 1 || ((uintptr_t)in & 3) == 0);
     if (vec) {
         const int nb = (int)((n + lead + SCAN_CHUNK - 1) / SCAN_CHUNK);
         hipLaunchKernelGGL((k_scan_sums<MODE, true>), dim3(nb), dim3(SCAN_T), 0, st, in, n, lead, block_sums);
-        hipLaunchKernelGGL(k_scan_block_sums, dim3(1), dim3(1024), 0, st, block_sums, nb, total);
+        hipLaunchKernelGGL(k_scan_block_sums, dim3(1), dim3(1024), 0, st, block_sums, nb, total, tail_cnt, tail_start);
         hipLaunchKernelGGL((k_scan_final<MODE, true>), dim3(nb), dim3(SCAN_T), 0, st, in, n, lead, (const int*)block_sums, out);
     } else {
         const int nb = (int)((n + SCAN_CHUNK - 1) / SCAN_CHUNK);
         hipLaunchKernelGGL((k_scan_sums<MODE, false>), dim3(nb), dim3(SCAN_T), 0, st, in, n, 0, block_sums);
-        hipLaunchKernelGGL(k_scan_block_sums, dim3(1), dim3(1024), 0, st, block_sums, nb, total);
+        hipLaunchKernelGGL(k_scan_block_sums, dim3(1), dim3(1024), 0, st, block_sums, nb, total, tail_cnt, tail_start);
         hipLaunchKernelGGL((k_scan_final<MODE, false>), dim3(nb), dim3(SCAN_T), 0, st, in, n, 0, (const int*)block_sums, out);
     }
 }
@@ -137,6 +149,10 @@
 void launch_exclusive_scan(hipStream_t st, const int* in, int* out, long n, int* block_sums, int* total)
 {
     scan_impl<0>(st, in, out, n, block_sums, total);
+}
+void launch_exclusive_scan_tail(hipStream_t st, int* in, int* out, long n, int* block_sums, int* total, int* tail_cnt, int* tail_start)
+{
+    scan_impl<0>(st, in, out, n, block_sums, total, tail_cnt, tail_start);
 }
 void launch_index_scan_flat(hipStream_t st, const uint8_t* flags, int* indices, long n, int* block_sums, int* total)
 {
diff --git a/fluid-simulation_amd/csrc/kernels_mg.hip b/fluid-simulation_amd/csrc/kernels_mg.hip
--- a/fluid-simulation_amd/csrc/kernels_mg.hip
+++ b/fluid-simulation_amd/csrc/kernels_mg.hip
@@ -73,6 +73,103 @@
         n = (typ[c - m.sx] != 0) + (typ[c + m.sx] != 0) + (typ[c - m.sy] != 0) + (typ[c + m.sy] != 0) + (typ[c - 1] != 0) + (typ[c + 1] != 0);
     }
     cnt[c] = n;
+}
+
+constexpr int MG_HB = 16;
+constexpr int MG_HL = 5;
+constexpr int MG_HT = 1024;
+struct MgTypes {
+    int nl;
+    MLevel m[MG_HL];
+    uint8_t* typ[MG_HL];
+};
+template <int LV>
+__device__ __forceinline__ void mg_brick_coarsen(const MgTypes& a, const uint8_t* sf, uint8_t* sc, int bx, int by, int bz, int tid)
+{
+    constexpr int E = MG_HB >> LV, F = 2 * E;
+    for (int t = tid; t < E * E * E; t += MG_HT) {
+        const int K = t % E, J = (t / E) % E, I = t / (E * E);
+        bool any_air = false, all_solid = true;
+#pragma unroll
+        for (int c = 0; c < 8; ++c) {
+            const int i = 2 * I + (c & 1), j = 2 * J + ((c >> 1) & 1), k = 2 * K + (c >> 2);
+            const uint8_t ty = sf[(i * F + j) * F + k];
+            any_air |= (ty == 1);
+            all_solid &= (ty == 0);
+        }
+        const uint8_t ty = any_air ? 1 : (all_solid ? 0 : 2);
+        sc[t] = ty;
+        const int gi = bx * E + I, gj = by * E + J, gk = bz * E + K;
+        if (gi < a.m[LV].dx && gj < a.m[LV].dy && gk < a.m[LV].dz) a.typ[LV][a.m[LV].at(gi, gj, gk)] = ty;
+    }
+}
+__global__ __launch_bounds__(MG_HT) void k_mg_types_all(Grid g, LBox L, MgTypes a, const uint8_t* __restrict__ flags, const uint8_t* __restrict__ cnt, int nby,
+                                                        int nbz)
+{
+    constexpr int Q = MG_HB * MG_HB * MG_HB / MG_HT;
+    __shared__ uint8_t s0[MG_HB * MG_HB * MG_HB], s1[512], s2[64], s3[8], s4[1];
+    const int tid = threadIdx.x;
+    const int bz = blockIdx.x % nbz, by = (blockIdx.x / nbz) % nby, bx = blockIdx.x / (nbz * nby);
+    bool dom[Q], grd[Q];
+    size_t c[Q];
+    uint8_t f[Q], n[Q];
+#pragma unroll
+    for (int q = 0; q < Q; ++q) {
+        const int t = tid + MG_HT * q;
+        const int i = bx * MG_HB + t / (MG_HB * MG_HB), j = by * MG_HB + (t / MG_HB) % MG_HB, k = bz * MG_HB + t % MG_HB;
+        const int gx = L.x0 + i - 1, gy = L.y0 + j - 1, gz = L.z0 + k - 1;
+        dom[q] = i < a.m[0].dx && j < a.m[0].dy && k < a.m[0].dz;
+        grd[q] = dom[q] && gx >= 0 && gx < g.nx && gy >= 0 && gy < g.ny && gz >= 0 && gz < g.nz;
+        c[q] = dom[q] ? a.m[0].at(i, j, k) : 0;
+        f[q] = flags[grd[q] ? g.idx(gx, gy, gz) : 0];
+        n[q] = cnt[c[q]];
+    }
+#pragma unroll
+    for (int q = 0; q < Q; ++q) {
+        uint8_t ty = 0;
+        if (grd[q]) ty = (f[q] & F_SOLID) ? 0 : (n[q] ? 2 : 1);
+        if (dom[q]) a.typ[0][c[q]] = ty;
+        s0[tid + MG_HT * q] = ty;
+    }
+    if (a.nl < 2) return;
+    __syncthreads();
+    mg_brick_coarsen<1>(a, s0, s1, bx, by, bz, tid);
+    if (a.nl < 3) return;
+    __syncthreads();
+    mg_brick_coarsen<2>(a, s1, s2, bx, by, bz, tid);
+    if (a.nl < 4) return;
+    __syncthreads();
+    mg_brick_coarsen<3>(a, s2, s3, bx, by, bz, tid);
+    if (a.nl < 5) return;
+    __syncthreads();
+    mg_brick_coarsen<4>(a, s3, s4, bx, by, bz, tid);
+}
+
+constexpr int MG_CL = 7;
+struct MgCounts {
+    int n;
+    int b0[MG_CL + 1];
+    MLevel m[MG_CL];
+    const uint8_t* typ[MG_CL];
+    uint8_t* cnt[MG_CL];
+};
+__device__ __forceinline__ void mg_cnt_cell(const MLevel& m, const uint8_t* __restrict__ typ, uint8_t* __restrict__ cnt, long t)
+{
+    int i, j, k;
+    if (!mg_cell(m, t, i, j, k)) return;
+    const size_t c = m.at(i, j, k);
+    uint8_t n = 0;
+    if (typ[c] == 2) {
+        n = (typ[c - m.sx] != 0) + (typ[c + m.sx] != 0) + (typ[c - m.sy] != 0) + (typ[c + m.sy] != 0) + (typ[c - 1] != 0) + (typ[c + 1] != 0);
+    }
+    cnt[c] = n;
+}
+__global__ __launch_bounds__(256) void k_mg_cnt_all(MgCounts a)
+{
+    const int b = blockIdx.x;
+#pragma unroll
+    for (int l = 0; l < MG_CL; ++l)
+        if (l < a.n && b >= a.b0[l] && b < a.b0[l + 1]) mg_cnt_cell(a.m[l], a.typ[l], a.cnt[l], (long)(b - a.b0[l]) * 256 + threadIdx.x);
 }
 
 
@@ -528,6 +625,7 @@
     int o_u[MG_TAIL_MAX], o_v[MG_TAIL_MAX], o_f[MG_TAIL_MAX], o_c[MG_TAIL_MAX];
     int lds_bytes;
     T off[MG_TAIL_MAX];
+    unsigned rz[MG_TAIL_MAX], ry[MG_TAIL_MAX];
     int sweeps;
     double wc;
 };
@@ -539,12 +637,27 @@
     int down;
     int bits;
 };
-__device__ __forceinline__ TailCell tail_cell(const MLevel& m, bool has_coarser, const MLevel& coarser, bool has_finer, const MLevel& finer, int t)
+template <bool FAST>
+__device__ __forceinline__ bool tail_ijk(const MLevel& m, unsigned rz, unsigned ry, int t, int& i, int& j, int& k)
+{
+    if (!FAST) return mg_cell(m, t, i, j, k);
+    const unsigned n = (unsigned)m.dx * (unsigned)m.dy * (unsigned)m.dz;
+    if ((unsigned)t >= n) return false;
+    const unsigned u = (unsigned)t;
+    const unsigned q = rz ? __umulhi(u, rz) : u;
+    k = (int)(u - q * (unsigned)m.dz);
+    const unsigned p = ry ? __umulhi(q, ry) : q;
+    j = (int)(q - p * (unsigned)m.dy);
+    i = (int)p;
+    return true;
+}
+template <bool FAST>
+__device__ __forceinline__ TailCell tail_cell(const MLevel& m, unsigned rz, unsigned ry, bool has_coarser, const MLevel& coarser, bool has_finer,
+                                              const MLevel& finer, int t, int& i, int& j, int& k)
 {
     TailCell d;
     d.c = -1; d.n = 0; d.up = 0; d.down = 0; d.bits = 0;
-    int i, j, k;
-    if (mg_cell(m, t, i, j, k)) {
+    if (tail_ijk<FAST>(m, rz, ry, t, i, j, k)) {
         d.c = (int)m.at(i, j, k);
         d.bits = (i & 1) | ((j & 1) << 1) | ((k & 1) << 2) | ((((i + j + k) & 1) == 0) << 3);
         if (has_coarser) d.up = (int)coarser.at(i >> 1, j >> 1, k >> 1);
@@ -558,7 +671,7 @@
     return p[c - sx] + p[c + sx] + p[c - sy] + p[c + sy] + p[c - 1] + p[c + 1];
 }
 
-template <typename T, typename IO>
+template <typename T, typename IO, bool FAST>
 __device__ __forceinline__ void mg_tail_body(const MgTail<T>& a, double* tail_lds, T (*sd)[8], T (*si)[8], int tid)
 {
     char* base = (char*)tail_lds;
@@ -571,12 +684,12 @@
     int zg[MG_TAIL_Q0];
 #pragma unroll
     for (int q = 0; q < MG_TAIL_Q0; ++q) {
-        z[q] = tail_cell(a.ml[0], a.nl > 1, a.ml[1], false, a.ml[0], tid + 1024 * q);
+        int i, j, k;
+        z[q] = tail_cell<FAST>(a.ml[0], a.rz[0], a.ry[0], a.nl > 1, a.ml[1], false, a.ml[0], tid + 1024 * q, i, j, k);
         zg[q] = 0;
         zf[q] = 0;
         if (z[q].c >= 0) {
-            int i, j, k;
-            mg_cell(a.mg[0], tid + 1024 * q, i, j, k);
+            if (!FAST) mg_cell(a.mg[0], tid + 1024 * q, i, j, k);
             zg[q] = (int)a.mg[0].at(i, j, k);
             z[q].n = a.cnt[0][zg[q]];
             zf[q] = IO::ld(a.f0 + zg[q]);
@@ -587,10 +700,10 @@
     for (int l = 1; l < MG_TAIL_MAX; ++l) {
         w[l].c = -1; w[l].n = 0; w[l].up = 0; w[l].down = 0; w[l].bits = 0;
         if (l < a.nl) {
-            w[l] = tail_cell(a.ml[l], l + 1 < a.nl, a.ml[l + 1 < MG_TAIL_MAX ? l + 1 : l], true, a.ml[l - 1], tid);
+            int i, j, k;
+            w[l] = tail_cell<FAST>(a.ml[l], a.rz[l], a.ry[l], l + 1 < a.nl, a.ml[l + 1 < MG_TAIL_MAX ? l + 1 : l], true, a.ml[l - 1], tid, i, j, k);
             if (w[l].c >= 0) {
-                int i, j, k;
-                mg_cell(a.mg[l], tid, i, j, k);
+                if (!FAST) mg_cell(a.mg[l], tid, i, j, k);
                 w[l].n = a.cnt[l][a.mg[l].at(i, j, k)];
             }
         }
@@ -715,13 +828,13 @@
 #undef TC
 }
 
-template <typename T>
+template <typename T, bool FAST>
 __global__ __launch_bounds__(1024) void k_mg_tail(MgTail<T> a, const PcgState* ps)
 {
     extern __shared__ double tail_lds[];
     __shared__ T sd[MG_TAIL_MAX][8], si[MG_TAIL_MAX][8];
     if (ps && ps->done) return;
-    mg_tail_body<T, IoPlain>(a, tail_lds, sd, si, threadIdx.x);
+    mg_tail_body<T, IoPlain, FAST>(a, tail_lds, sd, si, threadIdx.x);
 }
 
 static inline unsigned mg_blocks(const MLevel& m) { return (unsigned)(((long)m.dx * m.dy * m.dz + 255) / 256); }
@@ -763,6 +876,32 @@
     hipLaunchKernelGGL(k_mg_coarsen, dim3(mg_blocks(mc)), dim3(256), 0, st, mf, tf, mc, tc);
     hipLaunchKernelGGL(k_mg_cnt, dim3(mg_blocks(mc)), dim3(256), 0, st, mc, (const uint8_t*)tc, cnt_c);
 }
+void launch_mg_hierarchy(hipStream_t st, Grid g, LBox L, int nl, const MLevel* m, uint8_t* const* typ, uint8_t* const* cnt, const uint8_t* flags,
+                         const uint8_t* cnt0)
+{
+    MgTypes a;
+    a.nl = nl < MG_HL ? nl : MG_HL;
+    for (int l = 0; l < MG_HL; ++l) {
+        const int q = l < a.nl ? l : a.nl - 1;
+        a.m[l] = m[q]; a.typ[l] = typ[q];
+    }
+    const int nbx = (m[0].dx + MG_HB - 1) / MG_HB, nby = (m[0].dy + MG_HB - 1) / MG_HB, nbz = (m[0].dz + MG_HB - 1) / MG_HB;
+    hipLaunchKernelGGL(k_mg_types_all, dim3((unsigned)(nbx * nby * nbz)), dim3(MG_HT), 0, st, g, L, a, flags, cnt0, nby, nbz);
+    for (int l = MG_HL; l < nl; ++l) launch_mg_coarsen_types(st, m[l - 1], typ[l - 1], m[l], typ[l]);
+    if (nl < 2) return;
+    MgCounts c;
+    c.n = nl - 1 < MG_CL ? nl - 1 : MG_CL;
+    int b = 0;
+    for (int l = 0; l < MG_CL; ++l) {
+        const int q = l < c.n ? l + 1 : c.n;
+        c.m[l] = m[q]; c.typ[l] = typ[q]; c.cnt[l] = cnt[q];
+        c.b0[l] = b;
+        if (l < c.n) b += (int)mg_blocks(m[q]);
+    }
+    c.b0[MG_CL] = b;
+    for (int l = c.n; l < MG_CL; ++l) c.b0[l] = b;
+    if (b) hipLaunchKernelGGL(k_mg_cnt_all, dim3((unsigned)b), dim3(256), 0, st, c);
+}
 template <typename T>
 void launch_mg_restrict(hipStream_t st, MLevel mf, const T* rf, MLevel mc, const uint8_t* cnt_c, T* fc, const PcgState* ps)
 {
@@ -770,6 +909,7 @@
 }
 constexpr int MG_TX = 8, MG_TY = 8, MG_TZ = 16;
 constexpr int MG_RX = 8, MG_RY = 8, MG_RZ = 8;
+constexpr unsigned MG_ONE_ROUND_TILES = 1024;
 constexpr unsigned MG_FEW_TILES = 384;
 template <int TX, int TY, int TZ>
 __global__ __launch_bounds__(256) void k_mg_tile_flags(MLevel m, const uint8_t* __restrict__ cnt, int gx, int gy, uint8_t* __restrict__ flags)
@@ -799,7 +939,7 @@
 }
 template <typename T, typename F>
 void launch_mg_down(hipStream_t st, MLevel m, const uint8_t* cnt, const F* f, T* u, T* r, MLevel mc, const uint8_t* cnt_c, T* fc, MgCoef<T> cf,
-                    const PcgState* ps, const int* tlist, int nlist, bool pcr)
+                    const PcgState* ps, const int* tlist, int nlist, bool pcr, int groups)
 {
     if (m.dx <= 0 || m.dy <= 0 || m.dz <= 0) return;
     if (fc && !pcr) {
@@ -812,7 +952,15 @@
                                ps, (int)g.x, (int)g.y, (const int*)nullptr);
     } else {
         const dim3 g = mg_tiles(m, MG_TX, MG_TY, MG_TZ);
-        hipLaunchKernelGGL((k_mg_down<T, F, MG_TX, MG_TY, MG_TZ, false>), dim3(tlist ? (unsigned)nlist : g.x * g.y * g.z), dim3(256), 0, st, m, cnt, f, u,
+        const unsigned nt = tlist ? (unsigned)nlist : g.x * g.y * g.z;
+        if constexpr (sizeof(F) != sizeof(T)) {
+            if (groups == 2 && nt <= MG_ONE_ROUND_TILES) {
+                hipLaunchKernelGGL((k_mg_down<T, F, MG_TX, MG_TY, MG_TZ, false, 2>), dim3(nt), dim3(512), 0, st, m, cnt, f, u, r, mc, cnt_c, fc, cf, ps,
+                                   (int)g.x, (int)g.y, tlist);
+                return;
+            }
+        }
+        hipLaunchKernelGGL((k_mg_down<T, F, MG_TX, MG_TY, MG_TZ, false>), dim3(nt), dim3(256), 0, st, m, cnt, f, u,
                            r, mc, cnt_c, fc, cf, ps, (int)g.x, (int)g.y, tlist);
     }
 }
@@ -864,6 +1012,8 @@
         const int q = l < nl ? l : nl - 1;
         a.mg[l] = lv[q]; a.cnt[l] = cnt[q]; a.off[l] = off[q];
         a.ml[l] = tail_lds_level(lv[q]);
+        a.rz[l] = lv[q].dz > 1 ? (unsigned)((1ull << 32) / (unsigned)lv[q].dz) + 1u : 0u;
+        a.ry[l] = lv[q].dy > 1 ? (unsigned)((1ull << 32) / (unsigned)lv[q].dy) + 1u : 0u;
         if (l < nl) {
             const size_t c = a.ml[l].cells;
             a.o_u[l] = take(c * sizeof(T)); a.o_v[l] = take(c * sizeof(T)); a.o_f[l] = take(c * sizeof(T)); a.o_c[l] = take(c);
@@ -877,28 +1027,30 @@
 }
 template <typename T>
 void launch_mg_tail(hipStream_t st, int nl, const T* f0, const MLevel* lv, uint8_t* const* cnt, T* u0, const T* off, int sweeps, const PcgState* ps,
-                    double wc)
+                    double wc, bool recip)
 {
     const MgTail<T> a = make_mg_tail<T>(nl, f0, lv, cnt, u0, off, sweeps, wc);
     static bool attr_set = false;
     if (!attr_set) {
-        hipFuncSetAttribute((const void*)k_mg_tail<T>, hipFuncAttributeMaxDynamicSharedMemorySize, (int)MG_TAIL_LDS);
+        hipFuncSetAttribute((const void*)k_mg_tail<T, true>, hipFuncAttributeMaxDynamicSharedMemorySize, (int)MG_TAIL_LDS);
+        hipFuncSetAttribute((const void*)k_mg_tail<T, false>, hipFuncAttributeMaxDynamicSharedMemorySize, (int)MG_TAIL_LDS);
         attr_set = true;
     }
-    hipLaunchKernelGGL((k_mg_tail<T>), dim3(1), dim3(1024), (size_t)a.lds_bytes, st, a, ps);
+    if (recip) hipLaunchKernelGGL((k_mg_tail<T, true>), dim3(1), dim3(1024), (size_t)a.lds_bytes, st, a, ps);
+    else hipLaunchKernelGGL((k_mg_tail<T, false>), dim3(1), dim3(1024), (size_t)a.lds_bytes, st, a, ps);
 }
 
 #define INSTMG(T)                                                                                                                        \
     template void launch_mg_down<T, T>(hipStream_t, MLevel, const uint8_t*, const T*, T*, T*, MLevel, const uint8_t*, T*, MgCoef<T>, const PcgState*, \
-                                       const int*, int, bool); \
+                                       const int*, int, bool, int); \
     template void launch_mg_up<T, T, T>(hipStream_t, MLevel, const uint8_t*, const T*, const T*, T*, MLevel, const T*, MgCoef<T>, double*,  \
                                         const PcgState*, double, const int*, int, const uint8_t*, int);                                                                          \
     template void launch_mg_restrict<T>(hipStream_t, MLevel, const T*, MLevel, const uint8_t*, T*, const PcgState*);                     \
-    template void launch_mg_tail<T>(hipStream_t, int, const T*, const MLevel*, uint8_t* const*, T*, const T*, int, const PcgState*, double);
+    template void launch_mg_tail<T>(hipStream_t, int, const T*, const MLevel*, uint8_t* const*, T*, const T*, int, const PcgState*, double, bool);
 INSTMG(double)
 INSTMG(float)
 template void launch_mg_down<float, double>(hipStream_t, MLevel, const uint8_t*, const double*, float*, float*, MLevel, const uint8_t*, float*,
-                                            MgCoef<float>, const PcgState*, const int*, int, bool);
+                                            MgCoef<float>, const PcgState*, const int*, int, bool, int);
 template void launch_mg_up<float, double, double>(hipStream_t, MLevel, const uint8_t*, const double*, const float*, double*, MLevel, const float*,
                                                   MgCoef<float>, double*, const PcgState*, double, const int*, int, const uint8_t*, int);
 template void launch_mg_up<float, double, float>(hipStream_t, MLevel, const uint8_t*, const double*, const float*, float*, MLevel, const float*,
diff --git a/fluid-simulation_amd/csrc/kernels_particles.hip b/fluid-simulation_amd/csrc/kernels_particles.hip
--- a/fluid-simulation_amd/csrc/kernels_particles.hip
+++ b/fluid-simulation_amd/csrc/kernels_particles.hip
@@ -771,7 +771,7 @@
 }
 
 constexpr int G2P_TX = 4, G2P_TY = 4, G2P_TZ = 30;
-template <bool PIC>
+template <bool PIC, bool DELTA = false>
 __global__ __launch_bounds__(256) void k_g2p_tiled(Grid g, Box pb, Particles p, const int* __restrict__ cell_start,
                                                    const double* __restrict__ dcx, const double* __restrict__ dcy,
                                                    const double* __restrict__ dcz, const double* __restrict__ pcx,
@@ -802,9 +802,26 @@
         const int gx = x0 - 1 + lx, gy = y0 - 1 + ly, gz = z0 - 1 + lz;
         const bool in = gx >= 0 && gx < g.nx && gy >= 0 && gy < g.ny && gz >= 0 && gz < g.nz;
         const size_t c = in ? g.idx(gx, gy, gz) : 0;
-        sf[0][t] = in ? dcx[c] : 0.0;
-        sf[1][t] = in ? dcy[c] : 0.0;
-        sf[2][t] = in ? dcz[c] : 0.0;
+        if (DELTA) {
+            double d0 = 0.0, d1 = 0.0, d2 = 0.0;
+            if (in) {
+                const long sx = g.sx(), sy = g.nz;
+                const bool hxp = gx < g.nx - 1, hyp = gy < g.ny - 1, hzp = gz < g.nz - 1;
+                const double cu = (dcx[c] + (hxp ? dcx[c + sx] : 0.0)) / 2.0, pu = (pcx[c] + (hxp ? pcx[c + sx] : 0.0)) / 2.0;
+                const double cv = (dcy[c] + (hyp ? dcy[c + sy] : 0.0)) / 2.0, pv = (pcy[c] + (hyp ? pcy[c + sy] : 0.0)) / 2.0;
+                const double cw = (dcz[c] + (hzp ? dcz[c + 1] : 0.0)) / 2.0, pw = (pcz[c] + (hzp ? pcz[c + 1] : 0.0)) / 2.0;
+                d0 = cu - pu;
+                d1 = cv - pv;
+                d2 = cw - pw;
+            }
+            sf[0][t] = d0;
+            sf[1][t] = d1;
+            sf[2][t] = d2;
+        } else {
+            sf[0][t] = in ? dcx[c] : 0.0;
+            sf[1][t] = in ? dcy[c] : 0.0;
+            sf[2][t] = in ? dcz[c] : 0.0;
+        }
         if (PIC) {
             sf[PIC ? 3 : 0][t] = in ? pcx[c] : 0.0;
             sf[PIC ? 4 : 0][t] = in ? pcy[c] : 0.0;
@@ -1089,6 +1106,13 @@
     if (pcx) hipLaunchKernelGGL(k_g2p_tiled<true>, dim3(nt), dim3(256), 0, st, g, pb, p, cell_start, dcx, dcy, dcz, pcx, pcy, pcz, blend, ss);
     else hipLaunchKernelGGL(k_g2p_tiled<false>, dim3(nt), dim3(256), 0, st, g, pb, p, cell_start, dcx, dcy, dcz, pcx, pcy, pcz, blend, ss);
 }
+void launch_g2p_tiled_delta(hipStream_t st, Grid g, Box pb, Particles p, const int* cell_start, const double* u, const double* v, const double* w,
+                            const double* ub, const double* vb, const double* wb, StepState* ss)
+{
+    if (pb.cells() <= 0) return;
+    const unsigned nt = (unsigned)(((pb.nx() + G2P_TX - 1) / G2P_TX) * ((pb.ny() + G2P_TY - 1) / G2P_TY) * ((pb.nz() + G2P_TZ - 1) / G2P_TZ));
+    hipLaunchKernelGGL((k_g2p_tiled<false, true>), dim3(nt), dim3(256), 0, st, g, pb, p, cell_start, u, v, w, ub, vb, wb, 1.0, ss);
+}
 void launch_g2p(hipStream_t st, Grid g, long n, Particles p, const double* dcx, const double* dcy, const double* dcz, const double* pcx,
                 const double* pcy, const double* pcz, double blend, StepState* ss)
 {
diff --git a/fluid-simulation_amd/csrc/sim.h b/fluid-simulation_amd/csrc/sim.h
--- a/fluid-simulation_amd/csrc/sim.h
+++ b/fluid-simulation_amd/csrc/sim.h
@@ -122,8 +122,11 @@
     bool sort_hint = false;
     bool advect_bin = true;
     bool binned = false;
+    bool sort_fold = true;
+    bool tail_zero = false;
     int bin_x0 = 0, bin_x1 = -1;
     int bin_min[3] = {0, 0, 0}, bin_max[3] = {-1, -1, -1}, bin_n_out = 0, bin_max_cell = 0;
+    bool g2p_delta = true;
     bool solve_tail = true;
     bool tail_ran = false;
     double dt = 0.1;
@@ -135,6 +138,9 @@
     int mg_csweeps = 3;
     MLevel mgl[MG_MAXL];
     uint8_t *mg_typ[MG_MAXL] = {}, *mg_cnt[MG_MAXL] = {};
+    bool tail_recip = true;
+    bool down_ng2 = true;
+    bool mg_fused = true;
     int gal_mode = 1;
     int gal_it[2] = {-1, -1};
     int gal_since_probe = 0;
```

Measured after the change: 159.3, median of 3. About the same (+0.3%).
